# r9y9/gantts

Measured on AMD Instinct MI355X. Metric: acoustic frames/sec per G+D GAN step (B=32,T=512), higher is better.
Workload: dtype f32; 1 GPU; cfg2: TTS acoustic MLP G 425-512x3-187 + conditioned MLP D 483-256x3-1, Adagrad, MGE+ADV loss, global B=32 T=512 (32 sequences per GPU, strong scaling), fp32, dropout 0.5 (Philox); global_batch=32, per_gpu_batch=32, parallelism=dp1

## Files before the change

### gantts_amd/_lib.py

```python
import ctypes as C
import os

import torch

_HERE = os.path.dirname(os.path.abspath(__file__))
LIB_PATH = os.environ.get("GT_HIP_LIB") or os.path.join(_HERE, "libgantts_hip.so")

GT_OK, GT_ERR_INVALID, GT_ERR_HIP, GT_ERR_STATE, GT_ERR_DIM = 0, 1, 2, 3, 4
ROLE_G, ROLE_D = 0, 1
OPT_LSTM_PERSISTENT, OPT_LSTM_FWD_UNITS, OPT_LSTM_XCD_LOCAL, OPT_MATMUL_BF16, OPT_SPLIT_FIRST_LAYER = 2, 3, 4, 5, 6
OPT_COMM_D_ONE_MSG, OPT_COMM_EARLY_G, OPT_COMM_FORCE = 10, 11, 13
OPT_LAUNCH_RIDERS, OPT_COMM_CLOSE_INLINE, OPT_POLL_RESULTS = 14, 15, 16
OPT_COMM_TV_IN_SUMS, OPT_COMM_IPC, OPT_FUSED_DSTACK = 17, 18, 19
OPT_SRU_D_BF16 = 20
IPC_HANDLE_BYTES, IPC_MAX_WORLD = 64, 8
PROFILE_SLOTS = 16
LSTM_PATH_SLOTS, LSTM_PATH_STEPS, LSTM_PATH_DECLINED = 34, 32, 33
GEMM_PATH_SLOTS = 588
GEMM_B16_PATH_SLOTS = 66
SRU_PATH_SLOTS = 13
CAST_PLAIN_F32, CAST_PLAIN_BF16, CAST_SEQDROP, CAST_CAT, CAST_CATDROP, CAST_MULTI = 0, 1, 2, 3, 4, 5
CAST_MAX_JOBS = 8
GEMM_ROUTE_FORWARD, GEMM_ROUTE_FORWARD_SEG, GEMM_ROUTE_BACKWARD_DATA, GEMM_ROUTE_WEIGHT_GRAD, GEMM_ROUTE_WEIGHT_GRAD_SPLIT = 0, 1, 2, 3, 4
ARCH_MLP, ARCH_IN2OUT, ARCH_LSTM, ARCH_SRU, ARCH_IN2OUT_RNN = 0, 1, 2, 3, 4
OPT_ADAGRAD, OPT_ADAM = 0, 1
OPT_SGD, OPT_RMSPROP, OPT_ADADELTA, OPT_ADAMW, OPT_ADAMAX = 2, 3, 4, 5, 6
OPT_NADAM, OPT_RADAM, OPT_RPROP, OPT_ASGD = 7, 8, 9, 10
OPTF_NESTEROV, OPTF_CENTERED, OPTF_AMSGRAD, OPTF_BUFFER_LIVE = 1, 2, 4, 8
OPTF_DECOUPLED_WD = 32
MAX_STREAMS = 8
COMM_ID_BYTES = 128


class StreamConfig(C.Structure):
    _fields_ = [("n_streams", C.c_int32),
                ("stream_sizes", C.c_int32 * MAX_STREAMS),
                ("has_dynamic_features", C.c_int32 * MAX_STREAMS),
                ("num_windows", C.c_int32),
                ("adversarial_streams", C.c_int32 * MAX_STREAMS),
                ("mask_nth_mgc_for_adv_loss", C.c_int32),
                ("discriminator_linguistic_condition", C.c_int32),
                ("cond_dim", C.c_int32)]


class ModelDesc(C.Structure):
    _fields_ = [("arch", C.c_int32), ("in_dim", C.c_int32), ("out_dim", C.c_int32),
                ("num_hidden", C.c_int32), ("hidden_dim", C.c_int32), ("static_dim", C.c_int32),
                ("dropout", C.c_float), ("last_sigmoid", C.c_int32),
                ("bidirectional", C.c_int32), ("use_relu", C.c_int32),
                ("rnn_dropout", C.c_float), ("reserved_", C.c_int32),
                ("params", C.c_void_p), ("grads", C.c_void_p), ("n_params", C.c_int64)]


class OptimDesc(C.Structure):
    _fields_ = [("kind", C.c_int32), ("lr", C.c_float), ("weight_decay", C.c_float), ("eps", C.c_float),
                ("lr_decay", C.c_float), ("beta1", C.c_float), ("beta2", C.c_float),
                ("max_grad_norm", C.c_float), ("step", C.c_int64),
                ("state0", C.c_void_p), ("state1", C.c_void_p)]


class OptimDescEx(C.Structure):
    _fields_ = ([("kind", C.c_int32), ("flags", C.c_uint32)]
                + [(n, C.c_double) for n in ("lr", "weight_decay", "eps", "lr_decay", "beta1", "beta2", "momentum", "dampening", "alpha")]
                + [("max_grad_norm", C.c_float), ("reserved_", C.c_int32), ("step", C.c_int64),
                   ("state0", C.c_void_p), ("state1", C.c_void_p), ("state2", C.c_void_p)])


class OptimDescEx2(OptimDescEx):
    _fields_ = [(n, C.c_double) for n in ("momentum_decay", "etaminus", "etaplus", "step_size_min", "step_size_max", "lambd", "t0",
                                          "host_state0", "host_state1")]


class DResult(C.Structure):
    _fields_ = [("loss_d", C.c_float), ("loss_fake_d", C.c_float), ("loss_real_d", C.c_float),
                ("real_correct_count", C.c_float), ("fake_correct_count", C.c_float), ("grad_norm", C.c_float)]


class GResult(C.Structure):
    _fields_ = [("loss_mse", C.c_float), ("loss_mge", C.c_float), ("loss_adv", C.c_float),
                ("loss_g", C.c_float), ("grad_norm", C.c_float)]


class GemmCase(C.Structure):
    _fields_ = ([(n, C.c_int32) for n in ("route", "prec", "rows", "in_dim", "out_dim", "act", "drop")] + [("p", C.c_float)]
                + [("key0", C.c_uint32), ("key1", C.c_uint32)]
                + [(n, C.c_int32) for n in ("accumulate", "col0", "ncols", "wrap", "cd", "rider", "defer", "ldx", "ldw", "ldy", "ld_dy",
                                            "ldh", "ld_mask", "ld_addm", "ld_adv", "ld_dx")]
                + [(n, C.c_void_p) for n in ("x", "w", "bias", "y", "dy", "h", "mask", "addm", "adv", "dx", "dw", "db")])


class GemmB16Case(C.Structure):
    _fields_ = ([(n, C.c_int32) for n in ("route", "rows", "in_dim", "out_dim", "act", "drop")] + [("p", C.c_float)]
                + [("key0", C.c_uint32), ("key1", C.c_uint32)]
                + [(n, C.c_int32) for n in ("accumulate", "ldx", "ldw", "ld_dy", "ldh", "ld_mask", "ldc", "ldcb", "ldcbt")]
                + [(n, C.c_void_p) for n in ("x", "w", "bias", "dy", "h", "mask", "c", "cb", "cbt", "dw", "db")])


# ... 13 lines not shown

class CastCase(C.Structure):
    _fields_ = ([(n, C.c_int32) for n in ("kind", "cols", "ldi", "ldo", "colsum_accumulate", "T", "cd", "ldf", "n_jobs", "pad_")]
                + [(n, C.c_int64) for n in ("rows", "ldt", "N", "row_off")]
                + [(n, C.c_void_p) for n in ("in_", "out", "outT", "colsum", "mul", "x", "fa", "fb", "idx")]
                + [("jobs", CastJob * CAST_MAX_JOBS)])


_P, _I, _F, _L = C.c_void_p, C.c_int, C.c_float, C.c_int64

class DistortionSums(C.Structure):
    _fields_ = [(n, C.c_double) for n in
                ("s_mcd", "s_bap", "s_f0", "n_voiced", "n_vuv_err", "s_mse", "n_frames")]


SIGNATURES = {
    "gt_last_error": (C.c_char_p, []),
    "gt_version": (C.c_char_p, []),
    "gt_engine_create": (_I, [C.POINTER(StreamConfig), C.POINTER(_P)]),
    "gt_engine_destroy": (None, [_P]),
    "gt_bind_model": (_I, [_P, _I, C.POINTER(ModelDesc)]),
    "gt_bind_optimizer": (_I, [_P, _I, C.POINTER(OptimDesc)]),
    "gt_bind_optimizer_ex": (_I, [_P, _I, C.POINTER(OptimDescEx)]),
    "gt_op_optim_step": (_I, [C.POINTER(OptimDescEx), _P, _P, _L, _P, C.POINTER(_F), _P]),
    "gt_set_training": (_I, [_P, _I, _I]),
    "gt_set_lr": (_I, [_P, _I, _F]),
    "gt_get_optimizer_step": (_I, [_P, _I, C.POINTER(_L)]),
    "gt_get_optimizer_scalars": (_I, [_P, _I, C.POINTER(C.c_double)]),
    "gt_op_optim_scalars": (_I, [C.POINTER(OptimDescEx), _L, C.POINTER(C.c_double)]),
    "gt_set_seed": (_I, [_P, C.c_uint64]),
    "gt_set_dropout_mask": (_I, [_P, _I, _I, _I, _P]),
    "gt_op_philox_mask": (_I, [_P, _I, _I, _I, _L, _F, _L, _I, _P, _P]),
    "gt_set_lengths": (_I, [_P, C.POINTER(_L), _I, _P]),
    "gt_invalidate_mlpg_cache": (_I, [_P]),
    "gt_zero_grad": (_I, [_P, _I]),
    "gt_apply_generator": (_I, [_P, _P, _P, _I, _I, _P, _P, _P]),
    "gt_update_discriminator": (_I, [_P, _P, _P, _P, _P, _I, _I, _I, _F, C.POINTER(DResult), _P]),
    "gt_update_generator": (_I, [_P, _P, _P, _P, _P, _P, _F, _P, _I, _I, _I, _F, _F, _F, C.POINTER(GResult), _P]),
    "gt_set_loss_normalizer": (_I, [_P, _F]),
    "gt_set_loss_normalizer_device": (_I, [_P, _P]),
    "gt_set_option": (_I, [_P, _I, _I]),
    "gt_set_x_pitch": (_I, [_P, _I, _I]),
    "gt_set_tuning": (_I, [C.c_char_p, _I]),
    "gt_check_faults": (_I, [_P, _P]),
    "gt_lstm_path_counts": (_I, [_P, C.POINTER(_L), _I]),
    "gt_gemm_path_counts": (_I, [C.POINTER(_L), _I]),
    "gt_op_gemm_f32": (_I, [C.POINTER(GemmCase), _P]),
    "gt_gemm_b16_path_counts": (_I, [C.POINTER(_L), _I]),
    "gt_op_gemm_b16": (_I, [C.POINTER(GemmB16Case), _P]),
    "gt_op_cast_image": (_I, [C.POINTER(CastCase), _P]),
    "gt_sru_path_counts": (_I, [C.POINTER(_L), _I]),
    "gt_op_sru_scan": (_I, [C.POINTER(SruScanCase), _P]),
    "gt_op_sru_dx_adv_finish": (_I, [_P, _L, _I, _I, _P, _I, _P, _I, _P]),
    "gt_op_sru_input_mask": (_I, [_P, _I, _I, _F, C.c_uint32, C.c_uint32, _P, _I, _I, _P]),
    "gt_op_sru_input_dropout": (_I, [_P, _I, _P, _I, _I, _I, _I, _P, _P]),
    "gt_clear_faults": (_I, [_P, _P]),
    "gt_comm_unique_id": (_I, [_P]),
    "gt_comm_init": (_I, [_P, _I, _I, _P]),
    "gt_comm_destroy": (_I, [_P]),
    "gt_comm_info": (_I, [_P, C.POINTER(_I), C.POINTER(_I)]),
    "gt_comm_trace": (_I, [_P, _I]),
    "gt_comm_trace_read": (_I, [_P, C.POINTER(C.c_double), _I, C.POINTER(_I)]),
    "gt_set_shard": (_I, [_P, _I, _I]),
    "gt_comm_ipc_export": (_I, [_P, _P]),
    "gt_comm_ipc_attach": (_I, [_P, _I, _I, _P]),
    "gt_comm_ipc_messages": (_I, [_P, C.POINTER(C.c_longlong)]),
    "gt_update_discriminator_begin": (_I, [_P, _P, _P, _P, _P, _I, _I, _I, _F, _P]),
    "gt_update_discriminator_end": (_I, [_P, _I, C.POINTER(DResult), _P]),
    "gt_update_generator_begin": (_I, [_P, _P, _P, _P, _P, _P, _F, _P, _I, _I, _I, _F, _F, _F, _P]),
    "gt_update_generator_end": (_I, [_P, _I, _F, _F, _F, C.POINTER(GResult), _P]),
    "gt_update_discriminator_result": (_I, [_P, C.POINTER(DResult)]),
    "gt_update_generator_result": (_I, [_P, C.POINTER(GResult)]),
    "gt_scalar_buffer": (_I, [_P, C.POINTER(_P), C.POINTER(_I)]),
    "gt_model_forward": (_I, [_P, _I, _P, _P, _I, _I, _P, _P, _P]),
    "gt_flush_generator_grads": (_I, [_P, _P]),
    "gt_op_sequence_mask": (_I, [_P, _I, _I, _P, _P]),
    "gt_op_masked_mse": (_I, [_P, _P, _P, _I, _I, _I, C.POINTER(_F), _P, _P]),
    "gt_compute_distortions": (_I, [_P, _P, _I, _P, _P, _I, C.POINTER(_I), C.POINTER(_I), _I, C.POINTER(_L), _I, _I,
                                    C.POINTER(DistortionSums), _P]),
    "gt_op_gather_cols": (_I, [_P, _I, _P, _I, _P, _I, _I, _L, _P]),
    "gt_op_pad_sequences": (_I, [_P, _I, _P, _P, _I, _I, _P, _I, _P]),
    "gt_op_mlpg_forward": (_I, [_P, _P, _P, _I, _I, _P, _P]),
    "gt_op_mlpg_backward": (_I, [_P, _P, _P, _I, _I, _P, _P]),
    "gt_op_linear_forward": (_I, [_P, _I, _P, _P, _P, _I, _L, _I, _I, _I, _P, _F, _P]),
    "gt_op_linear_bf16": (_I, [_P, _P, _P, _L, _I, _I, _I, _P, _F, _P, _P, _P, _I, _P, _F, _P, _P, _P, _P, _P, _P]),
    "gt_profile_enable": (_I, [_I]),
    "gt_profile_read": (_I, [C.POINTER(C.c_double), C.POINTER(C.c_double), C.POINTER(_L)]),
    "gt_profile_bytes": (_I, [C.POINTER(C.c_double)]),
    "gt_op_linear_backward": (_I, [_P, _I, _P, _I, _P, _L, _I, _I, _P, _I, _P, _I, _P, _F, _P, _P, _P]),
}


def _build_if_missing():
    import fcntl
    import shutil
    import subprocess
    if os.path.isfile(LIB_PATH):
        return
    if shutil.which("hipcc") is None and not os.path.isfile("/opt/rocm/bin/hipcc"):
        return
    with open(os.path.join(_HERE, ".build.lock"), "w") as lock:
        fcntl.flock(lock, fcntl.LOCK_EX)
        try:
            if not os.path.isfile(LIB_PATH):
                subprocess.call(["make", "-j8", "-C", os.path.join(_HERE, "csrc")], stdout=subprocess.DEVNULL)
        finally:
            fcntl.flock(lock, fcntl.LOCK_UN)


def _load():
    _build_if_missing()
    if not os.path.isfile(LIB_PATH):
        raise ImportError(
            "gantts_amd: %s not found -- the HIP engine is the product and has no fallback. "
            "Build it: make -C %s" % (LIB_PATH, os.path.join(_HERE, "csrc")))
    lib = C.CDLL(LIB_PATH)
    for name, (res, args) in SIGNATURES.items():
        fn = getattr(lib, name)
        fn.restype, fn.argtypes = res, args
    return lib


lib = _load()


class GanttsHipError(RuntimeError):
    pass


def check(rc):
    if rc == GT_OK:
        return
    msg = lib.gt_last_error().decode("utf-8", "replace")
    if rc == GT_ERR_DIM:
        raise RuntimeError(msg)
    if rc == GT_ERR_INVALID:
        raise ValueError(msg)
    if rc == GT_ERR_STATE:
        raise RuntimeError(msg)
    raise GanttsHipError("HIP error: " + msg)


def ptr(t):
    return None if t is None else C.c_void_p(t.data_ptr())


def current_stream():
    import torch
    return C.c_void_p(torch.cuda.current_stream().cuda_stream)
```

### gantts_amd/csrc/eng_core.hip

```cpp
#include "engine_internal.hip.h"

using namespace gt;
static thread_local char g_err[512] = "";
int fail(int code, const char* fmt, ...) {
  va_list ap;
  va_start(ap, fmt);
  vsnprintf(g_err, sizeof(g_err), fmt, ap);
  va_end(ap);
  return code;
}
extern "C" const char* gt_last_error(void) { return g_err; }
extern "C" const char* gt_version(void) { return "gantts_hip 0.1 (gfx950, f32 MFMA)"; }

int ensure_dyn_lds(const void* kernel, size_t bytes) {
  static std::mutex mu;
  static std::map<std::pair<const void*, int>, size_t> done;
  int dev = 0;
  HIPCHK(hipGetDevice(&dev));
  std::lock_guard<std::mutex> lk(mu);
  size_t& cur = done[std::make_pair(kernel, dev)];
  if (bytes > cur) {
    HIPCHK(hipFuncSetAttribute(kernel, hipFuncAttributeMaxDynamicSharedMemorySize, (int)bytes));
    cur = bytes;
  }
// ... 281 lines not shown
  Net& n = e->net[role];
  if (!n.bound) return fail(GT_ERR_STATE, "bind the model before its optimizer");
  if (!n.d.grads) return fail(GT_ERR_INVALID, "model was bound without a grads buffer");
  if (od->kind != GT_OPT_ADAGRAD && od->kind != GT_OPT_ADAM) return fail(GT_ERR_INVALID, "unknown optimizer kind");
  if (!od->state0 || (od->kind == GT_OPT_ADAM && !od->state1)) return fail(GT_ERR_INVALID, "optimizer state buffer is null");
  gt_optim_desc_ex x;
  memset(&x, 0, sizeof(x));
  x.kind = od->kind; x.lr = od->lr; x.weight_decay = od->weight_decay; x.eps = od->eps; x.lr_decay = od->lr_decay;
  x.beta1 = od->beta1; x.beta2 = od->beta2; x.max_grad_norm = od->max_grad_norm; x.step = od->step;
  x.state0 = od->state0; x.state1 = od->state1;
  n.od = x;
  n.step = n.bound_step = od->step;
  n.buf_live = false;
  n.hs_cache = OptimScalarCache();
  n.has_opt = true;
  return GT_OK;
}
extern "C" int gt_bind_optimizer_ex(gt_engine* e, int role, const gt_optim_desc_ex* od) {
  if (!e || !od || role < 0 || role > 1) return fail(GT_ERR_INVALID, "bad argument");
  Net& n = e->net[role];
  if (!n.bound) return fail(GT_ERR_STATE, "bind the model before its optimizer");
  if (!n.d.grads) return fail(GT_ERR_INVALID, "model was bound without a grads buffer");
  CHK(optim_check_desc(od));
  optim_desc_copy(od, &n.od);
  if (od->kind != GT_OPT_ASGD) n.od.lr = (double)(float)od->lr;
  n.step = n.bound_step = od->step;
  n.hs_cache = OptimScalarCache();
  n.buf_live = (od->flags & GT_OPTF_BUFFER_LIVE) != 0;
  n.has_opt = true;
  return GT_OK;
}
extern "C" int gt_set_training(gt_engine* e, int role, int training) {
  if (!e || role < 0 || role > 1) return fail(GT_ERR_INVALID, "bad argument");
  e->net[role].training = training != 0;
  return GT_OK;
}
extern "C" int gt_set_lr(gt_engine* e, int role, float lr) {
  if (!e || role < 0 || role > 1 || !e->net[role].has_opt) return fail(GT_ERR_INVALID, "no optimizer bound");
  e->net[role].od.lr = lr;
  return GT_OK;
}
extern "C" int gt_get_optimizer_step(gt_engine* e, int role, int64_t* step) {
  if (!e || role < 0 || role > 1 || !step) return fail(GT_ERR_INVALID, "bad argument");
  *step = e->net[role].step;
  return GT_OK;
}
extern "C" int gt_get_optimizer_scalars(gt_engine* e, int role, double out[2]) {
  if (!e || role < 0 || role > 1 || !out) return fail(GT_ERR_INVALID, "bad argument");
  Net& n = e->net[role];
  if (!n.has_opt) return fail(GT_ERR_INVALID, "no optimizer bound");
  optim_host_scalars(n.od, n.step, &n.hs_cache, out);
  return GT_OK;
}
extern "C" int gt_set_seed(gt_engine* e, uint64_t seed) {
  if (!e) return fail(GT_ERR_INVALID, "null engine");
  e->seed = seed;
  e->step_counter = 0;
  return GT_OK;
}
extern "C" int gt_set_dropout_mask(gt_engine* e, int role, int pass, int layer, const float* mask) {
  if (!e || role < 0 || role > 1 || pass < 0 || pass > 2 || layer < 0 || layer > 15) return fail(GT_ERR_INVALID, "bad argument");
  e->net[role].inj[pass][layer] = mask;
  return GT_OK;
}
extern "C" int gt_set_option(gt_engine* e, int option, int value) {
  if (!e) return fail(GT_ERR_INVALID, "null engine");
  switch (option) {
    case GT_OPT_LSTM_PERSISTENT: e->lstm_persistent = value != 0; return GT_OK;
    case GT_OPT_LSTM_FWD_UNITS: e->lstm_fwd_upc = value; return GT_OK;
    case GT_OPT_LSTM_XCD_LOCAL: e->lstm_xcd_local = value != 0; return GT_OK;
    case GT_OPT_SPLIT_FIRST_LAYER:
      if (e->opt_split_first != (value != 0)) invalidate_d_images(e);
      e->opt_split_first = value != 0;
      return GT_OK;
    case GT_OPT_COMM_D_ONE_MSG: e->opt_comm_d_one_msg = value != 0; return GT_OK;
    case GT_OPT_COMM_EARLY_G: e->opt_comm_early_g = value != 0; return GT_OK;
    case GT_OPT_COMM_FORCE: e->opt_comm_force = value != 0; return GT_OK;
    case GT_OPT_COMM_CLOSE_INLINE: e->opt_comm_close_inline = value != 0; return GT_OK;
    case GT_OPT_COMM_IPC: e->opt_comm_ipc = value != 0; return GT_OK;
    case GT_OPT_FUSED_DSTACK: e->opt_fused_dstack = value < 0 ? 0 : value > 2 ? 2 : value; return GT_OK;
    case GT_OPT_COMM_TV_IN_SUMS: e->opt_comm_tv_in_sums = value != 0; return GT_OK;
    case GT_OPT_POLL_RESULTS: e->opt_poll_results = value != 0; return GT_OK;
    case GT_OPT_LAUNCH_RIDERS: e->opt_launch_riders = value != 0; return GT_OK;
    case GT_OPT_MATMUL_BF16:
      if (e->matmul_bf16 != (value != 0)) {
        invalidate_d_images(e);
        e->g_pass_valid = false; e->leak_pending = false; e->cxd_src = nullptr;
        e->d_begin_done = false; e->g_begin_done = false;
      }
      e->matmul_bf16 = value != 0;
      return GT_OK;
    case GT_OPT_SRU_D_BF16:
      if (value != 0 && value != 1) return fail(GT_ERR_INVALID, "GT_OPT_SRU_D_BF16 takes 0 or 1, not %d", value);
      if (e->sru_d_bf16 != (value != 0)) { invalidate_d_images(e); e->leak_pending = false; e->d_begin_done = false; e->g_begin_done = false; }
      e->sru_d_bf16 = value != 0;
      return GT_OK;
  }
  return fail(GT_ERR_INVALID, "unknown option %d", option);
}
GtTuning& gt_tuning() {
  static GtTuning t = [] {
    GtTuning v;
    auto geti = [](const char* n, int d) { const char* s = getenv(n); return s && s[0] ? atoi(s) : d; };
    v.gemm_pair = geti("GT_GEMM_PAIR", v.gemm_pair); v.pair_order = geti("GT_PAIR_ORDER", v.pair_order);
    { const char* s = getenv("GT_GEMM_TILES"); v.gemm_tiles_big = s && !strcmp(s, "big") ? 1 : 0; }
    v.gemm_unaligned = geti("GT_GEMM_UNALIGNED", v.gemm_unaligned); v.tn_wgs = geti("GT_TN_WGS", v.tn_wgs); v.tn_split_wgs = geti("GT_TN_SPLIT_WGS", v.tn_split_wgs); v.split_fused = geti("GT_SPLIT_FUSED", v.split_fused);
    v.b16_tiles = geti("GT_B16_TILES", v.b16_tiles); v.b16_wg_tile = geti("GT_B16_WG_TILE", v.b16_wg_tile); v.b16_dma = geti("GT_B16_DMA", v.b16_dma);
    v.mlpg_fpl = geti("GT_MLPG_FPL", v.mlpg_fpl); v.mlpg_tt = geti("GT_MLPG_TT", v.mlpg_tt); v.sru_coop = geti("GT_SRU_COOP", v.sru_coop); v.sru_cs_waves = geti("GT_SRU_CS_WAVES", v.sru_cs_waves); v.leak_rider = geti("GT_LEAK_RIDER", v.leak_rider);
    v.head_vec = geti("GT_HEAD_VEC", v.head_vec);
    v.lstm_bt = geti("GT_LSTM_BT", v.lstm_bt);
    if (v.lstm_bt != 8 && v.lstm_bt != 16) v.lstm_bt = 0;
    return v;
  }();
  return t;
}
extern "C" int gt_set_tuning(const char* name, int value) {
  if (!name) return fail(GT_ERR_INVALID, "null name");
  GtTuning& t = gt_tuning();
  struct { const char* n; int* p; } tab[] = {
      {"gemm_pair", &t.gemm_pair}, {"pair_order", &t.pair_order}, {"gemm_tiles_big", &t.gemm_tiles_big}, {"gemm_unaligned", &t.gemm_unaligned},
      {"tn_wgs", &t.tn_wgs}, {"tn_split_wgs", &t.tn_split_wgs}, {"split_fused", &t.split_fused}, {"b16_tiles", &t.b16_tiles},
      {"b16_wg_tile", &t.b16_wg_tile}, {"b16_dma", &t.b16_dma}, {"mlpg_fpl", &t.mlpg_fpl}, {"mlpg_tt", &t.mlpg_tt}, {"sru_coop", &t.sru_coop}, {"sru_cs_waves", &t.sru_cs_waves}, {"leak_rider", &t.leak_rider}, {"head_vec", &t.head_vec}};
  if (!strcmp(name, "lstm_bt")) {
    if (value != 0 && value != 8 && value != 16) return fail(GT_ERR_INVALID, "lstm_bt must be 0 (by shape), 8 or 16, not %d", value);
    t.lstm_bt = value;
    return GT_OK;
  }
  if (!strcmp(name, "sru_lw")) { t.sru_coop = value >= 2; return GT_OK; }
  for (auto& e : tab) if (!strcmp(e.n, name)) { *e.p = value; return GT_OK; }
  return fail(GT_ERR_INVALID, "unknown tuning knob '%s'", name);
}
extern "C" int gt_set_x_pitch(gt_engine* e, int ld_generator_input, int ld_condition) {
  if (!e || ld_generator_input < 0 || ld_condition < 0) return fail(GT_ERR_INVALID, "bad argument");
  e->ld_gx = ld_generator_input; e->ld_cx = ld_condition;
  return GT_OK;
}
extern "C" int gt_set_loss_normalizer(gt_engine* e, float tv) {
  if (!e) return fail(GT_ERR_INVALID, "null engine");
  e->tv_override = tv;
  e->tv_dev = nullptr;
  return GT_OK;
}
extern "C" int gt_set_loss_normalizer_device(gt_engine* e, const double* tv_dev) {
  if (!e) return fail(GT_ERR_INVALID, "null engine");
  e->tv_dev = tv_dev;
  e->tv_mask = nullptr; e->tv_inflight = false;
  return GT_OK;
}
extern "C" int gt_set_lengths(gt_engine* e, const int64_t* lengths_host, int B, void* stream) {
  if (!e || !lengths_host || B < 1) return fail(GT_ERR_INVALID, "bad argument");
  hipStream_t s = (hipStream_t)stream;
  e->h_lengths.resize(B);
  for (int b = 0; b < B; ++b) {
    if (lengths_host[b] < 0 || lengths_host[b] > 0x3fffffff) return fail(GT_ERR_INVALID, "length out of range");
    e->h_lengths[b] = (int)lengths_host[b];
  }
  if (2 * B > e->len_cap) {
    HIPCHK(hipStreamSynchronize(s));
    const int cap = std::max(64, 2 * B + B);
    for (int i = 0; i < gt_engine::LEN_RING; ++i) {
      if (e->len_ev[i]) HIPCHK(hipEventSynchronize(e->len_ev[i]));
      if (e->len_host[i]) { HIPCHK(hipHostFree(e->len_host[i])); e->len_host[i] = nullptr; }
      HIPCHK(hipHostMalloc((void**)&e->len_host[i], (size_t)cap * sizeof(int)));
      if (!e->len_ev[i]) HIPCHK(hipEventCreateWithFlags(&e->len_ev[i], hipEventDisableTiming));
    }
    e->len_cap = cap;
// ... 127 lines not shown
```

### gantts_amd/csrc/eng_ops.hip

```cpp
#include "engine_internal.hip.h"

using namespace gt;
extern "C" int gt_op_sequence_mask(const int64_t* lengths, int B, int T, float* mask, void* stream) {
  if (!lengths || !mask || B < 1 || T < 1) return fail(GT_ERR_INVALID, "bad argument");
  hipLaunchKernelGGL(sequence_mask_kernel, dim3(cdiv((long)B * T, 256)), dim3(256), 0, (hipStream_t)stream, (const long*)lengths, B, T, mask);
  LAUNCH_CHECK();
  return GT_OK;
}

extern "C" int gt_op_masked_mse(const float* input, const float* target, const float* mask, int B, int T, int D, float* loss_out,
                                float* grad_input, void* stream) {
  if (!input || !target) return fail(GT_ERR_INVALID, "null tensor");
  if (!mask) return fail(GT_ERR_INVALID, "Should provide either lengths or mask");
  hipStream_t s = (hipStream_t)stream;
  const long N = (long)B * T;
  static thread_local Scratch tls_ws;
  CHK(tls_ws.ensure(1024 + 1024 * sizeof(double)));
  void* ws = tls_ws.p;
  StepScalars* sc = (StepScalars*)ws;
  double* part = (double*)((char*)ws + 1024);
  hipLaunchKernelGGL(mask_sum_kernel, dim3(1), dim3(1024), 0, s, mask, (int)N, -1.f, (const double*)nullptr, sc);
  const int nblk = (int)std::min<long>(1000, cdiv(N * D, RED_THREADS * 4));
  hipLaunchKernelGGL(masked_sqerr_kernel, dim3(nblk), dim3(RED_THREADS), 0, s, input, D, target, D, mask, N, D, part, grad_input, D,
                     1.f, sc);
  hipLaunchKernelGGL(sum_partials_kernel, dim3(1), dim3(256), 0, s, part, nblk, &sc->s_mse);
  StepScalars h;
  hipError_t err = hipMemcpyAsync(&h, sc, sizeof(h), hipMemcpyDeviceToHost, s);
  if (err == hipSuccess) err = hipStreamSynchronize(s);
  if (err != hipSuccess) return fail(GT_ERR_HIP, "masked_mse: %s", hipGetErrorString(err));
  if (loss_out) *loss_out = (float)h.s_mse / h.tv;
  return GT_OK;
}

extern "C" int gt_compute_distortions(const float* y_static, const float* y_hat_static, int Ds, const void* stat_mean,
                                      const void* stat_std, int stats_f64, const int32_t* col_stat_host,
                                      const int32_t* col_role_host, int vuv_col, const int64_t* lengths_host, int B, int T,
                                      gt_distortion_sums* out, void* stream) {
  if (!y_static || !y_hat_static || !stat_mean || !stat_std || !col_stat_host || !col_role_host || !out)
    return fail(GT_ERR_INVALID, "null argument");
  if (Ds < 1 || B < 1 || T < 1 || vuv_col >= Ds) return fail(GT_ERR_DIM, "bad sizes: Ds=%d B=%d T=%d vuv_col=%d", Ds, B, T, vuv_col);
  hipStream_t s = (hipStream_t)stream;
  const long N = (long)B * T;
  const int nblk = (int)std::min<long>(1024, cdiv(N, 4));
  std::vector<int> host(2 * Ds + B);
  for (int c = 0; c < Ds; ++c) {
    if (col_stat_host[c] < 0) return fail(GT_ERR_INVALID, "negative statistics index");
    host[c] = col_stat_host[c];
    host[Ds + c] = col_role_host[c];
  }
  for (int b = 0; b < B; ++b) {
    const int64_t n = lengths_host ? lengths_host[b] : T;
    if (n < 0 || n > T) return fail(GT_ERR_INVALID, "length %lld outside [0, T=%d]", (long long)n, T);
    host[2 * Ds + b] = (int)n;
  }
  static thread_local Scratch tls_ws;
  const size_t off_part = ((host.size() * sizeof(int) + 255) / 256) * 256;
  const size_t off_out = off_part + (size_t)nblk * DIST_NSUM * sizeof(double);
  CHK(tls_ws.ensure(off_out + DIST_NSUM * sizeof(double)));
  void* ws = tls_ws.p;
  int* d_int = (int*)ws;
  double* part = (double*)((char*)ws + off_part);
  double* d_out = (double*)((char*)ws + off_out);
  hipError_t err = hipMemcpyAsync(d_int, host.data(), host.size() * sizeof(int), hipMemcpyHostToDevice, s);
  if (err == hipSuccess) {
    if (stats_f64)
      hipLaunchKernelGGL(distortion_kernel<double>, dim3(nblk), dim3(256), 0, s, y_static, y_hat_static, Ds, (const double*)stat_mean,
                         (const double*)stat_std, d_int, d_int + Ds, vuv_col, d_int + 2 * Ds, B, T, part);
    else
      hipLaunchKernelGGL(distortion_kernel<float>, dim3(nblk), dim3(256), 0, s, y_static, y_hat_static, Ds, (const float*)stat_mean,
                         (const float*)stat_std, d_int, d_int + Ds, vuv_col, d_int + 2 * Ds, B, T, part);
    hipLaunchKernelGGL(distortion_finalize_kernel, dim3(1), dim3(64 * DIST_NSUM), 0, s, part, nblk, d_out);
    err = hipGetLastError();
  }
  double h[DIST_NSUM];
  if (err == hipSuccess) err = hipMemcpyAsync(h, d_out, sizeof(h), hipMemcpyDeviceToHost, s);
  if (err == hipSuccess) err = hipStreamSynchronize(s);
  if (err != hipSuccess) return fail(GT_ERR_HIP, "compute_distortions: %s", hipGetErrorString(err));
  out->s_mcd = h[0]; out->s_bap = h[1]; out->s_f0 = h[2]; out->n_voiced = h[3];
  out->n_vuv_err = h[4]; out->s_mse = h[5]; out->n_frames = h[6];
  return GT_OK;
}

extern "C" int gt_op_pad_sequences(const float* ragged, int D, const int64_t* start, const int64_t* len, int B, int T, float* out, int ld_out,
                                   void* stream) {
  if (!ragged || !start || !len || !out || D < 1 || B < 1 || T < 1 || ld_out < D) return fail(GT_ERR_INVALID, "bad argument");
  hipLaunchKernelGGL(pad_sequences_kernel, dim3(cdiv((long)B * T * ld_out, 256)), dim3(256), 0, (hipStream_t)stream, ragged, D,
                     (const long*)start, (const long*)len, B, T, out, ld_out);
  LAUNCH_CHECK();
  return GT_OK;
}
extern "C" int gt_op_gather_cols(const float* in, int ld_in, const int32_t* idx, int n_idx, float* out, int ld_out,
                                 int out_col_offset, int64_t rows, void* stream) {
  if (!in || !out || n_idx < 0 || rows < 0) return fail(GT_ERR_INVALID, "bad argument");
  if (rows == 0 || n_idx == 0) return GT_OK;
  hipLaunchKernelGGL(gather_cols_kernel, dim3(cdiv(rows * n_idx, 256)), dim3(256), 0, (hipStream_t)stream, in, ld_in, 0, idx, out,
                     ld_out, out_col_offset, (int)rows, n_idx);
  LAUNCH_CHECK();
  return GT_OK;
}

extern "C" int gt_op_mlpg_forward(gt_engine* e, const float* y, const float* R, int B, int T, float* y_static, void* stream) {
  CHK(check_common(e, B, T));
  if (!y || !R || !y_static) return fail(GT_ERR_INVALID, "null tensor");
  hipStream_t s = (hipStream_t)stream;
  CHK(ensure_band(e, R, T, s));
  return mlpg_forward(e, y, e->Dout_cfg, e->d_scol, e->d_sstride, e->Ds, y_static, e->Ds, B, T, s);
}
extern "C" int gt_op_mlpg_backward(gt_engine* e, const float* g_static, const float* R, int B, int T, float* g_y, void* stream) {
  CHK(check_common(e, B, T));
  if (!g_static || !R || !g_y) return fail(GT_ERR_INVALID, "null tensor");
  hipStream_t s = (hipStream_t)stream;
  CHK(ensure_band(e, R, T, s));
  return mlpg_backward(e, g_static, e->Ds, e->d_scol, e->d_sstride, e->Ds, g_y, e->Dout_cfg, B, T, 0.f, nullptr, nullptr, 0, nullptr, s);
}

static DropoutSpec buffer_spec(const float* keep_mask, float p, int ld) {
  DropoutSpec d = no_drop();
  if (keep_mask && p > 0.f) { d.mode = DROP_BUFFER; d.mask = keep_mask; d.ld_mask = ld; d.p = p; d.scale = 1.f / (1.f - p); }
  return d;
}

extern "C" int gt_op_linear_forward(const float* X, int ldx, const float* W, const float* bias, float* Y, int ldy, int64_t rows,
                                    int in_dim, int out_dim, int act, const float* keep_mask, float p, void* stream) {
  if (!X || !W || !Y || rows < 1 || in_dim < 1 || out_dim < 1) return fail(GT_ERR_INVALID, "bad argument");
  if (act < 0 || act > 2) return fail(GT_ERR_INVALID, "unknown activation");
  tl_gemm_prec = PREC_F32;
  return linear_forward(X, ldx, W, in_dim, bias, Y, ldy, rows, in_dim, out_dim, act, buffer_spec(keep_mask, p, out_dim), (hipStream_t)stream);
}

extern "C" int gt_op_linear_backward(const float* dY, int lddy, const float* X, int ldx, const float* W, int64_t rows, int in_dim,
                                     int out_dim, float* dX, int lddx, const float* H_prev, int act_prev,
                                     const float* keep_mask_prev, float p_prev, float* dW, float* db, void* stream) {
  if (!dY || rows < 1 || in_dim < 1 || out_dim < 1) return fail(GT_ERR_INVALID, "bad argument");
  hipStream_t s = (hipStream_t)stream;
  tl_gemm_prec = PREC_F32;
  if (dX) {
    if (!W) return fail(GT_ERR_INVALID, "dX requested without W");
    if (act_prev != ACT_NONE && !H_prev) return fail(GT_ERR_INVALID, "activation derivative requested without H_prev");
    CHK(linear_backward_data(dY, lddy, W, in_dim, 0, dX, lddx, rows, out_dim, in_dim, act_prev, H_prev, in_dim,
                             buffer_spec(keep_mask_prev, p_prev, in_dim), s));
  }
  if (dW || db) {
    if (dW && !X) return fail(GT_ERR_INVALID, "dW requested without X");
    Scratch slabs, colp;
    int r = linear_backward_weight(dY, lddy, X, ldx, rows, out_dim, in_dim, dW, db, false, slabs, colp, s);
    hipError_t err = hipStreamSynchronize(s);
    slabs.release(); colp.release();
    if (r) return r;
    if (err != hipSuccess) return fail(GT_ERR_HIP, "linear_backward: %s", hipGetErrorString(err));
  }
  return GT_OK;
}

extern "C" int gt_op_linear_bf16(const float* X, const float* W, const float* bias, int64_t rows, int in_dim, int out_dim, int act,
                                 const float* keep_mask, float p, float* Y, const float* dY, const float* H_prev, int act_prev,
                                 const float* keep_mask_prev, float p_prev, float* dX, float* dW, float* db,
                                 float* Y_image, float* YT_image, void* stream) {
  if (!X || !W || rows < 1 || in_dim < 1 || out_dim < 1) return fail(GT_ERR_INVALID, "bad argument");
  if (act < 0 || act > 2 || act_prev < 0 || act_prev > 2) return fail(GT_ERR_INVALID, "unknown activation");
  hipStream_t s = (hipStream_t)stream;
  const int in8 = pad8(in_dim), out8 = pad8(out_dim);
  const long rows8 = pad8(rows);
  Scratch xb, xbt, wb, wbt, yb, ybt, dyb, dybt, hb, slabs, colp;
  int r = GT_OK;
  auto body = [&]() -> int {
    CHK(xb.ensure((size_t)rows * in8 * 2)); CHK(xbt.ensure((size_t)in_dim * rows8 * 2));
    CHK(wb.ensure((size_t)out_dim * in8 * 2)); CHK(wbt.ensure((size_t)in_dim * out8 * 2));
    CHK(cast_transpose(X, in_dim, rows, in_dim, xb.as<__bf16>(), in8, xbt.as<__bf16>(), rows8, nullptr, false, &colp, s));
    CHK(cast_transpose(W, in_dim, out_dim, in_dim, wb.as<__bf16>(), in8, wbt.as<__bf16>(), out8, nullptr, false, &colp, s));
    if (Y) {
      CHK(yb.ensure((size_t)rows * out8 * 2)); CHK(ybt.ensure((size_t)out_dim * rows8 * 2));
      GemmB16Args g = b16_args();
      g.A = xb.as<__bf16>(); g.lda = in8; g.B = wb.as<__bf16>(); g.ldb = in8; g.M = (int)rows; g.N = out_dim; g.K = in_dim;
      g.C = Y; g.ldc = out_dim; g.Cb = yb.as<__bf16>(); g.ldcb = out8; g.CbT = ybt.as<__bf16>(); g.ldcbt = (int)rows8;
      g.bias = bias; g.epi = B16_FWD; g.act = act; g.drop = buffer_spec(keep_mask, p, out_dim);
      CHK(launch_gemm_b16(g, 1, s));
      if (Y_image) {
        hipLaunchKernelGGL(bf16_to_f32_kernel, dim3(cdiv(rows * out_dim, 256)), dim3(256), 0, s, (const __bf16*)yb.as<__bf16>(), (long)out8, rows, out_dim, Y_image);
        LAUNCH_CHECK();
      }
      if (YT_image) {
        hipLaunchKernelGGL(bf16_to_f32_kernel, dim3(cdiv(rows * out_dim, 256)), dim3(256), 0, s, (const __bf16*)ybt.as<__bf16>(), rows8, (long)out_dim, (int)rows, YT_image);
        LAUNCH_CHECK();
      }
    }
    if (dY) {
      CHK(dyb.ensure((size_t)rows * out8 * 2)); CHK(dybt.ensure((size_t)out_dim * rows8 * 2));
      CHK(cast_transpose(dY, out_dim, rows, out_dim, dyb.as<__bf16>(), out8, dybt.as<__bf16>(), rows8, nullptr, false, &colp, s));
      if (dX) {
// ... 597 lines not shown
```

### gantts_amd/csrc/eng_step.hip

```cpp
#include "engine_internal.hip.h"
#include "dstack_f32.hip.h"

using namespace gt;
int ensure_band(gt_engine* e, const float* R, int T, hipStream_t s) {
  MlpgCache& m = e->mlpg;
  ++m.tick;
  for (auto* b : m.entries)
    if (b->R == R && b->T == T) { b->last_use = m.tick; m.cur = b; return GT_OK; }
  const int nW = e->cfg.num_windows;
  CHK(m.tmp.ensure((size_t)(2 * T - 1) * sizeof(float)));
  hipLaunchKernelGGL(mlpg_offset_max_kernel, dim3(2 * T - 1), dim3(256), 0, s, R, T, nW, m.tmp.as<float>());
  LAUNCH_CHECK();
  std::vector<float> off(2 * T - 1);
  HIPCHK(hipMemcpyAsync(off.data(), m.tmp.p, off.size() * sizeof(float), hipMemcpyDeviceToHost, s));
  HIPCHK(hipStreamSynchronize(s));
  float peak = 0.f;
  for (float v : off) peak = fmaxf(peak, v);
  if (!(peak > 0.f) || !isfinite(peak)) return fail(GT_ERR_INVALID, "MLPG matrix R is empty or not finite");
  int kb = 0;
  for (int o = -(T - 1); o <= T - 1; ++o)
    if (off[o + T - 1] > 1e-9f * peak) kb = std::max(kb, abs(o));
  if (kb > 63 || (kb > 48 && kb > T / 4))
    return fail(GT_ERR_INVALID, "MLPG matrix R is not banded (half-width %d of T=%d): only window sets whose "
                "R = (W^T W)^-1 W^T decays (hparams.py:22-26) are supported", kb, T);
  MlpgBand* b = nullptr;
  if (m.entries.size() >= MlpgCache::MAX_ENTRIES) {
    size_t lru = 0;
    for (size_t i = 1; i < m.entries.size(); ++i) if (m.entries[i]->last_use < m.entries[lru]->last_use) lru = i;
    b = m.entries[lru];
    HIPCHK(hipStreamSynchronize(s));
  } else {
    b = new MlpgBand();
    m.entries.push_back(b);
  }
  const int nb = 2 * kb + 1;
  b->R = nullptr;
  CHK(b->band.ensure((size_t)T * nW * nb * sizeof(float)));
  hipLaunchKernelGGL(mlpg_extract_band_kernel, dim3(cdiv((long)T * nW * nb, 256)), dim3(256), 0, s, R, T, nW, kb, b->band.as<float>());
  LAUNCH_CHECK();
  b->R = R; b->T = T; b->kb = kb; b->last_use = m.tick;
  m.cur = b;
  return GT_OK;
}
extern "C" int gt_invalidate_mlpg_cache(gt_engine* e) {
  if (!e) return fail(GT_ERR_INVALID, "null engine");
  HIPCHK(hipDeviceSynchronize());
  e->mlpg.clear();
  return GT_OK;
}

static int mlpg_tile_frames() { return gt_tuning().mlpg_tt == 16 ? 16 : 32; }
int mlpg_forward(gt_engine* e, const float* y, int ldy, const int* scol, const int* sstride, int Ds,
                 float* ys, int ldys, int B, int T, hipStream_t s) {
  const int nW = e->cfg.num_windows, kb = e->mlpg.cur->kb;
  auto lds_of = [&](int tt) { return ((size_t)(tt + 2 * kb) * nW * MLPG_CC + (size_t)tt * nW * (2 * kb + 1 + 2 * MLPG_PAD)) * sizeof(float); };
  const int tt = mlpg_tile_frames();
  const size_t lds = lds_of(tt);
  dim3 grid(B * cdiv(T, tt), cdiv(Ds, MLPG_CC));
  const int fpl = gt_tuning().mlpg_fpl;
#define GT_MLPG_FWD(F, TTV) { CHK(ensure_dyn_lds((const void*)mlpg_forward_kernel<F, TTV>, lds)); \
    hipLaunchKernelGGL((mlpg_forward_kernel<F, TTV>), grid, dim3(MLPG_THREADS), lds, s, y, ldy, e->mlpg.cur->band.as<float>(), kb, nW, scol, sstride, Ds, ys, ldys, B, T); }
  if (tt == 16) GT_MLPG_FWD(2, 16)
  else { if (fpl == 1) GT_MLPG_FWD(1, 32) else if (fpl == 2) GT_MLPG_FWD(2, 32) else GT_MLPG_FWD(4, 32) }
#undef GT_MLPG_FWD
  LAUNCH_CHECK();
  return GT_OK;
}
int mlpg_backward(gt_engine* e, const float* gs, int ldgs, const int* scol, const int* sstride, int Ds,
                  float* gy, int ldgy, int B, int T, float mse_w, const float* yhat, const float* ytgt, int ldt,
                  const float* mask, hipStream_t s) {
  const int nW = e->cfg.num_windows, kb = e->mlpg.cur->kb;
  auto lds_of = [&](int tt) { return ((size_t)(tt + 2 * kb) * MLPG_CC + (size_t)(tt + 2 * kb) * nW * (2 * kb + 1 + 2 * MLPG_PAD)) * sizeof(float); };
  const int tt = mlpg_tile_frames();
  const size_t lds = lds_of(tt);
  dim3 grid(B * cdiv(T, tt), cdiv(Ds, MLPG_CC));
  const int fpl = gt_tuning().mlpg_fpl;
#define GT_MLPG_BWD(F, TTV) { CHK(ensure_dyn_lds((const void*)mlpg_backward_kernel<F, TTV>, lds)); \
    hipLaunchKernelGGL((mlpg_backward_kernel<F, TTV>), grid, dim3(MLPG_THREADS), lds, s, gs, ldgs, e->mlpg.cur->band.as<float>(), kb, nW, scol, sstride, Ds, \
                       gy, ldgy, B, T, mse_w, yhat, ytgt, ldt, mask, e->sc()); }
  if (tt == 16) GT_MLPG_BWD(2, 16)
  else { if (fpl == 1) GT_MLPG_BWD(1, 32) else if (fpl == 2) GT_MLPG_BWD(2, 32) else GT_MLPG_BWD(4, 32) }
#undef GT_MLPG_BWD
  LAUNCH_CHECK();
  return GT_OK;
}

static int stage_injected(gt_engine* e, int role, int layer, const int* passes, int npass, long rows_each, int width,
                          const float** out, hipStream_t s) {
  Net& n = e->net[role];
  *out = nullptr;
  if (!n.training || n.d.dropout <= 0.f) return GT_OK;
  bool any = false, all = true;
  for (int i = 0; i < npass; ++i) { any |= n.inj[passes[i]][layer] != nullptr; all &= n.inj[passes[i]][layer] != nullptr; }
  if (!any) return GT_OK;
  if (!all) return fail(GT_ERR_INVALID, "injected dropout masks must be given for every pass of a step or for none");
  if (npass == 1) { *out = n.inj[passes[0]][layer]; return GT_OK; }
  const size_t per_layer = (size_t)npass * rows_each * width * sizeof(float);
  CHK(e->dmask.ensure(per_layer * n.d.num_hidden));
  float* base = (float*)((char*)e->dmask.p + per_layer * layer);
  for (int i = 0; i < npass; ++i)
    HIPCHK(hipMemcpyAsync(base + (size_t)i * rows_each * width, n.inj[passes[i]][layer], (size_t)rows_each * width * sizeof(float),
                          hipMemcpyDeviceToDevice, s));
  *out = base;
  return GT_OK;
}

struct FirstSplit {
  const float* x; int ldx; int cd;
  const float* xp; int ldxp;
  const float* adv; int ld_adv;
  long wrap;
};
static int pitched_rows(gt_engine* e, int slot, const float* p, int ld, int cols, long rows, const float** out, int* ldo, hipStream_t s) {
  if (gemm_vec_ok(p, ld)) { *out = p; *ldo = ld; return GT_OK; }
  gt_engine::Pitched& P = e->pitched[slot];
  const int ldp = (cols + 3) & ~3;
  if (!(P.src == p && P.ld == ld && P.cols == cols && P.rows == rows && P.step == e->step_counter)) {
    CHK(P.buf.ensure((size_t)rows * ldp * sizeof(float)));
    hipLaunchKernelGGL(repitch_kernel, dim3(cdiv(rows * (ldp / 4), 256)), dim3(256), 0, s, p, ld, cols, rows, P.buf.as<float>(), ldp);
    LAUNCH_CHECK();
    P.src = p; P.ld = ld; P.cols = cols; P.rows = rows; P.step = e->step_counter;
  }
  *out = P.buf.as<float>(); *ldo = ldp;
  return GT_OK;
}

static int stack_forward(gt_engine* e, int role, const float* in, int ld_in, long rows, std::vector<Scratch>& acts,
                         const int* passes, int npass, long rows_each, std::vector<DropoutSpec>& specs, hipStream_t s,
                         const FirstSplit* fs = nullptr, int max_layers = 1 << 30 ) {
  Net& n = e->net[role];
  specs.resize(n.hidden.size());
  const float* cur = in;
  int ld = ld_in;
  for (size_t l = 0; l < n.hidden.size(); ++l) {
    const Lin& L = n.hidden[l];
    CHK(acts[l].ensure((size_t)rows * L.out * sizeof(float)));
    const float* inj = nullptr;
    CHK(stage_injected(e, role, (int)l, passes, npass, rows_each, L.out, &inj, s));
    specs[l] = drop_spec(e, role, passes[0], (int)l, inj, L.out, npass == 2 ? rows_each : 0);
    if ((int)l >= max_layers) continue;
    if (l == 0 && fs && specs[l].mode == DROP_PHILOX && gt_tuning().split_fused && gemm_vec_ok(fs->x, fs->ldx, true) &&
        gemm_vec_ok(L.W, L.in, true) && gemm_vec_ok(fs->adv, fs->ld_adv, true) && fs->wrap > 64 && gemm_small_tiles_ok() &&
        tl_gemm_prec == PREC_F32 && (rows == fs->wrap || rows == 2 * fs->wrap)) {
      GemmArgs g;
      memset(&g, 0, sizeof(g));
      g.A = fs->x; g.lda = fs->ldx; g.B = L.W; g.ldb = L.in; g.C = acts[l].as<float>(); g.ldc = L.out;
      g.M = (int)fs->wrap; g.N = L.out; g.K = fs->cd; g.bias = L.b; g.act = ACT_LEAKY_DROPOUT; g.drop = specs[l];
      g.A_seg = fs->adv; g.lda_seg = fs->ld_adv; g.B_seg = L.W + fs->cd; g.K_seg = L.in - fs->cd;
      g.dual_rows = rows == 2 * fs->wrap ? (int)fs->wrap : 0;
      CHK(launch_gemm(GEMM_NT, g, 1, s));
      cur = acts[l].as<float>();
      ld = L.out;
      continue;
    }
    if (l == 0 && fs) {
      const int Da = L.in - fs->cd;
      CHK(e->d_pre.ensure((size_t)fs->wrap * L.out * sizeof(float)));
      CHK(linear_forward(fs->x, fs->ldx, L.W, L.in, L.b, e->d_pre.as<float>(), L.out, fs->wrap, fs->cd, L.out, ACT_NONE, no_drop(), s));
      GemmArgs g;
      memset(&g, 0, sizeof(g));
      g.A = fs->adv; g.lda = fs->ld_adv; g.B = L.W + fs->cd; g.ldb = L.in; g.C = acts[l].as<float>(); g.ldc = L.out;
      g.M = (int)rows; g.N = L.out; g.K = Da; g.act = ACT_LEAKY_DROPOUT; g.drop = specs[l];
      g.addm = e->d_pre.as<float>(); g.ld_addm = L.out; g.addm_wrap = (int)fs->wrap;
      CHK(launch_gemm(GEMM_NT, g, 1, s));
// ... 729 lines not shown
  CHK(d_pass_head(e, p, hc, nullptr, s));
  e->early_done = false;
  if (plain_early) CHK(post_early_results(e, s, hc.ticket));
  if (comm_early) CHK(comm_early_results(e, GT_ROLE_D, unnorm ? &e->sc()->tv_sum : &e->sc()->s_real, unnorm ? 5 : 4, 0.f, 0.f, 0.f, s));
  if (tr) {
    CHK(comm_grads_ready(e, GT_ROLE_D, D.last.dW, (long)D.last.in * D.last.out + D.last.out, s));
    Net& G = e->net[GT_ROLE_G];
    const bool want_leak = G.bound && G.d.grads && e->g_pass_valid && y_hat_static == e->last_yhs && e->N == N;
    if (want_leak && e->leak_pending)
      return fail(GT_ERR_STATE, "update_discriminator called twice without optimizer_g.zero_grad() (train.py:538)");
    float* leak = nullptr;
    if (want_leak) { CHK(e->leak.ensure((size_t)N * e->Da * sizeof(float))); leak = e->leak.as<float>(); }
    CHK(d_pass_backward(e, p, leak, s));
    D.grads_dirty = true;
    if (want_leak) { e->leak_pending = true; e->leak_unnorm = unnorm; }
  }
  CHK(comm_finish_step(e, GT_ROLE_D, tr, &e->sc()->s_real, comm_early ? 0 : 4, s));
  e->d_begin_done = true;
  return GT_OK;
}

static void fill_d_result(const StepResults* h, gt_d_result* out) {
  out->loss_d = h->loss_d; out->loss_fake_d = h->loss_fake_d; out->loss_real_d = h->loss_real_d;
  out->real_correct_count = h->real_correct; out->fake_correct_count = h->fake_correct;
  out->grad_norm = h->gnorm_d;
}
static void fill_g_result(const StepResults* h, gt_g_result* out) {
  out->loss_mse = h->loss_mse; out->loss_mge = h->loss_mge; out->loss_adv = h->loss_adv;
  out->loss_g = h->loss_g; out->grad_norm = h->gnorm_g;
}

extern "C" int gt_update_discriminator_end(gt_engine* e, int train, gt_d_result* out, void* stream) {
  if (!e) return fail(GT_ERR_INVALID, "null argument");
  if (!e->d_begin_done) return fail(GT_ERR_STATE, "gt_update_discriminator_end without _begin");
  hipStream_t s = (hipStream_t)stream;
  e->d_begin_done = false;
  if (!out && e->early_done) return fail(GT_ERR_STATE, "deferred results are a split-phase feature");
  if (train) CHK(optimizer_step(e, GT_ROLE_D, &e->sc()->gnorm2_d, s));
  if (e->early_done) {
    CHK(wait_early_results(e));
    e->early_done = false;
  } else {
    hipLaunchKernelGGL(finalize_d_kernel, dim3(1), dim3(1), 0, s, e->sc(), e->res(), train ? 0 : 1);
    LAUNCH_CHECK();
    if (!out) return post_deferred_results(e, GT_ROLE_D, s);
    CHK(fetch_results(e, s));
  }
  fill_d_result(e->h_res, out);
  return GT_OK;
}
extern "C" int gt_update_discriminator_result(gt_engine* e, gt_d_result* out) {
  if (!e || !out) return fail(GT_ERR_INVALID, "null argument");
  if (!e->def_pending[GT_ROLE_D]) return fail(GT_ERR_STATE, "no deferred discriminator result pending");
  HIPCHK(hipEventSynchronize(e->ev_def[GT_ROLE_D]));
  e->def_pending[GT_ROLE_D] = false;
  fill_d_result(e->h_def[GT_ROLE_D], out);
  return GT_OK;
}

extern "C" int gt_update_discriminator(gt_engine* e, const float* x, const float* y_static, const float* y_hat_static,
                                       const float* mask, int B, int T, int train, float eps, gt_d_result* out, void* stream) {
  if (!e) return fail(GT_ERR_INVALID, "null engine");
  e->early = true;
  int r = gt_update_discriminator_begin(e, x, y_static, y_hat_static, mask, B, T, train, eps, stream);
  e->early = false;
  if (r != GT_OK) { e->early_done = false; e->d_unnorm = false; e->ticket_wait = 0; return r; }
  return gt_update_discriminator_end(e, train, out, stream);
}

static int sum_sqerr(gt_engine* e, const float* a, int lda, const float* b, int ldb, const float* mask, long rows, int D,
                     double* out, float* g, int ldg, float gscale, hipStream_t s, int* deferred_blocks = nullptr) {
  const int nblk = (int)std::min<long>(1024, cdiv(rows * D, RED_THREADS * 4));
  CHK(e->partial.ensure(4096 * sizeof(double)));
  double* part = e->partial.as<double>() + 1024;
  hipLaunchKernelGGL(masked_sqerr_kernel, dim3(nblk), dim3(RED_THREADS), 0, s, a, lda, b, ldb, mask, rows, D, part, g, ldg, gscale, e->sc());
  LAUNCH_CHECK();
  if (deferred_blocks) { *deferred_blocks = nblk; return GT_OK; }
  hipLaunchKernelGGL(sum_partials_kernel, dim3(1), dim3(256), 0, s, part, nblk, out);
  LAUNCH_CHECK();
  return GT_OK;
}

static int generator_backward(gt_engine* e, const float* x, const float* y, const float* y_hat, const float* mask,
                              float mse_w, hipStream_t s) {
  Net& G = e->net[GT_ROLE_G];
  const long N = e->N;
  const int B = e->B, T = e->T, Do = G.d.out_dim;
  const bool mlp_body = !(has_lstm_body(G.d.arch) || G.d.arch == GT_ARCH_SRU);
  const int ldgy = mlp_body && (is_i2o(G.d.arch) || e->g_used_mlpg) ? (Do + 3) & ~3 : Do;
  CHK(e->gy.ensure((size_t)N * ldgy * sizeof(float)));
  float* gy = e->gy.as<float>();
  const float* gs = e->gs.as<float>();
  if (is_i2o(G.d.arch)) {
    const int sd = G.d.static_dim;
    if (G.d.arch == GT_ARCH_IN2OUT_RNN) mse_w = 0.f;
    CHK(e->dgx.ensure((size_t)N * sd * sizeof(float)));
    CHK(e->dtz.ensure((size_t)N * sd * sizeof(float)));
    hipLaunchKernelGGL(highway_backward_kernel, dim3(cdiv(N * sd, 256)), dim3(256), 0, s, gs, sd, e->tx.as<float>(), sd,
                       e->gx.as<float>(), sd, e->dgx.as<float>(), sd, e->dtz.as<float>(), sd, N, sd);
    LAUNCH_CHECK();
    CHK(linear_backward_weight(e->dtz.as<float>(), sd, x, G.d.in_dim, N, sd, sd, G.gate.dW, G.gate.db, G.grads_dirty, e->slabs,
                               e->colp, s, &e->sdefer[GT_ROLE_G]));
    CHK(comm_grads_ready(e, GT_ROLE_G, G.gate.dW, (long)sd * sd + sd, s));
    CHK(mlpg_backward(e, e->dgx.as<float>(), sd, e->d_scol_i2o, e->d_sstride_i2o, sd, gy, ldgy, B, T, mse_w, y_hat, y, Do, mask, s));
  } else if (e->g_used_mlpg) {
    CHK(mlpg_backward(e, gs, e->Ds, e->d_scol, e->d_sstride, e->Ds, gy, ldgy, B, T, mse_w, y_hat, y, Do, mask, s));
  } else {
    if (mse_w != 0.f) CHK(sum_sqerr(e, y_hat, Do, y, Do, mask, N, Do, &e->sc()->s_mse, gy, Do, mse_w, s));
    hipLaunchKernelGGL(slab_reduce_kernel, dim3(cdiv(N * Do, 256)), dim3(256), 0, s, gs, 0L, 1, N * Do, gy, mse_w != 0.f ? 1 : 0);
    LAUNCH_CHECK();
  }
  if (G.d.last_sigmoid && !is_i2o(G.d.arch)) {
    hipLaunchKernelGGL(sigmoid_grad_kernel, dim3(cdiv(N * Do, 256)), dim3(256), 0, s, gy, ldgy, y_hat, Do, N, Do);
    LAUNCH_CHECK();
  }
  if (has_lstm_body(G.d.arch) || G.d.arch == GT_ARCH_SRU) {
    CHK(has_lstm_body(G.d.arch) ? lstm_backward(e, x, gy, B, T, s) : sru_backward(e, x, gy, B, T, s));
    G.grads_dirty = true;
    return GT_OK;
  }
  if (use_b16(e, GT_ROLE_G)) {
    const int H = G.d.hidden_dim;
    CHK(e->gy_b.ensure(N, Do, true));
    CHK(cast_transpose(gy, ldgy, N, Do, e->gy_b.r(), e->gy_b.ld, e->gy_b.t(), e->gy_b.ldt, nullptr, false, &e->colp, s));
    B16Img& top = e->g_actb.back();
    CHK(weight_grad_b16(e->gy_b.t(), e->gy_b.ldt, top.t(), top.ldt, N, Do, G.last.in, G.last.dW, G.last.db, G.grads_dirty, e->slabs, s,
                        &e->sdefer[GT_ROLE_G]));
    CHK(comm_grads_ready(e, GT_ROLE_G, G.last.dW, (long)Do * G.last.in + Do, s));
    const LinShadow& ws = e->wsh[GT_ROLE_G][G.hidden.size()];
    CHK(e->dz_b[0].ensure(N, H, true));
    GemmB16Args g = b16_args();
    g.A = e->gy_b.r(); g.lda = e->gy_b.ld; g.B = ws.wt.as<__bf16>(); g.ldb = ws.ldwt; g.M = (int)N; g.N = H; g.K = Do;
    g.epi = B16_BWD_DATA; g.act = ACT_LEAKY_DROPOUT; g.H = top.r(); g.ldh = top.ld; g.drop = e->g_specs.back();
    g.Cb = e->dz_b[0].r(); g.ldcb = e->dz_b[0].ld; g.CbT = e->dz_b[0].t(); g.ldcbt = (int)e->dz_b[0].ldt;
    CHK(launch_gemm_b16(g, 1, s));
    CHK(stack_backward_b16(e, GT_ROLE_G, e->xin_b.t(), e->xin_b.ldt, N, e->g_actb, e->g_specs, 0, true, nullptr, 0, 0, 0, 0, 0, s));
    G.grads_dirty = true;
    return GT_OK;
  }
  const Lin& Lt = G.hidden.back();
  const int H = G.d.hidden_dim;
  CHK(e->dzA.ensure((size_t)2 * N * H * sizeof(float)));
  CHK(e->dzB.ensure((size_t)2 * N * H * sizeof(float)));
  const GemmArgs nn_last = backward_data_args(gy, ldgy, G.last.W, G.last.in, 0, e->dzA.as<float>(), H, N, Do, H, ACT_LEAKY_DROPOUT,
                                              e->g_act.back().as<float>(), H, e->g_specs.back());
  bool rode = false;
  CHK(linear_backward_weight(gy, ldgy, e->g_act.back().as<float>(), Lt.out, N, Do, G.last.in, G.last.dW, G.last.db, G.grads_dirty,
                             e->slabs, e->colp, s, &e->sdefer[GT_ROLE_G], &nn_last, &rode));
  CHK(comm_grads_ready(e, GT_ROLE_G, G.last.dW, (long)Do * G.last.in + Do, s));
  if (!rode) CHK(launch_gemm(GEMM_NN, nn_last, 1, s));
  const float* xin = x;
  int ldxin = gx_pitch(e);
  if (!gemm_vec_ok(x, ldxin) && tl_gemm_prec == PREC_F32) {
    if (e->img_cat.valid && e->img_cat.x == x && e->cfg.discriminator_linguistic_condition && cond_dim(e) == G.d.in_dim && e->dcat.p) {
      ldxin = (d_in_dim(e) + 3) & ~3;
      xin = e->dcat.as<float>() + N * ldxin;
    } else {
      const int slot = (e->pitched[0].src == x && e->pitched[0].ld == gx_pitch(e) && e->pitched[0].cols == G.d.in_dim && e->pitched[0].step == e->step_counter) ? 0 : 1;
      CHK(pitched_rows(e, slot, x, gx_pitch(e), G.d.in_dim, N, &xin, &ldxin, s));
    }
  }
  CHK(stack_backward(e, GT_ROLE_G, xin, ldxin, N, e->g_act, e->g_specs, e->dzA.as<float>(), e->dzB.as<float>(), true,
                     nullptr, 0, 0, 0, 0, 0, s));
  G.grads_dirty = true;
  return GT_OK;
}

extern "C" int gt_update_generator_begin(gt_engine* e, const float* x, const float* y, const float* y_hat, const float* y_static,
                                         const float* y_hat_static, float adv_w, const float* mask, int B, int T, int train,
                                         float mse_w, float mge_w, float eps, void* stream) {
  CHK(check_common(e, B, T));
  Net& G = e->net[GT_ROLE_G];
  Net& D = e->net[GT_ROLE_D];
  if (!G.bound) return fail(GT_ERR_STATE, "generator not bound");
  if (!y || !y_hat || !y_static || !y_hat_static || !mask) return fail(GT_ERR_INVALID, "null tensor");
  hipStream_t s = (hipStream_t)stream;
  const long N = (long)B * T;
  const bool tr = train != 0;
  if (tr) {
    if (!e->g_pass_valid || y_hat != e->last_yhat || y_hat_static != e->last_yhs || N != e->N)
      return fail(GT_ERR_STATE, "update_generator(phase=\"train\") needs the y_hat / y_hat_static returned by the last apply_generator");
    if (!G.d.grads) return fail(GT_ERR_STATE, "phase == \"train\" but the generator was bound without grads");
  }
  const int Do = G.d.out_dim;
  const int Ds = is_i2o(G.d.arch) ? G.d.static_dim : e->Ds;
  if (comm_on(e) && tr && G.grads_dirty)
    return fail(GT_ERR_STATE, "data-parallel step: optimizer_g.zero_grad() must precede update_generator");
  e->sdefer[GT_ROLE_G].reset(e->early && tr && G.has_opt);
  CHK(ensure_tv(e, mask, N, s));
  const bool direct = !is_i2o(G.d.arch) && !e->g_used_mlpg;
  const bool early_fold = e->early && !comm_on(e) && !(tr && direct && mse_w != 0.f);
  int mse_blocks = 0, mge_pre_blocks = 0;
  const bool riders = early_fold && e->opt_launch_riders;
  const bool riders_dp = e->early && comm_on(e) && e->opt_launch_riders && !(tr && direct && mse_w != 0.f);
  if (riders || riders_dp) {
    mse_blocks = (int)std::min<long>(1024, cdiv(N * Do, RED_THREADS * 4));
    mge_pre_blocks = (int)std::min<long>(1024, cdiv(N * Ds, RED_THREADS * 4));
    CHK(e->partial.ensure(4096 * sizeof(double)));
    hipLaunchKernelGGL(g_losses_kernel, dim3(mse_blocks + mge_pre_blocks), dim3(RED_THREADS), 0, s, y_hat, Do, y, Do, Do, mse_blocks,
                       e->partial.as<double>() + 1024, y_hat_static, Ds, y_static, Ds, Ds, e->partial.as<double>(), mask, N);
    LAUNCH_CHECK();
  } else if (!(tr && direct && mse_w != 0.f)) {
    CHK(sum_sqerr(e, y_hat, Do, y, Do, mask, N, Do, &e->sc()->s_mse, nullptr, 0, 0.f, s, early_fold ? &mse_blocks : nullptr));
  }
  e->g_has_adv = adv_w > 0.f;
  float* gadv = nullptr;
  int head_blocks = 0;
  if (adv_w > 0.f) {
    if (!D.bound) return fail(GT_ERR_STATE, "adv_w > 0 but no discriminator bound");
    DPass p;
    CHK(d_pass_plan(e, x, nullptr, y_hat_static, Ds, 1, B, T, false, &p));
    AdvRiders none;
    memset(&none, 0, sizeof(none));
    CHK(d_pass_input(e, p, none, s));
    CHK(d_pass_forward(e, p, s));
    if (tr) { CHK(e->gadv.ensure((size_t)N * e->Da * sizeof(float))); gadv = e->gadv.as<float>(); }
    HeadCall hc;
    memset(&hc, 0, sizeof(hc));
    hc.mode = HEAD_G_ADV; hc.rows = p.rows; hc.n_real = N; hc.mask = mask; hc.n_mask = N; hc.eps = eps; hc.want_grad = tr; hc.want_w = false;
    hc.defer_scalars = riders || riders_dp ? &head_blocks : nullptr;
    CHK(d_pass_head(e, p, hc, gadv, s));
    if (tr) CHK(d_pass_backward(e, p, gadv, s));
  }
  const bool early_ok = e->early && !(tr && direct && mse_w != 0.f);
  const bool early_now = early_ok && !comm_on(e), comm_early = early_ok && comm_on(e) && e->opt_comm_early_g;
  int mge_blocks = 0;
  e->early_done = false;
  {
    const int nblk = (int)std::min<long>(1024, cdiv(N * Ds, RED_THREADS * 4));
    CHK(e->partial.ensure(4096 * sizeof(double)));
    float* gs = nullptr;
    if (tr) { CHK(e->gs.ensure((size_t)N * Ds * sizeof(float))); gs = e->gs.as<float>(); }
    const float* leak = (tr && e->leak_pending) ? e->leak.as<float>() : nullptr;
    GFinalize fin;
    memset(&fin, 0, sizeof(fin));
    const bool rid = riders || riders_dp;
    if (rid) {
      fin.on = 1; fin.sc = e->sc(); fin.out = riders ? early_res_target(e) : (StepResults*)nullptr; fin.adv_w = adv_w; fin.mse_w = mse_w; fin.mge_w = mge_w;
      fin.has_adv = e->g_has_adv ? 1 : 0;
      fin.part_mge = e->partial.as<double>(); fin.n_mge = mge_pre_blocks;
      fin.part_mse = e->partial.as<double>() + 1024; fin.n_mse = mse_blocks;
      fin.hp = head_blocks ? e->headp.as<HeadPartials>() : (const HeadPartials*)nullptr; fin.n_hp = head_blocks;
      if (riders) { fin.ticket_value = take_ticket(e); fin.ticket = fin.ticket_value ? e->ticket_dev() : (unsigned*)nullptr; }
    }
    if (tr || !rid)
      hipLaunchKernelGGL(static_grad_kernel, dim3(nblk + (rid ? 1 : 0)), dim3(RED_THREADS), 0, s, y_hat_static, Ds,
                         y_static, Ds, mask, N, Ds, mge_w, e->d_adv_inv, leak, e->Da, gadv, e->Da, adv_w, gs, Ds,
                         rid ? (double*)nullptr : e->partial.as<double>(), e->sc(), fin, leak && e->leak_unnorm ? 1 : 0);
    else
      hipLaunchKernelGGL(finalize_g_rider_kernel, dim3(1), dim3(RED_THREADS), 0, s, fin);
    LAUNCH_CHECK();
    mge_blocks = nblk;
    if (riders) CHK(post_early_results(e, s, fin.ticket_value));
    else if (!early_now && !riders_dp) {
      hipLaunchKernelGGL(sum_partials_kernel, dim3(1), dim3(256), 0, s, e->partial.as<double>(), nblk, &e->sc()->s_mge);
      LAUNCH_CHECK();
    }
  }
  if (early_now && !riders) {
    hipLaunchKernelGGL(finalize_g_kernel, dim3(1), dim3(256), 0, s, e->sc(), early_res_target(e), adv_w, mse_w, mge_w, e->g_has_adv ? 1 : 0, 1,
                       (const double*)e->partial.as<double>(), mge_blocks,
                       mse_blocks ? (const double*)(e->partial.as<double>() + 1024) : (const double*)nullptr, mse_blocks);
    LAUNCH_CHECK();
    CHK(post_early_results(e, s));
  }
  if (comm_early) CHK(comm_early_results(e, GT_ROLE_G, &e->sc()->s_adv, 3, adv_w, mse_w, mge_w, s));
  if (tr) {
    CHK(generator_backward(e, e->last_x, y, y_hat, mask, mse_w, s));
    e->leak_pending = false; e->leak_unnorm = false;
  }
  CHK(comm_finish_step(e, GT_ROLE_G, tr, &e->sc()->s_adv, comm_early ? 0 : 3, s));
  e->g_begin_done = true;
  return GT_OK;
}

extern "C" int gt_update_generator_end(gt_engine* e, int train, float adv_w, float mse_w, float mge_w, gt_g_result* out,
                                       void* stream) {
  if (!e) return fail(GT_ERR_INVALID, "null argument");
  if (!e->g_begin_done) return fail(GT_ERR_STATE, "gt_update_generator_end without _begin");
  hipStream_t s = (hipStream_t)stream;
  e->g_begin_done = false;
  if (!out && e->early_done) return fail(GT_ERR_STATE, "deferred results are a split-phase feature");
  if (train) CHK(optimizer_step(e, GT_ROLE_G, &e->sc()->gnorm2_g, s));
  if (e->early_done) {
    CHK(wait_early_results(e));
    e->early_done = false;
  } else {
    hipLaunchKernelGGL(finalize_g_kernel, dim3(1), dim3(1), 0, s, e->sc(), e->res(), adv_w, mse_w, mge_w, e->g_has_adv ? 1 : 0,
                       train ? 0 : 1, (const double*)nullptr, 0, (const double*)nullptr, 0);
    LAUNCH_CHECK();
    if (!out) return post_deferred_results(e, GT_ROLE_G, s);
    CHK(fetch_results(e, s));
  }
  fill_g_result(e->h_res, out);
  return fault_seen(e);
}
extern "C" int gt_update_generator_result(gt_engine* e, gt_g_result* out) {
  if (!e || !out) return fail(GT_ERR_INVALID, "null argument");
  if (!e->def_pending[GT_ROLE_G]) return fail(GT_ERR_STATE, "no deferred generator result pending");
  HIPCHK(hipEventSynchronize(e->ev_def[GT_ROLE_G]));
  e->def_pending[GT_ROLE_G] = false;
  fill_g_result(e->h_def[GT_ROLE_G], out);
  return GT_OK;
}

extern "C" int gt_update_generator(gt_engine* e, const float* x, const float* y, const float* y_hat, const float* y_static,
                                   const float* y_hat_static, float adv_w, const float* mask, int B, int T, int train,
                                   float mse_w, float mge_w, float eps, gt_g_result* out, void* stream) {
  if (!e) return fail(GT_ERR_INVALID, "null engine");
  e->early = true;
  int r = gt_update_generator_begin(e, x, y, y_hat, y_static, y_hat_static, adv_w, mask, B, T, train, mse_w, mge_w, eps, stream);
  e->early = false;
  if (r != GT_OK) { e->early_done = false; return r; }
  return gt_update_generator_end(e, train, adv_w, mse_w, mge_w, out, stream);
}

extern "C" int gt_flush_generator_grads(gt_engine* e, void* stream) {
  if (!e) return fail(GT_ERR_INVALID, "null engine");
  Net& G = e->net[GT_ROLE_G];
  if (!G.bound || !G.d.grads || !e->g_pass_valid) return fail(GT_ERR_STATE, "no generator pass to back-propagate");
  hipStream_t s = (hipStream_t)stream;
  tl_gemm_prec = e->matmul_bf16 ? PREC_BF16 : PREC_F32;
  CHK(fault_seen(e));
  e->sdefer[GT_ROLE_G].reset(false);
  const long N = e->N;
  const int Ds = is_i2o(G.d.arch) ? G.d.static_dim : e->Ds;
  CHK(e->gs.ensure((size_t)N * Ds * sizeof(float)));
  HIPCHK(hipMemsetAsync(e->gs.p, 0, (size_t)N * Ds * sizeof(float), s));
  if (e->leak_pending) {
    std::vector<int>& cols = e->h_adv_cols;
    for (int j = 0; j < e->Da; ++j) {
      hipLaunchKernelGGL(gather_cols_kernel, dim3(cdiv(N, 256)), dim3(256), 0, s, e->leak.as<float>(), e->Da, j, (const int*)nullptr,
                         e->gs.as<float>(), Ds, cols[j], (int)N, 1);
    }
    if (e->leak_unnorm) hipLaunchKernelGGL(scale_by_inv_tv_kernel, dim3(cdiv(N * Ds, 256)), dim3(256), 0, s, e->gs.as<float>(), N * Ds, e->sc());
    LAUNCH_CHECK();
  }
  CHK(generator_backward(e, e->last_x, e->last_yhat, e->last_yhat, (const float*)nullptr, 0.f, s));
  e->leak_pending = false; e->leak_unnorm = false;
  HIPCHK(hipStreamSynchronize(s));
  return GT_OK;
}

extern "C" int gt_model_forward(gt_engine* e, int role, const float* x, const float* R, int B, int T, float* out, float* out2,
                                void* stream) {
  CHK(check_common(e, B, T));
  if (role < 0 || role > 1 || !e->net[role].bound) return fail(GT_ERR_STATE, "model not bound");
  if (!x || !out) return fail(GT_ERR_INVALID, "null tensor");
  hipStream_t s = (hipStream_t)stream;
  Net& n = e->net[role];
  const long N = (long)B * T;
// ... 40 lines not shown
```

### gantts_amd/csrc/engine_internal.hip.h

```cpp
#pragma once
#include <hip/hip_runtime.h>
#include <math.h>
#include <stdarg.h>
#include <stdio.h>
#include <stdlib.h>
#include <string.h>
#include <algorithm>
#include <map>
#include <mutex>
#include <string>
#include <vector>

#pragma GCC visibility push(default)
#include "../../include/gantts_hip.h"
#pragma GCC visibility pop
#include "frame_kernels.hip.h"
#include "gemm_f32.hip.h"
#include "gemm_bf16s.hip.h"
#include "sru_args.hip.h"

using namespace gt;

int fail(int code, const char* fmt, ...);
#define HIPCHK(expr)                                                                         \
  do {                                                                                       \
    hipError_t _e = (expr);                                                                  \
    if (_e != hipSuccess)                                                                    \
      return fail(GT_ERR_HIP, "%s failed: %s (%s:%d)", #expr, hipGetErrorString(_e), __FILE__, __LINE__); \
  } while (0)
#define CHK(expr)            \
  do {                       \
    int _r = (expr);         \
    if (_r != GT_OK) return _r; \
  } while (0)
#define LAUNCH_CHECK() HIPCHK(hipGetLastError())

static inline bool env_flag(const char* name, bool dflt) { const char* v = getenv(name); return v && v[0] ? v[0] != '0' : dflt; }
static inline int cdiv(long a, long b) { return (int)((a + b - 1) / b); }
static inline int pad8(long n) { return (int)((n + 7) & ~7L); }

int ensure_dyn_lds(const void* kernel, size_t bytes);
int gemm_cu_count();

struct GtTuning {
  int gemm_pair = 1;
  int pair_order = 1;
  int gemm_tiles_big = 0;
  int gemm_unaligned = 1;
  int tn_wgs = 512;
  int split_fused = 1;
  int tn_split_wgs = 1024;
  int b16_tiles = 0;
  int b16_wg_tile = 0;
  int b16_dma = 1;
  int mlpg_fpl = 2;
  int head_vec = 0;
  int mlpg_tt = 0;
  int leak_rider = 1;
  int sru_cs_waves = 0;
  int sru_coop = 1;
  int lstm_bt = 0;
};
GtTuning& gt_tuning();

struct GemmProfiler {
  bool on = false;
  int only_kind = -1;
  bool wants(int kind) const { return on && (only_kind < 0 || only_kind == kind); }
  struct Rec { int kind, bn, am; double flops, bytes; hipEvent_t e0, e1; };
  double last_bytes[GT_PROFILE_SLOTS] = {};
  std::vector<Rec> recs;
  std::vector<hipEvent_t> pool;
  hipEvent_t get() {
    if (!pool.empty()) { hipEvent_t e = pool.back(); pool.pop_back(); return e; }
    hipEvent_t e; (void)hipEventCreate(&e); return e;
  }
};
extern GemmProfiler g_prof;

struct Scratch {
  void* p = nullptr;
  size_t bytes = 0;
  int ensure(size_t need) {
    if (need <= bytes) return GT_OK;
    if (p) { HIPCHK(hipDeviceSynchronize()); HIPCHK(hipFree(p)); p = nullptr; bytes = 0; }
    const size_t cap = need + need / 8;
    HIPCHK(hipMalloc(&p, cap));
    bytes = cap;
    return GT_OK;
  }
  void release() { if (p) { (void)hipFree(p); p = nullptr; bytes = 0; } }
  template <typename T> T* as() const { return (T*)p; }
};

struct SlabDefer {
  Scratch pool;
  size_t used = 0;
  SlabJobs jobs;
  int blocks = 0;
  bool active = false;
  SlabDefer() { jobs.n = 0; jobs.pad_ = 0; }
  void reset(bool on) { jobs.n = 0; blocks = 0; used = 0; active = on; }
};

struct Lin { float *W, *b, *dW, *db; int in, out; };
struct B16Img {
  Scratch rm, tr;
  int ld = 0; long ldt = 0;
  __bf16* r() { return rm.as<__bf16>(); }
  __bf16* t() { return tr.as<__bf16>(); }
  int ensure(long rows, int cols, bool want_t) {
    ld = pad8(cols); ldt = pad8(rows);
    CHK(rm.ensure((size_t)rows * ld * 2 + 64));
    if (want_t) CHK(tr.ensure((size_t)cols * ldt * 2 + 64));
    return GT_OK;
  }
  void release() { rm.release(); tr.release(); }
};
struct LinShadow { Scratch w, wt; int ldw = 0, ldwt = 0; };
static inline bool is_i2o(int arch) { return arch == GT_ARCH_IN2OUT || arch == GT_ARCH_IN2OUT_RNN; }
static inline bool has_lstm_body(int arch) { return arch == GT_ARCH_LSTM || arch == GT_ARCH_IN2OUT_RNN; }
struct LstmDirP { float *Wih, *Whh, *bih, *bhh, *dWih, *dWhh, *dbih, *dbhh; };
struct LstmLayerP { int in; LstmDirP d[2]; };
struct SruLayerP { int in, k; float *W, *b, *dW, *db; };

struct OptimScalarCache { bool valid = false; long step = 0; float mu_product = 1.f; };

struct Net {
  bool bound = false;
  gt_model_desc d;
  std::vector<Lin> hidden;
  Lin last, gate;
  std::vector<LstmLayerP> lstm;
  std::vector<SruLayerP> sru;
  bool training = true;
  bool grads_dirty = false;
  bool has_opt = false;
  gt_optim_desc_ex od;
  long step = 0;
  long bound_step = 0;
  bool buf_live = false;
  OptimScalarCache hs_cache;
  const float* inj[3][16];
  Net() { memset(inj, 0, sizeof(inj)); }
};

struct MlpgBand {
  const float* R = nullptr;
  int T = 0, kb = 0;
  uint64_t last_use = 0;
  Scratch band;
};
struct MlpgCache {
  static constexpr size_t MAX_ENTRIES = 256;
  std::vector<MlpgBand*> entries;
  MlpgBand* cur = nullptr;
  uint64_t tick = 0;
  Scratch tmp;
  void clear() { for (auto* b : entries) { b->band.release(); delete b; } entries.clear(); cur = nullptr; }
};

struct gt_engine {
  gt_stream_config cfg;
  Net net[2];
  uint64_t seed = 0x5DEECE66DULL;
  uint64_t step_counter = 0;
  float tv_override = -1.f;
  const double* tv_dev = nullptr;
  int Dout_cfg = 0, Ds = 0, Da = 0;
  std::vector<int> h_scol, h_sstride, h_adv_cols, h_adv_inv;
  int *d_scol = nullptr, *d_sstride = nullptr, *d_adv_cols = nullptr, *d_adv_inv = nullptr;
  int *d_scol_i2o = nullptr, *d_sstride_i2o = nullptr; int i2o_ds = 0;
  MlpgCache mlpg;
  std::vector<Scratch> g_act, d_act;
  Scratch dcat, dzA, dzB, leak, gadv, gs, gy, slabs, colp, partial, headp, headw, dmask, tx, gx, dgx, dtz, dout;
  Scratch scal;
  StepResults* h_res = nullptr;
  StepResults* h_res_dev = nullptr;
  int B = 0, T = 0; long N = 0;
  const float* last_x = nullptr; const float* last_yhat = nullptr; const float* last_yhs = nullptr;
  bool g_pass_valid = false, leak_pending = false;
  struct DImage {
    bool valid = false; const float* x = nullptr; const float* yhs = nullptr;
    bool holds(const float* x_, const float* yhs_) const { return valid && x == x_ && yhs == yhs_; }
    void built(const float* x_, const float* yhs_) { valid = true; x = x_; yhs = yhs_; }
  };
  DImage img_cat, img_cat_b, img_adv2;
  bool d_begin_done = false, g_begin_done = false, g_has_adv = false, g_used_mlpg = false;
  const float* tv_mask = nullptr; long tv_n = 0; float tv_ovr = 0.f;
  bool early = false, early_done = false;
  hipEvent_t ev_res = nullptr;
  unsigned ticket_next = 0, ticket_wait = 0;
  unsigned* ticket_dev() { return h_res_dev ? (unsigned*)((char*)h_res_dev + 64) : nullptr; }
  volatile unsigned* ticket_host() { return (volatile unsigned*)((char*)h_res + 64); }
  StepResults* h_def[2] = {nullptr, nullptr}; hipEvent_t ev_def[2] = {nullptr, nullptr}; bool def_pending[2] = {false, false};
  std::vector<DropoutSpec> g_specs, d_specs;
  std::vector<Scratch> l_xproj, l_gates, l_cst, l_out, l_outd;
  Scratch i2o_gout;
  Scratch l_state, l_dout, l_hshift;
  std::vector<Scratch> dl_xproj, dl_gates, dl_cst, dl_out, dl_outd;
  Scratch dl_dout, dl_hshift, d_dx0;
  Scratch l_xch;
  struct GtComm* comm = nullptr;
  struct GtIpc* ipc = nullptr;
  bool opt_comm_ipc = env_flag("GT_COMM_IPC", true);
  int dp_rank = 0, dp_world = 1;
  int chk_B = 0, chk_T = 0;
  std::vector<std::pair<long, long>> comm_done[2];
  std::vector<std::pair<long, long>> comm_pending[2];
  Scratch comm_tv;
  bool tv_inflight = false;
  std::vector<B16Img> g_actb, d_actb;
  B16Img xin_b, dcat_b, gy_b, dz_b[2], fwd_b;
  std::vector<B16Img> l_in_b;
  std::vector<B16Img> s_in_b;
  B16Img s_du_b;
  std::vector<LinShadow> ssh;
  std::vector<B16Img> l_dg_b;
  B16Img l_hs_b;
  std::vector<LinShadow> lsh;
  std::vector<LinShadow> wsh[2];
  SlabDefer sdefer[2];
  Scratch d_pre;
  Scratch adv2; int ld_adv2 = 0;
  struct Pitched { Scratch buf; const float* src = nullptr; int ld = 0, cols = 0; long rows = 0; uint64_t step = ~0ULL; };
  Pitched pitched[2];
  int opt_fused_dstack = getenv("GT_FUSED_DSTACK") ? atoi(getenv("GT_FUSED_DSTACK")) : 1;
  bool opt_split_first = env_flag("GT_D_SPLIT", true);
  bool opt_comm_d_one_msg = env_flag("GT_COMM_D_ONE_MSG", true), opt_comm_early_g = env_flag("GT_COMM_EARLY_G", true),
       opt_comm_force = getenv("GT_COMM_FORCE_COLLECTIVES") != nullptr;
  bool opt_comm_close_inline = env_flag("GT_COMM_CLOSE_INLINE", true);
  bool opt_comm_tv_in_sums = env_flag("GT_COMM_TV_IN_SUMS", true);
  bool d_unnorm = false, leak_unnorm = false;
  bool opt_poll_results = env_flag("GT_POLL_RESULTS", true);
  bool opt_launch_riders = env_flag("GT_LAUNCH_RIDERS", true);
  int ld_gx = 0, ld_cx = 0;
  Scratch gx_dense, cx_dense;
  bool gx_dense_on = false;
  const float* cxd_src = nullptr; uint64_t cxd_step = ~0ull; long cxd_rows = 0; int cxd_ld = 0, cxd_cols = 0;
  Scratch w0pad[2];
  unsigned int* h_fault_dev = nullptr;
  unsigned int* d_fault = nullptr;
  unsigned int* h_fault = nullptr;
  bool lstm_persistent = getenv("GT_LSTM_STEPS") == nullptr;
  int lstm_fwd_upc = 0;
  bool lstm_xcd_local = getenv("GT_LSTM_NO_XCD_LOCAL") == nullptr;
  int64_t lstm_paths[GT_LSTM_PATH_SLOTS] = {};
  bool matmul_bf16 = false;
  static constexpr int LEN_RING = 4;
  int* len_host[LEN_RING] = {nullptr, nullptr, nullptr, nullptr};
  Scratch len_dev[LEN_RING];
  hipEvent_t len_ev[LEN_RING] = {nullptr, nullptr, nullptr, nullptr};
  int len_cap = 0, len_slot = -1;
  int* d_lengths() { return len_slot < 0 ? nullptr : len_dev[len_slot].as<int>(); }
  std::vector<Scratch> s_wt;
  std::vector<Scratch> s_u, s_h, s_c, s_xdrop, s_xmask;
  Scratch s_du, s_dx, s_dbias;
  std::vector<Scratch> ds_wt, ds_u, ds_h, ds_c, ds_xdrop, ds_xmask, ds_omask;
  bool sru_d_bf16 = env_flag("GT_SRU_D_BF16", false);
  std::vector<B16Img> ds_in_b;
  B16Img ds_du_b;
  std::vector<LinShadow> dssh;
  std::vector<int> h_lengths;
  StepScalars* sc() { return scal.as<StepScalars>(); }
  StepResults* res() { return (StepResults*)((char*)scal.p + 256); }
};
static inline void invalidate_d_images(gt_engine* e) { e->img_cat.valid = e->img_cat_b.valid = e->img_adv2.valid = false; }

int check_common(gt_engine* e, int B, int T);
int fault_seen(gt_engine* e);
int optim_check_desc(const gt_optim_desc_ex* od);
void optim_desc_copy(const gt_optim_desc_ex* in, gt_optim_desc_ex* out);
int launch_optim_step(const gt_optim_desc_ex& od, long step, bool buf_live, OptimScalarCache* cache, float* params, float* grads, long n,
                      const double* part, int n_partial, double* norm2_out, const unsigned int* fault_dev, unsigned int* fault_host,
                      unsigned int* skipped_host, const float* gscale, hipStream_t s);
void optim_host_scalars(const gt_optim_desc_ex& od, long t, OptimScalarCache* cache, double out[2]);
gt::DropoutSpec philox_site_spec(gt_engine* e, int role, int pass, int layer, uint64_t step, float p, long half_rows = 0);
gt::DropoutSpec drop_spec(gt_engine* e, int role, int pass, int layer, const float* stacked_mask, int ld, long half_rows = 0);

extern thread_local int tl_gemm_prec;
enum { GEMM_PATH_PAIR = 576, GEMM_PATH_TN_PAIR = 580, GEMM_PATH_REDUCE4 = 582, GEMM_PATH_REDUCE = 583, GEMM_PATH_REDUCE_SMALL = 584,
       GEMM_PATH_COLSUM_PARTIAL = 585, GEMM_PATH_COLSUM_FINALIZE = 586, GEMM_PATH_REDUCE_MULTI = 587 };
static_assert(GEMM_PATH_REDUCE_MULTI + 1 == GT_GEMM_PATH_SLOTS, "gt_gemm_path_counts slots");
constexpr int gemm_path_slot(int kind, int bm, int bn, bool va, bool vb, int prec, int amode) {
  return (((((kind * 2 + (bm == 128)) * 2 + (bn == 128)) * 2 + va) * 2 + vb) * 2 + (prec == gt::PREC_BF16)) * 6 + (amode + 1);
}
void gemm_path_count(int slot);
bool gemm_vec_ok(const float* p, int ld, bool k_contiguous = false);
bool gemm_wide_store_ok(int kind, const gt::GemmArgs& g);
bool gemm_small_tiles_ok();
namespace gt { struct DStackArgs; }
bool dstack_hidden_ok(int hidden_dim);
int dstack_panels(long rows);
int launch_dstack(const gt::DStackArgs& a, int hidden_dim, hipStream_t s);
gt::DropoutSpec no_drop();
int launch_gemm(int kind, const gt::GemmArgs& g, int nslab, hipStream_t s);
int linear_forward(const float* X, int ldx, const float* W, int ldw, const float* b, float* Y, int ldy,
                   long rows, int in, int out, int act, const gt::DropoutSpec& drop, hipStream_t s);
gt::GemmArgs backward_data_args(const float* dZ, int lddz, const float* W, int ldw, int col0, float* dX, int lddx,
                                long rows, int out, int ncols, int act_prev, const float* H, int ldh, const gt::DropoutSpec& drop);
int linear_backward_data(const float* dZ, int lddz, const float* W, int ldw, int col0, float* dX, int lddx,
                         long rows, int out, int ncols, int act_prev, const float* H, int ldh, const gt::DropoutSpec& drop, hipStream_t s);
int slab_defer_flush(SlabDefer& d, hipStream_t s);
int linear_backward_weight(const float* dZ, int lddz, const float* X, int ldx, long rows, int out, int in,
                           float* dW, float* db, bool accumulate, Scratch& slabs, Scratch& colp, hipStream_t s,
                           SlabDefer* defer = nullptr, const gt::GemmArgs* ride_along = nullptr, bool* rode = nullptr);

int linear_backward_weight_split(const float* dZ, int lddz, long rows, long wrap, const float* xp, int ldxp, int cd,
                                 const float* adv, int ld_adv, int Da, int out, float* dW, float* db, bool accumulate,
                                 Scratch& slabs, hipStream_t s, SlabDefer* defer, const GemmArgs* rider = nullptr, bool* rode = nullptr);

gt::GemmB16Args b16_args();
enum { B16_PATH_CAST_F32 = 60, B16_PATH_CAST_BF16 = 61, B16_PATH_CAST_SEQDROP = 62, B16_PATH_CAST_MULTI = 63, B16_PATH_CAST_CAT = 64,
       B16_PATH_CAST_CATDROP = 65 };
static_assert(B16_PATH_CAST_CATDROP + 1 == GT_GEMM_B16_PATH_SLOTS, "gt_gemm_b16_path_counts slots");
constexpr int b16_path_slot(int epi, int amode, int form) { return (epi * 5 + amode) * 4 + form; }
void b16_path_count(int slot);
int launch_gemm_b16(const gt::GemmB16Args& g, int nslab, hipStream_t s, int tile = 0);
int cast_transpose(const float* in, int ld_in, long rows, int cols, __bf16* out, int ldo, __bf16* outT, long ldt,
                   float* colsum, bool colsum_accumulate, Scratch* colp, hipStream_t s);
int cast_transpose(const __bf16* in, int ld_in, long rows, int cols, __bf16* out, int ldo, __bf16* outT, long ldt,
                   float* colsum, bool colsum_accumulate, Scratch* colp, hipStream_t s);
int cast_jobs_add(gt::CastJobs& jobs, int& blocks, const float* in, int ldi, long rows, int cols, __bf16* out, int ldo, __bf16* outT, long ldt);
int cast_transpose_multi(const gt::CastJobs& jobs, int blocks, hipStream_t s);
int seqdrop_cast_transpose(const gt::SeqDropSrc& src, long rows, int cols, __bf16* out, int ldo, __bf16* outT, long ldt, hipStream_t s);
int cat_cast_transpose(const gt::CatSrc& src, long rows, int cols, __bf16* out, int ldo, __bf16* outT, long ldt, hipStream_t s);
int catdrop_cast_transpose(const gt::CatDropSrc& src, long rows, int cols, __bf16* out, int ldo, __bf16* outT, long ldt, hipStream_t s);
int weight_grad_b16(const __bf16* dZT, long lddzt, const __bf16* XT, long ldxt, long rows, int out, int in, float* dW, float* db,
                    bool accumulate, Scratch& slabs, hipStream_t s, SlabDefer* defer = nullptr);

int ensure_band(gt_engine* e, const float* R, int T, hipStream_t s);
int mlpg_forward(gt_engine* e, const float* y, int ldy, const int* scol, const int* sstride, int Ds,
                 float* ys, int ldys, int B, int T, hipStream_t s);
int mlpg_backward(gt_engine* e, const float* gs, int ldgs, const int* scol, const int* sstride, int Ds,
                  float* gy, int ldgy, int B, int T, float mse_w, const float* yhat, const float* ytgt, int ldt,
                  const float* mask, hipStream_t s);
int post_early_results(gt_engine* e, hipStream_t s, unsigned ticket = 0);
int cond_dim(gt_engine* e);

struct GtComm {
  void* comm = nullptr;
  int rank = 0, world = 1;
  hipStream_t stream = nullptr;
  hipEvent_t ev[8] = {nullptr, nullptr, nullptr, nullptr, nullptr, nullptr, nullptr, nullptr};
  int next_ev = 0;
  hipEvent_t ev_done = nullptr;
  struct TraceRec { int kind, inl; double bytes; hipEvent_t e0, e1; bool closed; };
  bool trace = false;
  long trace_dropped = 0;
  std::vector<TraceRec> trec;
};
bool comm_on(const gt_engine* e);
int comm_grads_ready(gt_engine* e, int role, const float* lo, long count, hipStream_t compute);
int comm_flush(gt_engine* e, int role, hipStream_t compute, bool closing = false);
int comm_tv_sent(gt_engine* e, hipStream_t s);
void ipc_destroy(gt_engine* e);
bool ipc_usable(const gt_engine* e, size_t bytes);
int ipc_allreduce(gt_engine* e, void* buf, size_t count, bool dtype_double, hipStream_t s);
int comm_tv_join(gt_engine* e, hipStream_t s);
int comm_finish_step(gt_engine* e, int role, bool grads, double* sums, int n_sums, hipStream_t compute);
int comm_early_results(gt_engine* e, int role, double* sums, int n_sums, float adv_w, float mse_w, float mge_w, hipStream_t compute);
int ensure_tv_begin(gt_engine* e, const float* mask, long N, hipStream_t s);
int ensure_tv(gt_engine* e, const float* mask, long N, hipStream_t s);

int lstm_forward(gt_engine* e, const float* x, int B, int T, float* y_hat, hipStream_t s);
int lstm_check_lengths(gt_engine* e, int B, int T);
int lstm_stack_forward(gt_engine* e, int role, const float* x, int ld_x, int nseq, int T, const int* passes, int npass, hipStream_t s,
                       const float** top, int* ld_top);
int lstm_stack_backward(gt_engine* e, int role, const float* x, int ld_x, int nseq, int T, const int* passes, int npass, bool want_w,
                        float* dx0, hipStream_t s);
int lstm_backward(gt_engine* e, const float* x, const float* gy, int B, int T, hipStream_t s);
int sru_forward(gt_engine* e, const float* x, int B, int T, float* y_hat, hipStream_t s);
int sru_backward(gt_engine* e, const float* x, const float* gy, int B, int T, hipStream_t s);
int sru_stack_forward(gt_engine* e, int role, const float* x, int ld_x, int nseq, int T, const int* passes, int npass, hipStream_t s,
                      const float** top, int* ld_top, const gt::CatSrc* cat0 = nullptr, bool want_w = true);
bool sru_b16(const gt_engine* e, int role);
enum { SRU_PATH_FWD = 0, SRU_PATH_FWD_CS = 1, SRU_PATH_BWD = 5, SRU_PATH_BWD_CS = 6, SRU_PATH_INPUT_MASK = 10, SRU_PATH_INPUT_DROPOUT = 11,
       SRU_PATH_DX_ADV_FINISH = 12 };
static_assert(SRU_PATH_DX_ADV_FINISH + 1 == GT_SRU_PATH_SLOTS, "gt_sru_path_counts slots");
int sru_scan_waves(long B, int ncols);
uint32_t sru_drop_thresh(float p);
int sru_launch_fwd(const gt::SruArgs& a, hipStream_t s);
int sru_launch_bwd(const gt::SruArgs& a, hipStream_t s);
int sru_launch_input_mask(float* mul, int B, int n, float keep_scale, uint32_t thresh, uint32_t key0, uint32_t key1, const float* inj,
                          int seq_mul, int seq_add, hipStream_t s);
int sru_launch_input_dropout(const float* x, int ldx, float* y, int ldy, int B, int T, int n, const float* mul, hipStream_t s);
int sru_launch_dx_adv_finish(const gt::SruDxAdvArgs& f, hipStream_t s);
bool sru_d_needs_f32_input(const gt_engine* e);
int sru_stack_backward(gt_engine* e, int role, const float* x, int ld_x, int nseq, int T, const int* passes, int npass, bool want_w,
                       float* dx_adv, hipStream_t s);
```

### gantts_amd/csrc/frame_kernels.hip.h

```cpp
#pragma once
#include <hip/hip_runtime.h>
#include <stdint.h>
#include "gemm_f32.hip.h"

namespace gt {

constexpr int RED_THREADS = 256;

__device__ __forceinline__ float wave_sum(float v) {
#pragma unroll
  for (int o = 32; o > 0; o >>= 1) v += __shfl_xor(v, o, 64);
  return v;
}
__device__ __forceinline__ double wave_sum_d(double v) {
#pragma unroll
  for (int o = 32; o > 0; o >>= 1) v += __shfl_xor(v, o, 64);
  return v;
}
__device__ __forceinline__ float block_sum(float v, float* sh) {
  v = wave_sum(v);
  const int lane = threadIdx.x & 63, w = threadIdx.x >> 6;
  __syncthreads();
  if (lane == 0) sh[w] = v;
  __syncthreads();
// ... 171 lines not shown
                                        const float* __restrict__ tv_mask, int tv_n, float tv_override, StepScalars* sc,
                                        double* __restrict__ tv_total ) {
  if (tv_mask && blockIdx.x == gridDim.x - 1) {
    __shared__ double sh[16];
    if (tv_total) {
      const double tot = mask_total_body(tv_mask, tv_n, sh);
      if (threadIdx.x == 0) tv_total[0] = tot;
    } else mask_sum_body(tv_mask, tv_n, tv_override, nullptr, sc, sh);
    return;
  }
  __shared__ int sidx[256];
  const bool map_lds = na <= 256;
  if (map_lds) {
    for (int k = threadIdx.x; k < na; k += blockDim.x) sidx[k] = idx[k];
    __syncthreads();
  }
  const long e4 = (long)blockIdx.x * blockDim.x + threadIdx.x;
  const int g4 = ldo >> 2;
  if (e4 >= rows * g4) return;
  const long r = e4 / g4;
  const int c = (int)(e4 - r * g4) * 4;
  const float* src = r < split ? fa + r * ldf : fb + (r - split) * ldf;
  int ix[4];
#pragma unroll
  for (int k = 0; k < 4; ++k) ix[k] = map_lds ? sidx[min(c + k, na - 1)] : idx[min(c + k, na - 1)];
  f32x4 v;
#pragma unroll
  for (int k = 0; k < 4; ++k) v[k] = src[ix[k]];
#pragma unroll
  for (int k = 0; k < 4; ++k) v[k] = c + k < na ? v[k] : 0.f;
  *reinterpret_cast<f32x4*>(out + r * ldo + c) = v;
}
static __global__ void repitch_kernel(const float* __restrict__ in, int ld_in, int cols, long rows, float* __restrict__ out, int ldo) {
  const long i = (long)blockIdx.x * blockDim.x + threadIdx.x;
  const int g4 = ldo >> 2;
  if (i >= rows * g4) return;
  const long r = i / g4;
  const int c = (int)(i - r * g4) * 4;
  const float* src = in + r * ld_in + c;
  f32x4 v;
#pragma unroll
  for (int k = 0; k < 4; ++k) v[k] = c + k < cols ? src[k] : 0.f;
  *reinterpret_cast<f32x4*>(out + r * ldo + c) = v;
}
static __global__ void pad_rows_kernel(const float* __restrict__ in, int cols, int rows, float* __restrict__ out, int ldo) {
  const long i = (long)blockIdx.x * blockDim.x + threadIdx.x;
  if (i >= (long)rows * ldo) return;
  const int r = (int)(i / ldo), c = (int)(i - (long)r * ldo);
  out[i] = c < cols ? in[(long)r * cols + c] : 0.f;
}

static __global__ void mlpg_offset_max_kernel(const float* __restrict__ R, int T, int nW, float* __restrict__ offmax) {
  const int o = blockIdx.x - (T - 1);
  __shared__ float sh[16];
  float mx = 0.f;
  for (int i = threadIdx.x; i < T * nW; i += blockDim.x) {
    const int w = i / T, t = i - w * T;
    const int tt = t + o;
    if (tt >= 0 && tt < T) mx = fmaxf(mx, fabsf(R[(long)t * nW * T + (long)w * T + tt]));
  }
#pragma unroll
  for (int s = 32; s > 0; s >>= 1) mx = fmaxf(mx, __shfl_xor(mx, s, 64));
  const int lane = threadIdx.x & 63, wv = threadIdx.x >> 6;
  if (lane == 0) sh[wv] = mx;
  __syncthreads();
  if (threadIdx.x == 0) {
    for (int i = 1; i < (int)(blockDim.x >> 6); ++i) mx = fmaxf(mx, sh[i]);
    offmax[blockIdx.x] = mx;
  }
}

static __global__ void mlpg_extract_band_kernel(const float* __restrict__ R, int T, int nW, int kb, float* __restrict__ band) {
  const int nb = 2 * kb + 1;
  const int i = blockIdx.x * blockDim.x + threadIdx.x;
  if (i >= T * nW * nb) return;
  const int j = i % nb, w = (i / nb) % nW, t = i / (nb * nW);
  const int tt = t + j - kb;
  band[i] = (tt >= 0 && tt < T) ? R[(long)t * nW * T + (long)w * T + tt] : 0.f;
}

constexpr int MLPG_TT = 32;
constexpr int MLPG_CC = 64;

constexpr int MLPG_PAD = 3;
constexpr int MLPG_MAXW = 4;
constexpr int MLPG_THREADS = 1024;

template <int FPL, int TT = MLPG_TT>
__global__ __launch_bounds__(MLPG_THREADS) void mlpg_forward_kernel(
    const float* __restrict__ y, int ldy, const float* __restrict__ band, int kb, int nW,
    const int* __restrict__ scol, const int* __restrict__ sstride, int Ds,
    float* __restrict__ ys, int ldys, int B, int T) {
  extern __shared__ __attribute__((aligned(16))) float sm[];
  const int nb = 2 * kb + 1, nbp = nb + 2 * MLPG_PAD;
  const int tiles_t = (T + TT - 1) / TT;
  const int b = blockIdx.x / tiles_t, t0 = (blockIdx.x % tiles_t) * TT;
  const int c0 = blockIdx.y * MLPG_CC;
  const int nc = min(MLPG_CC, Ds - c0);
  const int rows = TT + 2 * kb;
  float* sb = sm + rows * nW * MLPG_CC;
  const float* yb = y + (long)b * T * ldy;
  const int lane = threadIdx.x & 63, wv = threadIdx.x >> 6, nwv = MLPG_THREADS / 64;
  float vb0[8];
  {
    const long src_rows = (long)T * nW;
    const int jc = min(max(lane - MLPG_PAD, 0), nb - 1);
#pragma unroll
    for (int q = 0; q < 8; ++q) vb0[q] = band[min((long)t0 * nW + wv + q * nwv, src_rows - 1) * nb + jc];
  }
  {
    const bool c_ok = lane < nc;
    const int my_col = c_ok ? scol[c0 + lane] : 0, my_st = c_ok ? sstride[c0 + lane] : 0;
    const int nrw = rows * nW;
    const int dr = nwv / nW, dw = nwv % nW;
    int r = wv / nW, w = wv % nW;
    for (int rw0 = wv; rw0 < nrw; rw0 += 8 * nwv) {
      float v[8];
#pragma unroll
      for (int q = 0; q < 8; ++q) {
        const int t = t0 - kb + r;
        const int tc = min(max(t, 0), T - 1);
        const float x = yb[(long)tc * ldy + my_col + (my_st > 0 ? w * my_st : 0)];
        v[q] = (c_ok && t >= 0 && t < T && (my_st > 0 || w == 0)) ? x : 0.f;
        r += dr; w += dw;
        if (w >= nW) { w -= nW; ++r; }
      }
#pragma unroll
      for (int q = 0; q < 8; ++q) {
        const int rw = rw0 + q * nwv;
        if (rw < nrw) sm[rw * MLPG_CC + lane] = v[q];
      }
    }
  }
  {
    const int nrow = TT * nW;
    const long src_rows = (long)T * nW;
    if (lane < nbp) {
      const int j = lane - MLPG_PAD;
      const bool j_ok = j >= 0 && j < nb;
#pragma unroll
      for (int q = 0; q < 8; ++q) {
        const int tw = wv + q * nwv;
        if (tw < nrow) sb[tw * nbp + lane] = (j_ok && (long)t0 * nW + tw < src_rows) ? vb0[q] : 0.f;
      }
    }
    for (int jp = lane; jp < nbp; jp += 64) {
      const int j = jp - MLPG_PAD;
      const bool j_ok = j >= 0 && j < nb;
      const int jc = min(max(j, 0), nb - 1);
      for (int tw0 = jp == lane ? wv + 8 * nwv : wv; tw0 < nrow; tw0 += 8 * nwv) {
        float v[8];
#pragma unroll
        for (int q = 0; q < 8; ++q) {
          const long row = (long)t0 * nW + tw0 + q * nwv;
          const float x = band[min(row, src_rows - 1) * nb + jc];
          v[q] = (j_ok && row < src_rows) ? x : 0.f;
        }
#pragma unroll
        for (int q = 0; q < 8; ++q) {
          const int tw = tw0 + q * nwv;
          if (tw < nrow) sb[tw * nbp + jp] = v[q];
        }
      }
    }
  }
  __syncthreads();
  static_assert(FPL >= 1 && FPL <= MLPG_PAD + 1, "the band rows are padded for at most MLPG_PAD + 1 frames per lane");
  if (threadIdx.x >= TT * 32 / FPL) return;
  const int cp = threadIdx.x & 31, fg = threadIdx.x >> 5;
  const int tl0 = fg * FPL;
  float acc[FPL][2];
#pragma unroll
  for (int i = 0; i < FPL; ++i) acc[i][0] = acc[i][1] = 0.f;
  const int ntap = (FPL - 1) + nb;
  for (int w = 0; w < nW; ++w) {
    const float* dcol = sm + (tl0 * nW + w) * MLPG_CC + 2 * cp;
    const float* cf = sb + (tl0 * nW + w) * nbp + MLPG_PAD;
#pragma unroll 8
    for (int j0 = 0; j0 < ntap; ++j0) {
      const float2 d = *reinterpret_cast<const float2*>(dcol + j0 * nW * MLPG_CC);
#pragma unroll
      for (int i = 0; i < FPL; ++i) {
        const float cfi = cf[i * nW * nbp + j0 - i];
        acc[i][0] = fmaf(cfi, d.x, acc[i][0]);
        acc[i][1] = fmaf(cfi, d.y, acc[i][1]);
      }
    }
  }
#pragma unroll
  for (int q = 0; q < 2; ++q) {
    const int c = 2 * cp + q;
    if (c >= nc) continue;
    const bool pass = sstride[c0 + c] == 0;
#pragma unroll
    for (int i = 0; i < FPL; ++i) {
      const int t = t0 + tl0 + i;
      if (t >= T) continue;
      const float out = pass ? sm[((tl0 + i + kb) * nW + 0) * MLPG_CC + c] : acc[i][q];
      ys[((long)b * T + t) * ldys + c0 + c] = out;
    }
  }
}

template <int FPL, int TT = MLPG_TT>
__global__ __launch_bounds__(MLPG_THREADS) __attribute__((amdgpu_waves_per_eu(FPL <= 2 ? 8 : 4)))
void mlpg_backward_kernel(
    const float* __restrict__ gs, int ldgs, const float* __restrict__ band, int kb, int nW,
    const int* __restrict__ scol, const int* __restrict__ sstride, int Ds,
    float* __restrict__ gy, int ldgy, int B, int T,
    float mse_w, const float* __restrict__ yhat, const float* __restrict__ ytgt, int ldt,
    const float* __restrict__ mask, const StepScalars* __restrict__ sc) {
  extern __shared__ __attribute__((aligned(16))) float sm[];
  const int nb = 2 * kb + 1, nbp = nb + 2 * MLPG_PAD;
  const int tiles_t = (T + TT - 1) / TT;
  const int b = blockIdx.x / tiles_t, t0 = (blockIdx.x % tiles_t) * TT;
  const int c0 = blockIdx.y * MLPG_CC;
  const int nc = min(MLPG_CC, Ds - c0);
  const int rows = TT + 2 * kb;
  float* sb = sm + rows * MLPG_CC;
  const float* gb = gs + (long)b * T * ldgs;
  const int lane = threadIdx.x & 63, wv = threadIdx.x >> 6, nwv = MLPG_THREADS / 64;
  float vb0[16];
  {
    const long src_rows = (long)T * nW, base = (long)(t0 - kb) * nW;
    const int jc = min(max(lane - MLPG_PAD, 0), nb - 1);
#pragma unroll
    for (int q = 0; q < 16; ++q) vb0[q] = band[min(max(base + wv + q * nwv, 0L), src_rows - 1) * nb + jc];
  }
  {
    const bool c_ok = lane < nc;
    const int ccl = c_ok ? c0 + lane : c0;
    for (int r0 = wv; r0 < rows; r0 += 8 * nwv) {
      float v[8];
#pragma unroll
      for (int q = 0; q < 8; ++q) {
        const int t = t0 - kb + r0 + q * nwv;
        const int tc = min(max(t, 0), T - 1);
        const float x = gb[(long)tc * ldgs + ccl];
        v[q] = (c_ok && t >= 0 && t < T) ? x : 0.f;
      }
#pragma unroll
      for (int q = 0; q < 8; ++q) {
        const int r = r0 + q * nwv;
        if (r < rows) sm[r * MLPG_CC + lane] = v[q];
      }
    }
  }
  {
    const int nrow = rows * nW;
    const long src_rows = (long)T * nW, base = (long)(t0 - kb) * nW;
    if (lane < nbp) {
      const int j = lane - MLPG_PAD;
      const bool j_ok = j >= 0 && j < nb;
#pragma unroll
      for (int q = 0; q < 16; ++q) {
        const int rw = wv + q * nwv;
        const long row = base + rw;
        if (rw < nrow) sb[rw * nbp + lane] = (j_ok && row >= 0 && row < src_rows) ? vb0[q] : 0.f;
      }
    }
    for (int jp = lane; jp < nbp; jp += 64) {
      const int j = jp - MLPG_PAD;
      const bool j_ok = j >= 0 && j < nb;
      const int jc = min(max(j, 0), nb - 1);
      for (int rw0 = jp == lane ? wv + 16 * nwv : wv; rw0 < nrow; rw0 += 8 * nwv) {
        float v[8];
#pragma unroll
        for (int q = 0; q < 8; ++q) {
          const long row = base + rw0 + q * nwv;
          const float x = band[min(max(row, 0L), src_rows - 1) * nb + jc];
          v[q] = (j_ok && row >= 0 && row < src_rows) ? x : 0.f;
        }
#pragma unroll
        for (int q = 0; q < 8; ++q) {
          const int rw = rw0 + q * nwv;
          if (rw < nrow) sb[rw * nbp + jp] = v[q];
        }
      }
    }
  }
  __syncthreads();
  static_assert(FPL >= 1 && FPL <= MLPG_PAD + 1, "the band rows are padded for at most MLPG_PAD + 1 frames per lane");
  if (threadIdx.x >= TT * 32 / FPL) return;
  const int cp = threadIdx.x & 31, fg = threadIdx.x >> 5;
  const int tl0 = fg * FPL;
  float acc[MLPG_MAXW][FPL][2];
#pragma unroll
  for (int w = 0; w < MLPG_MAXW; ++w)
#pragma unroll
    for (int i = 0; i < FPL; ++i) acc[w][i][0] = acc[w][i][1] = 0.f;
  const int ntap = (FPL - 1) + nb;
  const float* drow = sm + tl0 * MLPG_CC + 2 * cp;
  const float* cfrow = sb + (long)tl0 * nW * nbp + MLPG_PAD + (nb - 1);
#pragma unroll 4
  for (int j0 = 0; j0 < ntap; ++j0) {
    const float2 d = *reinterpret_cast<const float2*>(drow + j0 * MLPG_CC);
    const float* cf = cfrow + (long)j0 * nW * nbp - j0;
#pragma unroll
    for (int w = 0; w < MLPG_MAXW; ++w) {
      if (w >= nW) break;
#pragma unroll
      for (int i = 0; i < FPL; ++i) {
        const float cfi = cf[w * nbp + i];
        acc[w][i][0] = fmaf(cfi, d.x, acc[w][i][0]);
        acc[w][i][1] = fmaf(cfi, d.y, acc[w][i][1]);
      }
    }
  }
  const float msk_scale = mse_w != 0.f ? 2.f * mse_w * sc->inv_tv : 0.f;
#pragma unroll
  for (int q = 0; q < 2; ++q) {
    const int c = 2 * cp + q;
    if (c >= nc) continue;
    const int col0 = scol[c0 + c], st = sstride[c0 + c];
#pragma unroll
    for (int i = 0; i < FPL; ++i) {
      const int tp = t0 + tl0 + i;
      if (tp >= T) continue;
      const long row = (long)b * T + tp;
      const float m = msk_scale != 0.f ? mask[row] : 0.f;
#pragma unroll
      for (int w = 0; w < MLPG_MAXW; ++w) {
        if (w >= nW || (st == 0 && w > 0)) break;
        float out = st == 0 ? sm[(tl0 + i + kb) * MLPG_CC + c] : acc[w][i][q];
        const int col = col0 + w * st;
        if (msk_scale != 0.f) out += msk_scale * (yhat[row * ldt + col] * m - ytgt[row * ldt + col] * m) * m;
        gy[row * ldgy + col] = out;
      }
    }
  }
}

__device__ __forceinline__ double masked_sqerr_body(
    const float* __restrict__ a, int lda, const float* __restrict__ b, int ldb,
    const float* __restrict__ mask, long rows, int D, float* __restrict__ g, int ldg, float gs, int blk, int nblk) {
  double acc = 0.0;
  const long total = rows * D;
  const long stride = (long)nblk * blockDim.x;
  const long sr = stride / D;
  const int sd = (int)(stride - sr * D);
  long e = (long)blk * blockDim.x + threadIdx.x;
  long r = e / D;
  int d = (int)(e - r * D);
  for (; e < total; e += 4 * stride) {
    long rr[4];
    int dd[4];
    bool ok[4];
#pragma unroll
    for (int u = 0; u < 4; ++u) {
      rr[u] = r; dd[u] = d; ok[u] = e + u * stride < total;
      r += sr; d += sd;
      if (d >= D) { d -= D; ++r; }
    }
    float m[4], av[4], bv[4];
#pragma unroll
    for (int u = 0; u < 4; ++u) {
      m[u] = ok[u] ? mask[rr[u]] : 0.f; av[u] = ok[u] ? a[rr[u] * lda + dd[u]] : 0.f; bv[u] = ok[u] ? b[rr[u] * ldb + dd[u]] : 0.f;
    }
#pragma unroll
    for (int u = 0; u < 4; ++u) {
      if (!ok[u]) continue;
      const float diff = av[u] * m[u] - bv[u] * m[u];
      acc += (double)diff * (double)diff;
      if (g) g[rr[u] * ldg + dd[u]] = gs * diff * m[u];
    }
  }
  return acc;
}
static __global__ __launch_bounds__(RED_THREADS) void masked_sqerr_kernel(
    const float* __restrict__ a, int lda, const float* __restrict__ b, int ldb,
    const float* __restrict__ mask, long rows, int D, double* __restrict__ partial,
    float* __restrict__ g, int ldg, float gscale, const StepScalars* __restrict__ sc) {
  __shared__ double sh[16];
  const float gs = g ? 2.f * gscale * sc->inv_tv : 0.f;
  const double acc = masked_sqerr_body(a, lda, b, ldb, mask, rows, D, g, ldg, gs, blockIdx.x, gridDim.x);
  const double tot = block_sum_d(acc, sh);
  if (threadIdx.x == 0) partial[blockIdx.x] = tot;
}
static __global__ __launch_bounds__(RED_THREADS) void g_losses_kernel(
    const float* __restrict__ a1, int lda1, const float* __restrict__ b1, int ldb1, int D1, int n1, double* __restrict__ partial1,
    const float* __restrict__ a2, int lda2, const float* __restrict__ b2, int ldb2, int D2, double* __restrict__ partial2,
    const float* __restrict__ mask, long rows) {
  __shared__ double sh[16];
  const bool first = (int)blockIdx.x < n1;
  const int blk = first ? blockIdx.x : blockIdx.x - n1, nblk = first ? n1 : gridDim.x - n1;
  const double acc = first ? masked_sqerr_body(a1, lda1, b1, ldb1, mask, rows, D1, nullptr, 0, 0.f, blk, nblk)
                           : masked_sqerr_body(a2, lda2, b2, ldb2, mask, rows, D2, nullptr, 0, 0.f, blk, nblk);
  const double tot = block_sum_d(acc, sh);
  if (threadIdx.x == 0) (first ? partial1 : partial2)[blk] = tot;
}

enum HeadMode { HEAD_D_STEP = 0, HEAD_G_ADV = 1 };

struct HeadPartials {
  double s_real, s_fake, n_real_ok, n_fake_ok, db;
};

template <int KP, typename TH = float, bool B16OUT = false, bool VEC = false>
__global__ __launch_bounds__(256) void d_head_kernel(
    const TH* __restrict__ H, int ldh, int K, const float* __restrict__ w, const float* __restrict__ bias,
    const float* __restrict__ mask, int n_mask, int n_real, int n_rows, int mode, float eps,
    float* __restrict__ Dout, float* __restrict__ dH, int lddh, int want_grad, DropoutSpec drop,
    int has_act, const StepScalars* __restrict__ sc,
    HeadPartials* __restrict__ hp, float* __restrict__ dw_partial ,
    __bf16* __restrict__ dHb = nullptr, int lddhb = 0,
    __bf16* __restrict__ dHbT = nullptr, long lddhbt = 0,
    const double* __restrict__ tv_dev = nullptr,
    int unit_tv = 0) {
  extern __shared__ __attribute__((aligned(16))) float smf[];
  __shared__ double shd[5][4];
  const int lane = threadIdx.x & 63, wv = threadIdx.x >> 6;
  const float inv_tv = unit_tv ? 1.0f : tv_dev ? 1.0f / (float)*tv_dev : sc->inv_tv;
  if (tv_dev && blockIdx.x == 0 && threadIdx.x == 0) {
// ... 159 lines not shown
  }
  if (want_grad && dw_partial) {
    for (int k = threadIdx.x; k < K; k += blockDim.x)
      dw_partial[(long)blockIdx.x * K + k] = (smf[k] + smf[K + k]) + (smf[2 * K + k] + smf[3 * K + k]);
  }
}

static __global__ __launch_bounds__(1024) void d_head_finalize_kernel(const HeadPartials* __restrict__ hp, const float* __restrict__ dw_partial,
                                                               int nblk, int K, int mode, StepScalars* sc,
                                                               float* __restrict__ dw, float* __restrict__ db, int accumulate,
                                                               StepResults* early_res ,
                                                               unsigned* ticket = nullptr, unsigned ticket_value = 0,
                                                               int cgw = 64 ,
                                                               int scal_blk = 0 ) {
  __shared__ float shw[1024];
  __shared__ double shd[16];
  const int nparts = (int)blockDim.x / cgw;
  const int kl = threadIdx.x % cgw, part = threadIdx.x / cgw;
  const int k = blockIdx.x * cgw + kl;
  if (dw) {
    float sa[16];
#pragma unroll
    for (int u = 0; u < 16; ++u) sa[u] = 0.f;
    if (k < K) {
      int i = part;
      for (; i + 15 * nparts < nblk; i += 16 * nparts) {
#pragma unroll
        for (int u = 0; u < 16; ++u) sa[u] += dw_partial[(long)(i + nparts * u) * K + k];
      }
      for (; i < nblk; i += nparts) sa[0] += dw_partial[(long)i * K + k];
    }
#pragma unroll
    for (int u = 0; u < 8; ++u) sa[u] += sa[u + 8];
#pragma unroll
    for (int u = 0; u < 4; ++u) sa[u] += sa[u + 4];
    shw[part * cgw + kl] = (sa[0] + sa[1]) + (sa[2] + sa[3]);
    __syncthreads();
    if (part == 0 && k < K) {
      float tot = 0.f;
      for (int q = 0; q < nparts; ++q) tot += shw[q * cgw + kl];
      dw[k] = accumulate ? dw[k] + tot : tot;
    }
  }
  if ((int)blockIdx.x == scal_blk) {
    double v[5] = {0, 0, 0, 0, 0};
    for (int i = threadIdx.x; i < nblk; i += blockDim.x) {
      v[0] += hp[i].s_real; v[1] += hp[i].s_fake; v[2] += hp[i].n_real_ok; v[3] += hp[i].n_fake_ok; v[4] += hp[i].db;
    }
    double r[5];
    for (int q = 0; q < 5; ++q) r[q] = block_sum_d(v[q], shd);
    if (threadIdx.x == 0) {
      if (mode == HEAD_D_STEP) {
        sc->s_real = r[0]; sc->s_fake = r[1]; sc->n_real_ok = r[2]; sc->n_fake_ok = r[3];
        if (early_res) {
          const float T = sc->tv;
          const float lr = -((float)r[0]) / T, lf = -((float)r[1]) / T;
          early_res->loss_real_d = lr; early_res->loss_fake_d = lf; early_res->loss_d = lr + lf;
          early_res->real_correct = (float)r[2]; early_res->fake_correct = (float)r[3];
          early_res->gnorm_d = 0.f; early_res->tv = T;
          publish_ticket(ticket, ticket_value);
        }
      } else sc->s_adv = r[0];
      if (db) db[0] = accumulate ? db[0] + (float)r[4] : (float)r[4];
    }
  }
}


struct GFinalize {
  int on;
  StepScalars* sc;
  StepResults* out;
  float adv_w, mse_w, mge_w;
  int has_adv;
  const double* part_mge; int n_mge;
  const double* part_mse; int n_mse;
  const HeadPartials* hp; int n_hp;
  unsigned* ticket; unsigned ticket_value;
};
__device__ __forceinline__ void finalize_g_body(StepScalars* sc, StepResults* out, float adv_w, float mse_w, float mge_w, int has_adv,
                                                int zero_gnorm, const double* __restrict__ part_mge, int n_mge,
                                                const double* __restrict__ part_mse, int n_mse,
                                                const HeadPartials* __restrict__ hp, int n_hp, double* shp ,
                                                unsigned* ticket = nullptr, unsigned ticket_value = 0) {
  if (part_mge || part_mse || hp) {
    if (part_mge) {
      double v = 0.0;
      for (int i = threadIdx.x; i < n_mge; i += blockDim.x) v += __builtin_nontemporal_load(part_mge + i);
      const double t = block_sum_d(v, shp);
      if (threadIdx.x == 0) sc->s_mge = t;
    }
    if (part_mse) {
      double v = 0.0;
      for (int i = threadIdx.x; i < n_mse; i += blockDim.x) v += __builtin_nontemporal_load(part_mse + i);
      const double t = block_sum_d(v, shp);
      if (threadIdx.x == 0) sc->s_mse = t;
    }
    if (hp) {
      double v = 0.0;
      for (int i = threadIdx.x; i < n_hp; i += blockDim.x) v += hp[i].s_real;
      const double t = block_sum_d(v, shp);
      if (threadIdx.x == 0) sc->s_adv = t;
    }
    __syncthreads();
  }
  if (threadIdx.x || !out) return;
  const float T = sc->tv;
  const float mse = (float)sc->s_mse / T, mge = (float)sc->s_mge / T;
  const float adv = has_adv ? -((float)sc->s_adv) / T : 0.f;
  out->loss_mse = mse; out->loss_mge = mge; out->loss_adv = adv;
  out->loss_g = (mse_w * mse + mge_w * mge) + adv_w * adv;
  out->gnorm_g = zero_gnorm ? 0.f : (float)sqrt(sc->gnorm2_g); out->tv = T;
  publish_ticket(ticket, ticket_value);
}

static __global__ __launch_bounds__(RED_THREADS) void static_grad_kernel(
    const float* __restrict__ yhs, int ld1, const float* __restrict__ ys, int ld2,
    const float* __restrict__ mask, long rows, int Ds, float mge_w,
    const int* __restrict__ adv_inv , const float* __restrict__ leak, int ldl,
    const float* __restrict__ gadv, int lda, float adv_w,
    float* __restrict__ gs, int ldg, double* __restrict__ partial, StepScalars* __restrict__ sc, const GFinalize fin,
    int leak_unnorm ) {
  __shared__ double sh[16];
  int nblk = gridDim.x;
  const int blk = blockIdx.x;
  if (fin.on) {
    if (blockIdx.x == gridDim.x - 1) {
      finalize_g_body(fin.sc, fin.out, fin.adv_w, fin.mse_w, fin.mge_w, fin.has_adv, 1, fin.part_mge, fin.n_mge, fin.part_mse, fin.n_mse,
                      fin.hp, fin.n_hp, sh, fin.ticket, fin.ticket_value);
      return;
    }
    --nblk;
  }
  double acc = 0.0;
  const long total = rows * Ds;
  const float sc2 = 2.f * mge_w * sc->inv_tv;
  const float leak_s = leak_unnorm ? sc->inv_tv : 1.f;
  const long stride = (long)nblk * blockDim.x;
  const long sr = stride / Ds;
  const int sd = (int)(stride - sr * Ds);
  long e = (long)blk * blockDim.x + threadIdx.x;
  long r = e / Ds;
  int c = (int)(e - r * Ds);
  for (; e + 3 * stride < total; e += 4 * stride) {
    long rr[4];
    int cc[4];
#pragma unroll
    for (int u = 0; u < 4; ++u) {
      if (c >= Ds) { c -= Ds; ++r; }
      rr[u] = r; cc[u] = c;
      r += sr; c += sd;
    }
    float m[4], yv[4], tv[4], lk[4], ga[4];
    int jj[4];
#pragma unroll
    for (int u = 0; u < 4; ++u) {
      m[u] = mask[rr[u]]; yv[u] = yhs[rr[u] * ld1 + cc[u]]; tv[u] = ys[rr[u] * ld2 + cc[u]];
      jj[u] = (gs && adv_inv) ? adv_inv[cc[u]] : -1;
    }
#pragma unroll
    for (int u = 0; u < 4; ++u) {
      lk[u] = (jj[u] >= 0 && leak) ? leak[rr[u] * ldl + jj[u]] : 0.f;
      ga[u] = (jj[u] >= 0 && gadv) ? gadv[rr[u] * lda + jj[u]] : 0.f;
    }
#pragma unroll
    for (int u = 0; u < 4; ++u) {
      const float diff = yv[u] * m[u] - tv[u] * m[u];
      if (partial) acc += (double)diff * (double)diff;
      if (gs) {
        float v = sc2 * diff * m[u];
        if (jj[u] >= 0) {
          if (leak) v += leak_s * lk[u];
          if (gadv) v += adv_w * ga[u];
        }
        gs[rr[u] * ldg + cc[u]] = v;
      }
    }
  }
  for (; e < total; e += stride, r += sr, c += sd) {
    if (c >= Ds) { c -= Ds; ++r; }
    const float m = mask[r];
    const float diff = yhs[r * ld1 + c] * m - ys[r * ld2 + c] * m;
    if (partial) acc += (double)diff * (double)diff;
    if (gs) {
      float v = sc2 * diff * m;
      const int j = adv_inv ? adv_inv[c] : -1;
      if (j >= 0) {
        if (leak) v += leak_s * leak[r * ldl + j];
        if (gadv) v += adv_w * gadv[r * lda + j];
      }
      gs[r * ldg + c] = v;
    }
  }
  if (partial) {
    const double tot = block_sum_d(acc, sh);
    if (threadIdx.x == 0) partial[blk] = tot;
  }
}

static __global__ __launch_bounds__(RED_THREADS) void finalize_g_rider_kernel(const GFinalize fin) {
  __shared__ double sh[16];
  finalize_g_body(fin.sc, fin.out, fin.adv_w, fin.mse_w, fin.mge_w, fin.has_adv, 1, fin.part_mge, fin.n_mge, fin.part_mse, fin.n_mse,
                  fin.hp, fin.n_hp, sh, fin.ticket, fin.ticket_value);
}

static __global__ void scale_by_inv_tv_kernel(float* __restrict__ g, long n, const StepScalars* __restrict__ sc) {
  const long i = (long)blockIdx.x * blockDim.x + threadIdx.x;
  if (i < n) g[i] *= sc->inv_tv;
}

static __global__ __launch_bounds__(256) void sum_partials_kernel(const double* __restrict__ partial, int n, double* __restrict__ out) {
  __shared__ double sh[16];
  double v = 0.0;
  for (int i = threadIdx.x; i < n; i += blockDim.x) v += partial[i];
  const double tot = block_sum_d(v, sh);
  if (threadIdx.x == 0) *out = tot;
}

static __global__ __launch_bounds__(256) void colsum_partial_kernel(const float* __restrict__ X, int ldx, long rows, int cols,
                                                             int rows_per_blk, float* __restrict__ partial) {
  __shared__ float sh[4][64];
  const int cl = threadIdx.x & 63, rl = threadIdx.x >> 6;
  const int c = blockIdx.y * 64 + cl;
  const long r0 = (long)blockIdx.x * rows_per_blk;
  const long r1 = min(rows, r0 + rows_per_blk);
  float s = 0.f;
  if (c < cols) for (long r = r0 + rl; r < r1; r += 4) s += X[r * ldx + c];
  sh[rl][cl] = s;
  __syncthreads();
  if (rl == 0 && c < cols) partial[(long)blockIdx.x * cols + c] = (sh[0][cl] + sh[1][cl]) + (sh[2][cl] + sh[3][cl]);
}
static __global__ void colsum_finalize_kernel(const float* __restrict__ partial, int nblk, int cols, float* __restrict__ out, int accumulate) {
  const int c = blockIdx.x * blockDim.x + threadIdx.x;
  if (c >= cols) return;
  float s = 0.f;
  for (int i = 0; i < nblk; ++i) s += partial[(long)i * cols + c];
  out[c] = accumulate ? out[c] + s : s;
}

__device__ __forceinline__ void slab_reduce4_body(int blk, const float* __restrict__ slabs, long slab_stride, int nslab, long n4,
                                                  float* __restrict__ out, int accumulate,
                                                  const float* __restrict__ bslabs, int nb, float* __restrict__ bout, int main_blocks) {
  if (blk >= main_blocks) {
    const int c = (blk - main_blocks) * blockDim.x + threadIdx.x;
    if (c >= nb) return;
    float s0 = 0.f, s1 = 0.f, s2 = 0.f, s3 = 0.f;
    int k = 0;
    for (; k + 4 <= nslab; k += 4) {
      s0 += bslabs[(long)k * nb + c];       s1 += bslabs[(long)(k + 1) * nb + c];
      s2 += bslabs[(long)(k + 2) * nb + c]; s3 += bslabs[(long)(k + 3) * nb + c];
    }
    for (; k < nslab; ++k) s0 += bslabs[(long)k * nb + c];
    const float tot = (s0 + s1) + (s2 + s3);
    bout[c] = accumulate ? bout[c] + tot : tot;
    return;
  }
  const long i = (long)blk * blockDim.x + threadIdx.x;
  if (i >= n4) return;
  const f32x4* p = reinterpret_cast<const f32x4*>(slabs) + i;
  const long st4 = slab_stride / 4;
  f32x4 s = {0.f, 0.f, 0.f, 0.f};
  int k = 0;
  for (; k + 8 <= nslab; k += 8) {
    f32x4 v[8];
#pragma unroll
    for (int q = 0; q < 8; ++q) v[q] = p[(long)(k + q) * st4];
#pragma unroll
    for (int q = 0; q < 8; ++q) s += v[q];
  }
  for (; k < nslab; ++k) s += p[(long)k * st4];
  f32x4* o = reinterpret_cast<f32x4*>(out) + i;
  if (accumulate) s += *o;
  *o = s;
}
constexpr int SLAB_MAX_JOBS = 8;
struct SlabJob {
  const float* slabs; long slab_stride; long n4; float* out;
  const float* bslabs; float* bout;
  int nslab, accumulate, nb, main_blocks, block0, pad_;
};
struct SlabJobs { int n, pad_; SlabJob j[SLAB_MAX_JOBS]; };
static __global__ __launch_bounds__(256) void slab_reduce_multi_kernel(const SlabJobs jobs) {
  int q = 0;
  while (q + 1 < jobs.n && (int)blockIdx.x >= jobs.j[q + 1].block0) ++q;
  const SlabJob& J = jobs.j[q];
  slab_reduce4_body((int)blockIdx.x - J.block0, J.slabs, J.slab_stride, J.nslab, J.n4, J.out, J.accumulate, J.bslabs, J.nb, J.bout, J.main_blocks);
// ... 510 lines not shown
```

### gantts_amd/engine.py

```python
import ctypes as C
import weakref

import numpy as np
import torch

from . import _lib as L
from ._lib import check, lib, ptr


def stream_config_from_hp(hp):
    cfg = L.StreamConfig()
    ss = list(hp.stream_sizes)
    hd = list(hp.has_dynamic_features) if hp.has_dynamic_features is not None else [False] * len(ss)
    if len(ss) > L.MAX_STREAMS:
        raise ValueError("at most %d streams are supported" % L.MAX_STREAMS)
    cfg.n_streams = len(ss)
    for i, (s, d) in enumerate(zip(ss, hd)):
        cfg.stream_sizes[i] = int(s)
        cfg.has_dynamic_features[i] = int(bool(d))
    cfg.num_windows = len(hp.windows)
    adv = getattr(hp, "adversarial_streams", None)
    if adv is None:
        cfg.adversarial_streams[0] = -1
    else:
# ... 125 lines not shown
    def comm_destroy(self):
        check(lib.gt_comm_destroy(self._h))

    def comm_ipc_export(self):
        buf = (C.c_char * L.IPC_HANDLE_BYTES)()
        check(lib.gt_comm_ipc_export(self._h, buf))
        return bytes(buf.raw)

    def comm_ipc_attach(self, rank, world, handles):
        if len(handles) != world * L.IPC_HANDLE_BYTES:
            raise ValueError("handles must be world * %d bytes" % L.IPC_HANDLE_BYTES)
        buf = (C.c_char * len(handles)).from_buffer_copy(handles)
        check(lib.gt_comm_ipc_attach(self._h, int(rank), int(world), buf))

    def comm_ipc_messages(self):
        n = C.c_longlong()
        check(lib.gt_comm_ipc_messages(self._h, C.byref(n)))
        return n.value

    def set_shard(self, rank, world):
        check(lib.gt_set_shard(self._h, int(rank), int(world)))
        self._dp_world = int(world)

    def comm_trace(self, enable):
        check(lib.gt_comm_trace(self._h, 1 if enable else 0))

    def comm_trace_read(self):
        import numpy as np
        n = C.c_int()
        check(lib.gt_comm_trace_read(self._h, None, 0, C.byref(n)))
        out = np.zeros((max(n.value, 1), 5), dtype=np.float64)
        check(lib.gt_comm_trace_read(self._h, out.ctypes.data_as(C.POINTER(C.c_double)), n.value, C.byref(n)))
        return out[:n.value]

    def comm_info(self):
        r, w = C.c_int(), C.c_int()
        check(lib.gt_comm_info(self._h, C.byref(r), C.byref(w)))
        return r.value, w.value

    def check_faults(self):
        check(lib.gt_check_faults(self._h, L.current_stream()))

    def lstm_path_counts(self, reset=False):
        out = (C.c_int64 * L.LSTM_PATH_SLOTS)()
        check(lib.gt_lstm_path_counts(self._h, out, 1 if reset else 0))
        return list(out)

    def clear_faults(self):
        check(lib.gt_clear_faults(self._h, L.current_stream()))

    def invalidate_mlpg_cache(self):
        check(lib.gt_invalidate_mlpg_cache(self._h))

    def optimizer_step_count(self, role):
        n = C.c_int64()
        check(lib.gt_get_optimizer_step(self._h, role, C.byref(n)))
        return n.value

    def optimizer_scalars(self, role):
        out = (C.c_double * 2)()
        check(lib.gt_get_optimizer_scalars(self._h, role, out))
        return out[0], out[1]

    def zero_grad(self, role):
        check(lib.gt_zero_grad(self._h, role))

    def set_seed(self, seed):
        check(lib.gt_set_seed(self._h, C.c_uint64(int(seed))))

    def philox_mask(self, role, pass_index, layer, p, rows, cols, steps_ahead=1):
        m = torch.empty(rows, cols, device="cuda", dtype=torch.float32)
        check(lib.gt_op_philox_mask(self._h, role, pass_index, layer, int(steps_ahead), float(p), int(rows), int(cols),
                                    ptr(m), L.current_stream()))
        return m

    def set_option(self, name, value):
        opts = {"lstm_persistent": L.OPT_LSTM_PERSISTENT,
                "lstm_fwd_units": L.OPT_LSTM_FWD_UNITS, "lstm_xcd_local": L.OPT_LSTM_XCD_LOCAL,
                "matmul_bf16": L.OPT_MATMUL_BF16, "split_first_layer": L.OPT_SPLIT_FIRST_LAYER,
                "comm_d_one_msg": L.OPT_COMM_D_ONE_MSG, "comm_early_g": L.OPT_COMM_EARLY_G,
                "comm_force": L.OPT_COMM_FORCE, "launch_riders": L.OPT_LAUNCH_RIDERS,
                "comm_close_inline": L.OPT_COMM_CLOSE_INLINE, "poll_results": L.OPT_POLL_RESULTS,
                "comm_tv_in_sums": L.OPT_COMM_TV_IN_SUMS, "comm_ipc": L.OPT_COMM_IPC, "fused_dstack": L.OPT_FUSED_DSTACK,
                "sru_d_bf16": L.OPT_SRU_D_BF16}
        if name not in opts:
            raise ValueError("unknown engine option %r" % (name,))
        check(lib.gt_set_option(self._h, opts[name], int(value)))
        if name == "matmul_bf16":
            self._opt_bf16 = bool(value)

    def set_loss_normalizer(self, tv):
        if isinstance(tv, torch.Tensor) and tv.is_cuda:
            if tv.dtype != torch.float64 or tv.numel() != 1:
                raise ValueError("device loss normaliser must be a 1-element float64 tensor")
            self._keep["tv"] = tv
            check(lib.gt_set_loss_normalizer_device(self._h, ptr(tv)))
        else:
            self._keep.pop("tv", None)
            check(lib.gt_set_loss_normalizer(self._h, float(tv)))

    def set_lengths(self, lengths, B, T):
        if lengths is None:
            vals = [T] * B
        elif isinstance(lengths, torch.Tensor):
            vals = [int(v) for v in lengths.detach().cpu().view(-1).tolist()]
        else:
            vals = [int(v) for v in lengths]
        if len(vals) != B:
            raise RuntimeError("lengths has %d entries for a batch of %d sequences" % (len(vals), B))
        arr = (C.c_int64 * B)(*vals)
        check(lib.gt_set_lengths(self._h, arr, B, L.current_stream()))

    def apply_generator(self, model_g, x, R, lengths=None):
        x, ld = _check_x(x, "x", model_g.in_dim)
        self._set_pitch(gx=ld)
        B, T, _ = x.shape
        model_g._check_masks(B, T)
        self.bind_model(L.ROLE_G, model_g, with_grads=True)
        if getattr(model_g, "needs_lengths", False):
            self.set_lengths(lengths, B, T)
        static_w = model_g.static_dim if model_g.include_parameter_generation() else self.static_dim
        y_hat = torch.empty(B, T, model_g.out_dim, device=x.device, dtype=torch.float32)
        y_hat_static = torch.empty(B, T, static_w, device=x.device, dtype=torch.float32)
        if R is not None:
            R = _check_frames(R, "R")
            if R.dim() != 2 or R.size(0) != T or R.size(1) != self.num_windows * T:
                raise RuntimeError("R must be (T, num_windows*T) = (%d, %d), got %s" % (T, self.num_windows * T, tuple(R.shape)))
        check(lib.gt_apply_generator(self._h, ptr(x), ptr(R), B, T, ptr(y_hat), ptr(y_hat_static), L.current_stream()))
        self._keep["g"] = (x, R, y_hat, y_hat_static)
        y_hat._gt_engine = y_hat_static._gt_engine = self
        return y_hat, y_hat_static

    def _set_pitch(self, gx=None, cx=None):
        if gx is not None:
            self._ld_gx = gx
        if cx is not None:
            self._ld_cx = cx
        if (self._ld_gx, self._ld_cx) != self._pitch_sent:
            check(lib.gt_set_x_pitch(self._h, self._ld_gx, self._ld_cx))
            self._pitch_sent = (self._ld_gx, self._ld_cx)

    def _cond_x(self, x, model_d):
        x, ld = _check_x(x, "x", model_d.in_dim - self._adv_width())
        self._set_pitch(cx=ld)
        return x

    def _mask2d(self, mask, B, T):
        mask = _check_frames(mask, "mask")
        if mask.numel() != B * T:
            raise RuntimeError("mask must have B*T = %d elements, got %s" % (B * T, tuple(mask.shape)))
        return mask

    def _d_lengths(self, model_d, lengths, B, T):
        if getattr(model_d, "needs_lengths", False):
            self.set_lengths(lengths, B, T)

    def update_discriminator(self, model_d, optimizer_d, x, y_static, y_hat_static, mask, phase, eps=1e-20, lengths=None):
        y_static = _check_frames(y_static, "y_static")
        y_hat_static_c = _same_storage(y_hat_static, _check_frames(y_hat_static, "y_hat_static", y_static.size(-1)), "y_hat_static")
        B, T, _ = y_static.shape
        mask = self._mask2d(mask, B, T)
        train = phase == "train"
        model_d._check_masks(B, T)
        self._d_lengths(model_d, lengths, B, T)
        self.bind_model(L.ROLE_D, model_d, with_grads=True)
        if train:
            self.bind_optimizer(L.ROLE_D, optimizer_d)
# ... 65 lines not shown
        check(lib.gt_update_discriminator_end(self._h, int(train), None if defer else C.byref(res), L.current_stream()))
        if train:
            optimizer_d._note_step(self, L.ROLE_D)
        if defer:
            return None
        return res.loss_d, res.loss_fake_d, res.loss_real_d, res.real_correct_count, res.fake_correct_count

    def update_discriminator_result(self):
        res = L.DResult()
        check(lib.gt_update_discriminator_result(self._h, C.byref(res)))
        return res.loss_d, res.loss_fake_d, res.loss_real_d, res.real_correct_count, res.fake_correct_count

    def update_generator_begin(self, model_g, model_d, optimizer_g, x, y, y_hat, y_static, y_hat_static,
                               adv_w, mask, phase, mse_w, mge_w, eps=1e-20, lengths=None):
        y = _check_frames(y, "y", model_g.out_dim)
        y_hat_c = _check_frames(y_hat, "y_hat", model_g.out_dim)
        y_static = _check_frames(y_static, "y_static")
        y_hat_static_c = _same_storage(y_hat_static, _check_frames(y_hat_static, "y_hat_static", y_static.size(-1)), "y_hat_static")
        B, T, _ = y.shape
        mask = self._mask2d(mask, B, T)
        train = phase == "train"
        self.bind_model(L.ROLE_G, model_g, with_grads=True)
        if train:
            self.bind_optimizer(L.ROLE_G, optimizer_g)
        if adv_w > 0:
            model_d._check_masks(B, T)
            self._d_lengths(model_d, lengths, B, T)
            self.bind_model(L.ROLE_D, model_d, with_grads=False)
            x = self._cond_x(x, model_d) if self.signature[5] else None
        else:
            x = None
        check(lib.gt_update_generator_begin(self._h, ptr(x), ptr(y), ptr(y_hat_c), ptr(y_static), ptr(y_hat_static_c),
                                            float(adv_w), ptr(mask), B, T, int(train), float(mse_w), float(mge_w),
                                            float(eps), L.current_stream()))

    def update_generator_end(self, optimizer_g, adv_w, mse_w, mge_w, phase, defer=False):
        train = phase == "train"
        res = L.GResult()
        check(lib.gt_update_generator_end(self._h, int(train), float(adv_w), float(mse_w), float(mge_w),
                                          None if defer else C.byref(res), L.current_stream()))
        if train:
            optimizer_g._note_step(self, L.ROLE_G)
        if defer:
            return None
        return res.loss_mse, res.loss_mge, res.loss_adv, res.loss_g

    def update_generator_result(self):
        res = L.GResult()
        check(lib.gt_update_generator_result(self._h, C.byref(res)))
        return res.loss_mse, res.loss_mge, res.loss_adv, res.loss_g

    def _adv_width(self):
        ss, hd, nW, adv, nmask, _ = self.signature
        static = [s // nW if d else s for s, d in zip(ss, hd)]
        if adv is None:
            return sum(static)
        return sum(s for s, a in zip(static, adv) if a) - (nmask if nmask > 0 else 0)

    def flush_generator_grads(self):
        check(lib.gt_flush_generator_grads(self._h, L.current_stream()))

    def model_forward(self, model, x, R=None, lengths=None):
        squeeze = x.dim() == 2
        if squeeze:
            x = x.unsqueeze(0)
        x = _check_frames(x, "x", model.in_dim)
        B, T, _ = x.shape
        model._check_masks(B, T)
        self.bind_model(L.ROLE_G, model, with_grads=False)
        if getattr(model, "needs_lengths", False):
            self.set_lengths(lengths, B, T)
        out = torch.empty(B, T, model.out_dim, device=x.device, dtype=torch.float32)
        out2 = None
        if model.include_parameter_generation():
            if R is None:
                raise RuntimeError("In2OutHighwayNet.forward needs R")
            R = _check_frames(R, "R")
            out2 = torch.empty(B, T, model.static_dim, device=x.device, dtype=torch.float32)
        check(lib.gt_model_forward(self._h, L.ROLE_G, ptr(x), ptr(R), B, T, ptr(out), ptr(out2), L.current_stream()))
        if out2 is not None:
            return out, out2
        return out.squeeze(0) if squeeze else out

    def mlpg_forward(self, y, R):
        y = _check_frames(y, "inputs")
        R = _check_frames(R, "R")
        B, T, _ = y.shape
        out = torch.empty(B, T, self.static_dim, device=y.device, dtype=torch.float32)
        check(lib.gt_op_mlpg_forward(self._h, ptr(y), ptr(R), B, T, ptr(out), L.current_stream()))
        return out

    def mlpg_backward(self, g_static, R, full_dim):
        g = _check_frames(g_static, "grad")
        R = _check_frames(R, "R")
        B, T, _ = g.shape
        out = torch.empty(B, T, full_dim, device=g.device, dtype=torch.float32)
        check(lib.gt_op_mlpg_backward(self._h, ptr(g), ptr(R), B, T, ptr(out), L.current_stream()))
        return out


_engines_by_sig = {}


def engine_for(hp, model_g=None):
    sig = _hp_signature(hp)
    if model_g is not None:
        eng = getattr(model_g, "_step_engine", None)
        if eng is None or eng.signature != sig:
            eng = StepEngine(hp)
            model_g._step_engine = eng
        return eng
    eng = _engines_by_sig.get(sig)
    if eng is None:
        eng = _engines_by_sig[sig] = StepEngine(hp)
    return eng


class HipStepBackend(object):

    def __init__(self, hp, model_g, model_d, optimizer_g, optimizer_d):
        self.hp, self.mg, self.md, self.og, self.od = hp, model_g, model_d, optimizer_g, optimizer_d
        self.engine = engine_for(hp, model_g)
        self._out = None

    def mask_of(self, batch):
        return batch["mask"]

    def philox_mask(self, role, pass_index, layer, p, rows, cols, steps_ahead=1):
        return self.engine.philox_mask(role, pass_index, layer, p, rows, cols, steps_ahead)

    def set_option(self, name, value):
        self.engine.set_option(name, value)

    def set_shard(self, rank, world):
        self.engine.set_shard(rank, world)

    device_normalizer = True

    def set_loss_normalizer(self, tv):
        self.engine.set_loss_normalizer(tv)

    def zero_grad(self):
        self.og.zero_grad()
        self.od.zero_grad()

    def flat_grads(self, which):
        return (self.mg if which == "G" else self.md).flat_grads()

    def scalar_sums(self, which):
        return self.engine.scalar_sums(which)

    def apply_generator(self, batch):
        self._out = self.engine.apply_generator(self.mg, batch.get("g_in", batch["x"]), batch.get("R"), batch.get("lengths"))
        return self._out

    def update_discriminator_begin(self, batch, phase):
        self.engine.update_discriminator_begin(self.md, self.od, batch["x"], batch["y_static"], self._out[1],
                                               batch["mask"], phase)

    deferred_results = True

    def update_discriminator_end(self, batch, phase, defer=False):
        return self.engine.update_discriminator_end(self.od, phase, defer=defer)

    def update_discriminator_result(self):
        return self.engine.update_discriminator_result()
# ... 11 lines not shown
```

### include/gantts_hip.h

```cpp
#ifndef GANTTS_HIP_H_
#define GANTTS_HIP_H_

#include <stdint.h>

#ifdef __cplusplus
extern "C" {
#endif

#define GT_OK 0
#define GT_ERR_INVALID 1
#define GT_ERR_HIP 2
#define GT_ERR_STATE 3
#define GT_ERR_DIM 4

#define GT_ROLE_G 0
#define GT_ROLE_D 1

#define GT_ARCH_MLP 0
#define GT_ARCH_IN2OUT 1
#define GT_ARCH_LSTM 2
#define GT_ARCH_SRU 3
#define GT_ARCH_IN2OUT_RNN 4

#define GT_OPT_ADAGRAD 0
// ... 58 lines not shown
  int32_t kind;
  uint32_t flags;
  double lr, weight_decay, eps;
  double lr_decay;
  double beta1, beta2;
  double momentum;
  double dampening;
  double alpha;
  float max_grad_norm;
  int32_t reserved_;
  int64_t step;
  float* state0;
  float* state1;
  float* state2;
  double momentum_decay;
  double etaminus, etaplus;
  double step_size_min, step_size_max;
  double lambd, t0;
  double host_state0;
  double host_state1;
} gt_optim_desc_ex;

typedef struct {
  float loss_d, loss_fake_d, loss_real_d, real_correct_count, fake_correct_count;
  float grad_norm;
} gt_d_result;

typedef struct {
  float loss_mse, loss_mge, loss_adv, loss_g;
  float grad_norm;
} gt_g_result;

const char* gt_last_error(void);
const char* gt_version(void);
int gt_engine_create(const gt_stream_config* cfg, gt_engine** out);
void gt_engine_destroy(gt_engine* e);

int gt_bind_model(gt_engine* e, int role, const gt_model_desc* desc);
int gt_bind_optimizer(gt_engine* e, int role, const gt_optim_desc* desc);
int gt_bind_optimizer_ex(gt_engine* e, int role, const gt_optim_desc_ex* desc);
int gt_set_training(gt_engine* e, int role, int training);
int gt_set_lr(gt_engine* e, int role, float lr);
int gt_get_optimizer_step(gt_engine* e, int role, int64_t* step);
int gt_get_optimizer_scalars(gt_engine* e, int role, double out[2]);
int gt_set_seed(gt_engine* e, uint64_t seed);
int gt_set_dropout_mask(gt_engine* e, int role, int pass, int layer, const float* mask);
int gt_op_philox_mask(gt_engine* e, int role, int pass, int layer, int64_t steps_ahead, float p, int64_t rows, int cols,
                      float* mask, void* stream);

int gt_set_lengths(gt_engine* e, const int64_t* lengths_host, int B, void* stream);
int gt_invalidate_mlpg_cache(gt_engine* e);

int gt_zero_grad(gt_engine* e, int role);

int gt_apply_generator(gt_engine* e, const float* x, const float* R, int B, int T,
                       float* y_hat, float* y_hat_static, void* stream);

int gt_update_discriminator(gt_engine* e, const float* x, const float* y_static, const float* y_hat_static,
                            const float* mask, int B, int T, int train, float eps,
                            gt_d_result* out, void* stream);

int gt_update_generator(gt_engine* e, const float* x, const float* y, const float* y_hat,
                        const float* y_static, const float* y_hat_static, float adv_w,
                        const float* mask, int B, int T, int train, float mse_w, float mge_w, float eps,
                        gt_g_result* out, void* stream);

int gt_set_loss_normalizer(gt_engine* e, float tv_global);
int gt_set_loss_normalizer_device(gt_engine* e, const double* tv_global_dev);
#define GT_OPT_LSTM_PERSISTENT 2
#define GT_OPT_LSTM_FWD_UNITS 3
#define GT_OPT_LSTM_XCD_LOCAL 4
#define GT_OPT_MATMUL_BF16 5
#define GT_OPT_SPLIT_FIRST_LAYER 6
#define GT_OPT_COMM_D_ONE_MSG 10
#define GT_OPT_COMM_EARLY_G 11
#define GT_OPT_COMM_FORCE 13
#define GT_OPT_LAUNCH_RIDERS 14
#define GT_OPT_COMM_CLOSE_INLINE 15
#define GT_OPT_POLL_RESULTS 16
#define GT_OPT_COMM_TV_IN_SUMS 17
#define GT_OPT_COMM_IPC 18
#define GT_OPT_FUSED_DSTACK 19
#define GT_OPT_SRU_D_BF16 20
int gt_set_option(gt_engine* e, int option, int value);
int gt_set_tuning(const char* name, int value);
int gt_set_x_pitch(gt_engine* e, int ld_generator_input, int ld_condition);
int gt_check_faults(gt_engine* e, void* stream);
#define GT_LSTM_PATH_SLOTS 34
int gt_lstm_path_counts(gt_engine* e, int64_t* counts, int reset);
int gt_clear_faults(gt_engine* e, void* stream);
#define GT_COMM_ID_BYTES 128
int gt_comm_unique_id(void* id_out);
int gt_comm_init(gt_engine* e, int rank, int world, const void* id);
int gt_comm_destroy(gt_engine* e);
int gt_comm_info(gt_engine* e, int* rank, int* world);
int gt_comm_trace(gt_engine* e, int enable);
int gt_comm_trace_read(gt_engine* e, double* out, int max_records, int* n_records);
#define GT_IPC_HANDLE_BYTES 64
#define GT_IPC_MAX_WORLD 8
int gt_comm_ipc_export(gt_engine* e, void* handle_out);
int gt_comm_ipc_attach(gt_engine* e, int rank, int world, const void* handles);
int gt_comm_ipc_messages(gt_engine* e, long long* n);
int gt_set_shard(gt_engine* e, int rank, int world);

int gt_update_discriminator_begin(gt_engine* e, const float* x, const float* y_static, const float* y_hat_static,
                                  const float* mask, int B, int T, int train, float eps, void* stream);
int gt_update_discriminator_end(gt_engine* e, int train, gt_d_result* out, void* stream);
int gt_update_generator_begin(gt_engine* e, const float* x, const float* y, const float* y_hat,
                              const float* y_static, const float* y_hat_static, float adv_w,
                              const float* mask, int B, int T, int train, float mse_w, float mge_w, float eps,
                              void* stream);
int gt_update_generator_end(gt_engine* e, int train, float adv_w, float mse_w, float mge_w,
                            gt_g_result* out, void* stream);
int gt_update_discriminator_result(gt_engine* e, gt_d_result* out);
int gt_update_generator_result(gt_engine* e, gt_g_result* out);
int gt_scalar_buffer(gt_engine* e, double** dev_ptr, int* n_doubles);

int gt_model_forward(gt_engine* e, int role, const float* x, const float* R, int B, int T,
                     float* out, float* out2, void* stream);

int gt_flush_generator_grads(gt_engine* e, void* stream);

int gt_op_sequence_mask(const int64_t* lengths, int B, int T, float* mask, void* stream);
int gt_op_masked_mse(const float* input, const float* target, const float* mask, int B, int T, int D,
                     float* loss_out, float* grad_input, void* stream);
int gt_op_optim_step(const gt_optim_desc_ex* desc, float* params, float* grads, int64_t n, const float* gscale,
                     float* grad_norm_out, void* stream);
int gt_op_optim_scalars(const gt_optim_desc_ex* desc, int64_t t, double out[2]);
int gt_op_pad_sequences(const float* ragged, int D, const int64_t* start, const int64_t* len, int B, int T, float* out, int ld_out,
                        void* stream);
int gt_op_gather_cols(const float* in, int ld_in, const int32_t* idx, int n_idx, float* out, int ld_out,
                      int out_col_offset, int64_t rows, void* stream);
typedef struct gt_distortion_sums {
  double s_mcd;
  double s_bap;
  double s_f0;
  double n_voiced;
  double n_vuv_err;
  double s_mse;
  double n_frames;
} gt_distortion_sums;
int gt_compute_distortions(const float* y_static, const float* y_hat_static, int Ds, const void* stat_mean,
                           const void* stat_std, int stats_f64, const int32_t* col_stat_host,
                           const int32_t* col_role_host, int vuv_col, const int64_t* lengths_host, int B, int T,
                           gt_distortion_sums* out, void* stream);
int gt_op_mlpg_forward(gt_engine* e, const float* y, const float* R, int B, int T, float* y_static, void* stream);
int gt_op_mlpg_backward(gt_engine* e, const float* g_static, const float* R, int B, int T, float* g_y, void* stream);
int gt_op_linear_forward(const float* X, int ldx, const float* W, const float* bias, float* Y, int ldy,
                         int64_t rows, int in_dim, int out_dim, int act, const float* keep_mask, float p,
                         void* stream);
int gt_op_linear_backward(const float* dY, int lddy, const float* X, int ldx, const float* W,
                          int64_t rows, int in_dim, int out_dim,
                          float* dX, int lddx, const float* H_prev, int act_prev, const float* keep_mask_prev, float p_prev,
                          float* dW, float* db, void* stream);

int gt_op_linear_bf16(const float* X, const float* W, const float* bias, int64_t rows, int in_dim, int out_dim, int act,
                      const float* keep_mask, float p, float* Y, const float* dY, const float* H_prev, int act_prev,
                      const float* keep_mask_prev, float p_prev, float* dX, float* dW, float* db,
                      float* Y_image, float* YT_image, void* stream);

#define GT_GEMM_ROUTE_FORWARD 0
#define GT_GEMM_ROUTE_FORWARD_SEG 1
#define GT_GEMM_ROUTE_BACKWARD_DATA 2
#define GT_GEMM_ROUTE_WEIGHT_GRAD 3
#define GT_GEMM_ROUTE_WEIGHT_GRAD_SPLIT 4
typedef struct gt_gemm_case {
  int32_t route, prec;
  int32_t rows, in_dim, out_dim;
  int32_t act, drop;
  float p;
  uint32_t key0, key1;
  int32_t accumulate;
  int32_t col0, ncols;
  int32_t wrap, cd;
  int32_t rider, defer;
  int32_t ldx, ldw, ldy, ld_dy, ldh, ld_mask, ld_addm, ld_adv, ld_dx;
  const float* x;
  const float* w;
  const float* bias;
  float* y;
  const float* dy;
  const float* h;
  const float* mask;
  const float* addm;
  const float* adv;
  float* dx;
  float* dw;
  float* db;
} gt_gemm_case;
int gt_op_gemm_f32(const gt_gemm_case* c, void* stream);
#define GT_GEMM_PATH_SLOTS 588
int gt_gemm_path_counts(int64_t* counts, int reset);

#define GT_GEMM_B16_PATH_SLOTS 66
int gt_gemm_b16_path_counts(int64_t* counts, int reset);

typedef struct gt_gemm_b16_case {
  int32_t route;
  int32_t rows, in_dim, out_dim;
  int32_t act, drop;
  float p;
  uint32_t key0, key1;
  int32_t accumulate;
  int32_t ldx, ldw, ld_dy, ldh, ld_mask, ldc, ldcb, ldcbt;
  const float* x;
  const float* w;
  const float* bias;
  const float* dy;
  const float* h;
  const float* mask;
  float* c;
  uint16_t* cb;
  uint16_t* cbt;
  float* dw;
  float* db;
} gt_gemm_b16_case;
int gt_op_gemm_b16(const gt_gemm_b16_case* c, void* stream);

#define GT_CAST_PLAIN_F32 0
#define GT_CAST_PLAIN_BF16 1
#define GT_CAST_SEQDROP 2
#define GT_CAST_CAT 3
#define GT_CAST_CATDROP 4
#define GT_CAST_MULTI 5
#define GT_CAST_MAX_JOBS 8
typedef struct gt_cast_job {
  const float* in;
  uint16_t* out;
  uint16_t* outT;
  int64_t rows, ldt;
// ... 67 lines not shown
```

Measured before the change: 12.84 million frames/s.

## Fold static gradient into MLPG backward kernel and rework MLPG wave mapping

Adds a fused MLPG backward kernel that computes the static-feature gradient (MGE plus adversarial terms) inline instead of first writing it to a separate buffer with static_grad_kernel. The generator finalisation rider rides as an extra block of the fused kernel. The change also rewrites the MLPG forward and backward kernels to use one wave per few output frames, a workgroup size that varies with the tile, and no padded band copy in LDS; reads now go straight from the global band. This removes one kernel launch and an N×Ds round trip through global memory, at the cost of recomputing the static gradient for each window tap and a larger set of template variants.

Result: no change. 12.73 million frames/s (-0.8%).

```diff
diff --git a/gantts_amd/_lib.py b/gantts_amd/_lib.py
--- a/gantts_amd/_lib.py
+++ b/gantts_amd/_lib.py
@@ -13,6 +13,7 @@
 OPT_LAUNCH_RIDERS, OPT_COMM_CLOSE_INLINE, OPT_POLL_RESULTS = 14, 15, 16
 OPT_COMM_TV_IN_SUMS, OPT_COMM_IPC, OPT_FUSED_DSTACK = 17, 18, 19
 OPT_SRU_D_BF16 = 20
+OPT_STATIC_FOLD = 21
 IPC_HANDLE_BYTES, IPC_MAX_WORLD = 64, 8
 PROFILE_SLOTS = 16
 LSTM_PATH_SLOTS, LSTM_PATH_STEPS, LSTM_PATH_DECLINED = 34, 32, 33
@@ -192,6 +193,8 @@
     "gt_op_pad_sequences": (_I, [_P, _I, _P, _P, _I, _I, _P, _I, _P]),
     "gt_op_mlpg_forward": (_I, [_P, _P, _P, _I, _I, _P, _P]),
     "gt_op_mlpg_backward": (_I, [_P, _P, _P, _I, _I, _P, _P]),
+    "gt_static_grad_path_counts": (_I, [C.POINTER(_L)]),
+    "gt_op_peek_gy": (_I, [_P, _P, _L, _I, _P]),
     "gt_op_linear_forward": (_I, [_P, _I, _P, _P, _P, _I, _L, _I, _I, _I, _P, _F, _P]),
     "gt_op_linear_bf16": (_I, [_P, _P, _P, _L, _I, _I, _I, _P, _F, _P, _P, _P, _I, _P, _F, _P, _P, _P, _P, _P, _P]),
     "gt_profile_enable": (_I, [_I]),
diff --git a/gantts_amd/csrc/eng_core.hip b/gantts_amd/csrc/eng_core.hip
--- a/gantts_amd/csrc/eng_core.hip
+++ b/gantts_amd/csrc/eng_core.hip
@@ -387,6 +387,7 @@
     case GT_OPT_COMM_TV_IN_SUMS: e->opt_comm_tv_in_sums = value != 0; return GT_OK;
     case GT_OPT_POLL_RESULTS: e->opt_poll_results = value != 0; return GT_OK;
     case GT_OPT_LAUNCH_RIDERS: e->opt_launch_riders = value != 0; return GT_OK;
+    case GT_OPT_STATIC_FOLD: e->opt_static_fold = value != 0; return GT_OK;
     case GT_OPT_MATMUL_BF16:
       if (e->matmul_bf16 != (value != 0)) {
         invalidate_d_images(e);
diff --git a/gantts_amd/csrc/eng_ops.hip b/gantts_amd/csrc/eng_ops.hip
--- a/gantts_amd/csrc/eng_ops.hip
+++ b/gantts_amd/csrc/eng_ops.hip
@@ -105,6 +105,13 @@
   hipStream_t s = (hipStream_t)stream;
   CHK(ensure_band(e, R, T, s));
   return mlpg_forward(e, y, e->Dout_cfg, e->d_scol, e->d_sstride, e->Ds, y_static, e->Ds, B, T, s);
+}
+extern "C" int gt_op_peek_gy(gt_engine* e, float* out, int64_t rows, int cols, void* stream) {
+  if (!e || !out) return fail(GT_ERR_INVALID, "null argument");
+  if (!e->gy.p || e->gy_ld < cols || cols < 1 || rows < 1 || rows > e->N) return fail(GT_ERR_STATE, "no generator backward of that shape has run");
+  HIPCHK(hipMemcpy2DAsync(out, (size_t)cols * sizeof(float), e->gy.p, (size_t)e->gy_ld * sizeof(float), (size_t)cols * sizeof(float), (size_t)rows,
+                          hipMemcpyDeviceToDevice, (hipStream_t)stream));
+  return GT_OK;
 }
 extern "C" int gt_op_mlpg_backward(gt_engine* e, const float* g_static, const float* R, int B, int T, float* g_y, void* stream) {
   CHK(check_common(e, B, T));
diff --git a/gantts_amd/csrc/eng_step.hip b/gantts_amd/csrc/eng_step.hip
--- a/gantts_amd/csrc/eng_step.hip
+++ b/gantts_amd/csrc/eng_step.hip
@@ -49,37 +49,63 @@
   return GT_OK;
 }
 
+static std::atomic<long long> g_static_grad_paths[2];
+extern "C" int gt_static_grad_path_counts(int64_t out[2]) {
+  if (!out) return fail(GT_ERR_INVALID, "null argument");
+  out[0] = g_static_grad_paths[0].load(); out[1] = g_static_grad_paths[1].load();
+  return GT_OK;
+}
 static int mlpg_tile_frames() { return gt_tuning().mlpg_tt == 16 ? 16 : 32; }
+static int mlpg_frames_per_wave(int dflt, int tt) { const int f = gt_tuning().mlpg_fpl, g = f == 2 || f == 4 || f == 8 ? f : dflt; return std::min(g, tt / 4); }
+#define GT_MLPG_DISPATCH(LAUNCH) \
+  if (tt == 16) { if (fpl == 2) LAUNCH(2, 16) else LAUNCH(4, 16) } \
+  else { if (fpl == 2) LAUNCH(2, 32) else if (fpl == 4) LAUNCH(4, 32) else LAUNCH(8, 32) }
+#define GT_MLPG_DISPATCH_BWD(LAUNCH) \
+  if (tt == 16) LAUNCH(4, 16) else { if (fpl == 4) LAUNCH(4, 32) else LAUNCH(8, 32) }
+#define GT_MLPG_WINDOWS(LAUNCH, F, TTV) \
+  { if (nW == 1) LAUNCH(F, TTV, 1) else if (nW == 2) LAUNCH(F, TTV, 2) else if (nW == 3) LAUNCH(F, TTV, 3) else LAUNCH(F, TTV, 4) }
 int mlpg_forward(gt_engine* e, const float* y, int ldy, const int* scol, const int* sstride, int Ds,
                  float* ys, int ldys, int B, int T, hipStream_t s) {
   const int nW = e->cfg.num_windows, kb = e->mlpg.cur->kb;
-  auto lds_of = [&](int tt) { return ((size_t)(tt + 2 * kb) * nW * MLPG_CC + (size_t)tt * nW * (2 * kb + 1 + 2 * MLPG_PAD)) * sizeof(float); };
-  const int tt = mlpg_tile_frames();
-  const size_t lds = lds_of(tt);
+  const int tt = mlpg_tile_frames(), fpl = mlpg_frames_per_wave(MLPG_FPL_FWD, tt);
+  const size_t lds = (size_t)(tt + 2 * kb) * nW * MLPG_CC * sizeof(float);
   dim3 grid(B * cdiv(T, tt), cdiv(Ds, MLPG_CC));
-  const int fpl = gt_tuning().mlpg_fpl;
 #define GT_MLPG_FWD(F, TTV) { CHK(ensure_dyn_lds((const void*)mlpg_forward_kernel<F, TTV>, lds)); \
-    hipLaunchKernelGGL((mlpg_forward_kernel<F, TTV>), grid, dim3(MLPG_THREADS), lds, s, y, ldy, e->mlpg.cur->band.as<float>(), kb, nW, scol, sstride, Ds, ys, ldys, B, T); }
-  if (tt == 16) GT_MLPG_FWD(2, 16)
-  else { if (fpl == 1) GT_MLPG_FWD(1, 32) else if (fpl == 2) GT_MLPG_FWD(2, 32) else GT_MLPG_FWD(4, 32) }
+    hipLaunchKernelGGL((mlpg_forward_kernel<F, TTV>), grid, dim3(TTV / F * 64), lds, s, y, ldy, e->mlpg.cur->band.as<float>(), kb, nW, scol, sstride, Ds, ys, ldys, B, T); }
+  GT_MLPG_DISPATCH(GT_MLPG_FWD)
 #undef GT_MLPG_FWD
   LAUNCH_CHECK();
   return GT_OK;
 }
 int mlpg_backward(gt_engine* e, const float* gs, int ldgs, const int* scol, const int* sstride, int Ds,
                   float* gy, int ldgy, int B, int T, float mse_w, const float* yhat, const float* ytgt, int ldt,
-                  const float* mask, hipStream_t s) {
+                  const float* mask, hipStream_t s, const StaticFold* fold, const GFinalize* fin) {
   const int nW = e->cfg.num_windows, kb = e->mlpg.cur->kb;
-  auto lds_of = [&](int tt) { return ((size_t)(tt + 2 * kb) * MLPG_CC + (size_t)(tt + 2 * kb) * nW * (2 * kb + 1 + 2 * MLPG_PAD)) * sizeof(float); };
-  const int tt = mlpg_tile_frames();
-  const size_t lds = lds_of(tt);
-  dim3 grid(B * cdiv(T, tt), cdiv(Ds, MLPG_CC));
-  const int fpl = gt_tuning().mlpg_fpl;
-#define GT_MLPG_BWD(F, TTV) { CHK(ensure_dyn_lds((const void*)mlpg_backward_kernel<F, TTV>, lds)); \
-    hipLaunchKernelGGL((mlpg_backward_kernel<F, TTV>), grid, dim3(MLPG_THREADS), lds, s, gs, ldgs, e->mlpg.cur->band.as<float>(), kb, nW, scol, sstride, Ds, \
+  const int tt = mlpg_tile_frames(), fpl = std::max(4, mlpg_frames_per_wave(MLPG_FPL_BWD, tt));
+  const size_t lds = (size_t)(tt + 2 * kb) * MLPG_CC * sizeof(float);
+  const int nx = B * cdiv(T, tt);
+  if (fold) {
+    dim3 grid(nx + (fin && fin->on ? 1 : 0), cdiv(Ds, MLPG_CC));
+    GFinalize f0;
+    memset(&f0, 0, sizeof(f0));
+#define GT_MLPG_BWD_FOLD_W(F, TTV, NWV) { CHK(ensure_dyn_lds((const void*)mlpg_backward_fold_kernel<F, TTV, NWV>, lds)); \
+    hipLaunchKernelGGL((mlpg_backward_fold_kernel<F, TTV, NWV>), grid, dim3(TTV / F * 64), lds, s, *fold, e->mlpg.cur->band.as<float>(), kb, scol, sstride, Ds, \
+                       gy, ldgy, B, T, mse_w, yhat, ytgt, ldt, mask, e->sc(), fin ? *fin : f0, nx); }
+#define GT_MLPG_BWD_FOLD(F, TTV) GT_MLPG_WINDOWS(GT_MLPG_BWD_FOLD_W, F, TTV)
+    GT_MLPG_DISPATCH_BWD(GT_MLPG_BWD_FOLD)
+    ++g_static_grad_paths[1];
+#undef GT_MLPG_BWD_FOLD_W
+#undef GT_MLPG_BWD_FOLD
+    LAUNCH_CHECK();
+    return GT_OK;
+  }
+  dim3 grid(nx, cdiv(Ds, MLPG_CC));
+#define GT_MLPG_BWD_W(F, TTV, NWV) { CHK(ensure_dyn_lds((const void*)mlpg_backward_kernel<F, TTV, NWV>, lds)); \
+    hipLaunchKernelGGL((mlpg_backward_kernel<F, TTV, NWV>), grid, dim3(TTV / F * 64), lds, s, gs, ldgs, e->mlpg.cur->band.as<float>(), kb, scol, sstride, Ds, \
                        gy, ldgy, B, T, mse_w, yhat, ytgt, ldt, mask, e->sc()); }
-  if (tt == 16) GT_MLPG_BWD(2, 16)
-  else { if (fpl == 1) GT_MLPG_BWD(1, 32) else if (fpl == 2) GT_MLPG_BWD(2, 32) else GT_MLPG_BWD(4, 32) }
+#define GT_MLPG_BWD(F, TTV) GT_MLPG_WINDOWS(GT_MLPG_BWD_W, F, TTV)
+  GT_MLPG_DISPATCH_BWD(GT_MLPG_BWD)
+#undef GT_MLPG_BWD_W
 #undef GT_MLPG_BWD
   LAUNCH_CHECK();
   return GT_OK;
@@ -975,7 +1001,7 @@
 }
 
 static int generator_backward(gt_engine* e, const float* x, const float* y, const float* y_hat, const float* mask,
-                              float mse_w, hipStream_t s) {
+                              float mse_w, hipStream_t s, const StaticFold* fold = nullptr, const GFinalize* fin = nullptr) {
   Net& G = e->net[GT_ROLE_G];
   const long N = e->N;
   const int B = e->B, T = e->T, Do = G.d.out_dim;
@@ -983,6 +1009,7 @@
   const int ldgy = mlp_body && (is_i2o(G.d.arch) || e->g_used_mlpg) ? (Do + 3) & ~3 : Do;
   CHK(e->gy.ensure((size_t)N * ldgy * sizeof(float)));
   float* gy = e->gy.as<float>();
+  e->gy_ld = ldgy;
   const float* gs = e->gs.as<float>();
   if (is_i2o(G.d.arch)) {
     const int sd = G.d.static_dim;
@@ -997,7 +1024,8 @@
     CHK(comm_grads_ready(e, GT_ROLE_G, G.gate.dW, (long)sd * sd + sd, s));
     CHK(mlpg_backward(e, e->dgx.as<float>(), sd, e->d_scol_i2o, e->d_sstride_i2o, sd, gy, ldgy, B, T, mse_w, y_hat, y, Do, mask, s));
   } else if (e->g_used_mlpg) {
-    CHK(mlpg_backward(e, gs, e->Ds, e->d_scol, e->d_sstride, e->Ds, gy, ldgy, B, T, mse_w, y_hat, y, Do, mask, s));
+    CHK(mlpg_backward(e, gs, e->Ds, e->d_scol, e->d_sstride, e->Ds, gy, ldgy, B, T, mse_w, y_hat, y, Do, mask, s, fold, fin));
+    if (fold && fin && fin->on) CHK(post_early_results(e, s, fin->ticket_value));
   } else {
     if (mse_w != 0.f) CHK(sum_sqerr(e, y_hat, Do, y, Do, mask, N, Do, &e->sc()->s_mse, gy, Do, mse_w, s));
     hipLaunchKernelGGL(slab_reduce_kernel, dim3(cdiv(N * Do, 256)), dim3(256), 0, s, gs, 0L, 1, N * Do, gy, mse_w != 0.f ? 1 : 0);
@@ -1119,11 +1147,16 @@
   const bool early_now = early_ok && !comm_on(e), comm_early = early_ok && comm_on(e) && e->opt_comm_early_g;
   int mge_blocks = 0;
   e->early_done = false;
+  const bool fold = tr && riders && e->opt_static_fold && !direct && !is_i2o(G.d.arch) && !has_lstm_body(G.d.arch) && G.d.arch != GT_ARCH_SRU;
+  StaticFold sfold;
+  GFinalize gfin;
+  memset(&sfold, 0, sizeof(sfold));
+  memset(&gfin, 0, sizeof(gfin));
   {
     const int nblk = (int)std::min<long>(1024, cdiv(N * Ds, RED_THREADS * 4));
     CHK(e->partial.ensure(4096 * sizeof(double)));
     float* gs = nullptr;
-    if (tr) { CHK(e->gs.ensure((size_t)N * Ds * sizeof(float))); gs = e->gs.as<float>(); }
+    if (tr && !fold) { CHK(e->gs.ensure((size_t)N * Ds * sizeof(float))); gs = e->gs.as<float>(); }
     const float* leak = (tr && e->leak_pending) ? e->leak.as<float>() : nullptr;
     GFinalize fin;
     memset(&fin, 0, sizeof(fin));
@@ -1136,15 +1169,21 @@
       fin.hp = head_blocks ? e->headp.as<HeadPartials>() : (const HeadPartials*)nullptr; fin.n_hp = head_blocks;
       if (riders) { fin.ticket_value = take_ticket(e); fin.ticket = fin.ticket_value ? e->ticket_dev() : (unsigned*)nullptr; }
     }
-    if (tr || !rid)
+    if (fold) {
+      sfold.yhs = y_hat_static; sfold.ys = y_static; sfold.mask = mask; sfold.adv_inv = e->d_adv_inv; sfold.leak = leak; sfold.ldl = e->Da;
+      sfold.gadv = gadv; sfold.lda = e->Da; sfold.mge_w = mge_w; sfold.adv_w = adv_w; sfold.leak_unnorm = leak && e->leak_unnorm ? 1 : 0;
+      gfin = fin;
+    } else if (tr || !rid) {
+      ++g_static_grad_paths[0];
       hipLaunchKernelGGL(static_grad_kernel, dim3(nblk + (rid ? 1 : 0)), dim3(RED_THREADS), 0, s, y_hat_static, Ds,
                          y_static, Ds, mask, N, Ds, mge_w, e->d_adv_inv, leak, e->Da, gadv, e->Da, adv_w, gs, Ds,
                          rid ? (double*)nullptr : e->partial.as<double>(), e->sc(), fin, leak && e->leak_unnorm ? 1 : 0);
-    else
+    } else
       hipLaunchKernelGGL(finalize_g_rider_kernel, dim3(1), dim3(RED_THREADS), 0, s, fin);
     LAUNCH_CHECK();
     mge_blocks = nblk;
-    if (riders) CHK(post_early_results(e, s, fin.ticket_value));
+    if (fold) {}
+    else if (riders) CHK(post_early_results(e, s, fin.ticket_value));
     else if (!early_now && !riders_dp) {
       hipLaunchKernelGGL(sum_partials_kernel, dim3(1), dim3(256), 0, s, e->partial.as<double>(), nblk, &e->sc()->s_mge);
       LAUNCH_CHECK();
@@ -1159,7 +1198,7 @@
   }
   if (comm_early) CHK(comm_early_results(e, GT_ROLE_G, &e->sc()->s_adv, 3, adv_w, mse_w, mge_w, s));
   if (tr) {
-    CHK(generator_backward(e, e->last_x, y, y_hat, mask, mse_w, s));
+    CHK(generator_backward(e, e->last_x, y, y_hat, mask, mse_w, s, fold ? &sfold : nullptr, fold ? &gfin : nullptr));
     e->leak_pending = false; e->leak_unnorm = false;
   }
   CHK(comm_finish_step(e, GT_ROLE_G, tr, &e->sc()->s_adv, comm_early ? 0 : 3, s));
diff --git a/gantts_amd/csrc/engine_internal.hip.h b/gantts_amd/csrc/engine_internal.hip.h
--- a/gantts_amd/csrc/engine_internal.hip.h
+++ b/gantts_amd/csrc/engine_internal.hip.h
@@ -6,6 +6,7 @@
 #include <stdlib.h>
 #include <string.h>
 #include <algorithm>
+#include <atomic>
 #include <map>
 #include <mutex>
 #include <string>
@@ -53,7 +54,7 @@
   int b16_tiles = 0;
   int b16_wg_tile = 0;
   int b16_dma = 1;
-  int mlpg_fpl = 2;
+  int mlpg_fpl = 0;
   int head_vec = 0;
   int mlpg_tt = 0;
   int leak_rider = 1;
@@ -187,6 +188,7 @@
   };
   DImage img_cat, img_cat_b, img_adv2;
   bool d_begin_done = false, g_begin_done = false, g_has_adv = false, g_used_mlpg = false;
+  int gy_ld = 0;
   const float* tv_mask = nullptr; long tv_n = 0; float tv_ovr = 0.f;
   bool early = false, early_done = false;
   hipEvent_t ev_res = nullptr;
@@ -234,6 +236,7 @@
   bool d_unnorm = false, leak_unnorm = false;
   bool opt_poll_results = env_flag("GT_POLL_RESULTS", true);
   bool opt_launch_riders = env_flag("GT_LAUNCH_RIDERS", true);
+  bool opt_static_fold = env_flag("GT_STATIC_FOLD", true);
   int ld_gx = 0, ld_cx = 0;
   Scratch gx_dense, cx_dense;
   bool gx_dense_on = false;
@@ -334,7 +337,7 @@
                  float* ys, int ldys, int B, int T, hipStream_t s);
 int mlpg_backward(gt_engine* e, const float* gs, int ldgs, const int* scol, const int* sstride, int Ds,
                   float* gy, int ldgy, int B, int T, float mse_w, const float* yhat, const float* ytgt, int ldt,
-                  const float* mask, hipStream_t s);
+                  const float* mask, hipStream_t s, const StaticFold* fold = nullptr, const GFinalize* fin = nullptr);
 int post_early_results(gt_engine* e, hipStream_t s, unsigned ticket = 0);
 int cond_dim(gt_engine* e);
 
diff --git a/gantts_amd/csrc/frame_kernels.hip.h b/gantts_amd/csrc/frame_kernels.hip.h
--- a/gantts_amd/csrc/frame_kernels.hip.h
+++ b/gantts_amd/csrc/frame_kernels.hip.h
@@ -277,35 +277,30 @@
 constexpr int MLPG_TT = 32;
 constexpr int MLPG_CC = 64;
 
-constexpr int MLPG_PAD = 3;
 constexpr int MLPG_MAXW = 4;
 constexpr int MLPG_THREADS = 1024;
+constexpr int MLPG_CHUNK = 8;
+constexpr int MLPG_FPL_FWD = 4, MLPG_FPL_BWD = 4;
 
 template <int FPL, int TT = MLPG_TT>
-__global__ __launch_bounds__(MLPG_THREADS) void mlpg_forward_kernel(
+__global__ __launch_bounds__(TT / FPL * 64) void mlpg_forward_kernel(
     const float* __restrict__ y, int ldy, const float* __restrict__ band, int kb, int nW,
     const int* __restrict__ scol, const int* __restrict__ sstride, int Ds,
     float* __restrict__ ys, int ldys, int B, int T) {
   extern __shared__ __attribute__((aligned(16))) float sm[];
-  const int nb = 2 * kb + 1, nbp = nb + 2 * MLPG_PAD;
+  static_assert(TT % FPL == 0 && TT / FPL * 64 <= MLPG_THREADS, "one wave per FPL output frames");
+  const int nb = 2 * kb + 1;
   const int tiles_t = (T + TT - 1) / TT;
   const int b = blockIdx.x / tiles_t, t0 = (blockIdx.x % tiles_t) * TT;
   const int c0 = blockIdx.y * MLPG_CC;
   const int nc = min(MLPG_CC, Ds - c0);
   const int rows = TT + 2 * kb;
-  float* sb = sm + rows * nW * MLPG_CC;
   const float* yb = y + (long)b * T * ldy;
-  const int lane = threadIdx.x & 63, wv = threadIdx.x >> 6, nwv = MLPG_THREADS / 64;
-  float vb0[8];
+  const int lane = threadIdx.x & 63, wv = __builtin_amdgcn_readfirstlane(threadIdx.x >> 6);
+  constexpr int nwv = TT / FPL;
+  const bool c_ok = lane < nc;
+  const int my_col = c_ok ? scol[c0 + lane] : 0, my_st = c_ok ? sstride[c0 + lane] : 0;
   {
-    const long src_rows = (long)T * nW;
-    const int jc = min(max(lane - MLPG_PAD, 0), nb - 1);
-#pragma unroll
-    for (int q = 0; q < 8; ++q) vb0[q] = band[min((long)t0 * nW + wv + q * nwv, src_rows - 1) * nb + jc];
-  }
-  {
-    const bool c_ok = lane < nc;
-    const int my_col = c_ok ? scol[c0 + lane] : 0, my_st = c_ok ? sstride[c0 + lane] : 0;
     const int nrw = rows * nW;
     const int dr = nwv / nW, dw = nwv % nW;
     int r = wv / nW, w = wv % nW;
@@ -327,203 +322,182 @@
       }
     }
   }
+  __syncthreads();
+  const int tl0 = wv * FPL;
+  if (t0 + tl0 >= T) return;
+  float acc[FPL];
+#pragma unroll
+  for (int i = 0; i < FPL; ++i) acc[i] = 0.f;
+  const int rstride = nW * MLPG_CC;
+  for (int w = 0; w < nW; ++w) {
+    const float* dcol = sm + (tl0 * nW + w) * MLPG_CC + lane;
+    const float* cf[FPL];
+#pragma unroll
+    for (int i = 0; i < FPL; ++i) cf[i] = band + ((long)min(t0 + tl0 + i, T - 1) * nW + w) * nb;
+    int j = 0;
+    for (; j + MLPG_CHUNK <= nb; j += MLPG_CHUNK) {
+      float d[MLPG_CHUNK + FPL - 1];
+#pragma unroll
+      for (int u = 0; u < MLPG_CHUNK + FPL - 1; ++u) d[u] = dcol[(j + u) * rstride];
+#pragma unroll
+      for (int i = 0; i < FPL; ++i)
+#pragma unroll
+        for (int u = 0; u < MLPG_CHUNK; ++u) acc[i] = fmaf(cf[i][j + u], d[i + u], acc[i]);
+    }
+    for (; j < nb; ++j) {
+#pragma unroll
+      for (int i = 0; i < FPL; ++i) acc[i] = fmaf(cf[i][j], dcol[(j + i) * rstride], acc[i]);
+    }
+  }
+  if (!c_ok) return;
+  const bool pass = my_st == 0;
+#pragma unroll
+  for (int i = 0; i < FPL; ++i) {
+    const int t = t0 + tl0 + i;
+    if (t >= T) break;
+    const float out = pass ? sm[((tl0 + i + kb) * nW + 0) * MLPG_CC + lane] : acc[i];
+    ys[((long)b * T + t) * ldys + c0 + lane] = out;
+  }
+}
+
+struct StaticFold {
+  const float* yhs; const float* ys; const float* mask; const int* adv_inv;
+  const float* leak; int ldl; const float* gadv; int lda;
+  float mge_w, adv_w; int leak_unnorm;
+};
+
+template <int FPL, int TT, int NW, bool FOLD>
+__device__ __forceinline__ void mlpg_backward_body(
+    const float* __restrict__ gs, int ldgs, const StaticFold& fold, const float* __restrict__ band, int kb,
+    const int* __restrict__ scol, const int* __restrict__ sstride, int Ds,
+    float* __restrict__ gy, int ldgy, int B, int T,
+    float mse_w, const float* __restrict__ yhat, const float* __restrict__ ytgt, int ldt,
+    const float* __restrict__ mask, const StepScalars* __restrict__ sc, float* sm, int blk_x) {
+  static_assert(TT % FPL == 0 && TT / FPL * 64 <= MLPG_THREADS, "one wave per FPL output frames");
+  static_assert(NW >= 1 && NW <= MLPG_MAXW, "windows");
+  constexpr int nW = NW;
+  const int nb = 2 * kb + 1;
+  const int tiles_t = (T + TT - 1) / TT;
+  const int b = blk_x / tiles_t, t0 = (blk_x % tiles_t) * TT;
+  const int c0 = blockIdx.y * MLPG_CC;
+  const int nc = min(MLPG_CC, Ds - c0);
+  const int rows = TT + 2 * kb;
+  const int lane = threadIdx.x & 63, wv = __builtin_amdgcn_readfirstlane(threadIdx.x >> 6);
+  constexpr int nwv = TT / FPL;
+  const bool c_ok = lane < nc;
   {
-    const int nrow = TT * nW;
-    const long src_rows = (long)T * nW;
-    if (lane < nbp) {
-      const int j = lane - MLPG_PAD;
-      const bool j_ok = j >= 0 && j < nb;
-#pragma unroll
-      for (int q = 0; q < 8; ++q) {
-        const int tw = wv + q * nwv;
-        if (tw < nrow) sb[tw * nbp + lane] = (j_ok && (long)t0 * nW + tw < src_rows) ? vb0[q] : 0.f;
-      }
-    }
-    for (int jp = lane; jp < nbp; jp += 64) {
-      const int j = jp - MLPG_PAD;
-      const bool j_ok = j >= 0 && j < nb;
-      const int jc = min(max(j, 0), nb - 1);
-      for (int tw0 = jp == lane ? wv + 8 * nwv : wv; tw0 < nrow; tw0 += 8 * nwv) {
-        float v[8];
+    const int ccl = c_ok ? c0 + lane : c0;
+    float sc2 = 0.f, leak_s = 1.f;
+    int jadv = -1;
+    if constexpr (FOLD) {
+      sc2 = 2.f * fold.mge_w * sc->inv_tv;
+      leak_s = fold.leak_unnorm ? sc->inv_tv : 1.f;
+      jadv = fold.adv_inv ? fold.adv_inv[ccl] : -1;
+    }
+    for (int r0 = wv; r0 < rows; r0 += 8 * nwv) {
+      float v[8];
+      if constexpr (FOLD) {
+        float m[8], yv[8], tv[8], lk[8], ga[8];
 #pragma unroll
         for (int q = 0; q < 8; ++q) {
-          const long row = (long)t0 * nW + tw0 + q * nwv;
-          const float x = band[min(row, src_rows - 1) * nb + jc];
-          v[q] = (j_ok && row < src_rows) ? x : 0.f;
+          const int t = t0 - kb + r0 + q * nwv;
+          const long n = (long)b * T + min(max(t, 0), T - 1);
+          m[q] = fold.mask[n]; yv[q] = fold.yhs[n * Ds + ccl]; tv[q] = fold.ys[n * Ds + ccl];
+          lk[q] = (jadv >= 0 && fold.leak) ? fold.leak[n * fold.ldl + jadv] : 0.f;
+          ga[q] = (jadv >= 0 && fold.gadv) ? fold.gadv[n * fold.lda + jadv] : 0.f;
         }
 #pragma unroll
         for (int q = 0; q < 8; ++q) {
-          const int tw = tw0 + q * nwv;
-          if (tw < nrow) sb[tw * nbp + jp] = v[q];
+          const int t = t0 - kb + r0 + q * nwv;
+          const float diff = yv[q] * m[q] - tv[q] * m[q];
+          float x = sc2 * diff * m[q];
+          if (jadv >= 0) {
+            if (fold.leak) x += leak_s * lk[q];
+            if (fold.gadv) x += fold.adv_w * ga[q];
+          }
+          v[q] = (c_ok && t >= 0 && t < T) ? x : 0.f;
+        }
+      } else {
+        const float* gb = gs + (long)b * T * ldgs;
+#pragma unroll
+        for (int q = 0; q < 8; ++q) {
+          const int t = t0 - kb + r0 + q * nwv;
+          const int tc = min(max(t, 0), T - 1);
+          const float x = gb[(long)tc * ldgs + ccl];
+          v[q] = (c_ok && t >= 0 && t < T) ? x : 0.f;
         }
       }
+#pragma unroll
+      for (int q = 0; q < 8; ++q) {
+        const int r = r0 + q * nwv;
+        if (r < rows) sm[r * MLPG_CC + lane] = v[q];
+      }
     }
   }
   __syncthreads();
-  static_assert(FPL >= 1 && FPL <= MLPG_PAD + 1, "the band rows are padded for at most MLPG_PAD + 1 frames per lane");
-  if (threadIdx.x >= TT * 32 / FPL) return;
-  const int cp = threadIdx.x & 31, fg = threadIdx.x >> 5;
-  const int tl0 = fg * FPL;
-  float acc[FPL][2];
-#pragma unroll
-  for (int i = 0; i < FPL; ++i) acc[i][0] = acc[i][1] = 0.f;
+  const int tl0 = wv * FPL;
+  if (t0 + tl0 >= T) return;
+  float acc[NW][FPL];
+#pragma unroll
+  for (int w = 0; w < NW; ++w)
+#pragma unroll
+    for (int i = 0; i < FPL; ++i) acc[w][i] = 0.f;
   const int ntap = (FPL - 1) + nb;
-  for (int w = 0; w < nW; ++w) {
-    const float* dcol = sm + (tl0 * nW + w) * MLPG_CC + 2 * cp;
-    const float* cf = sb + (tl0 * nW + w) * nbp + MLPG_PAD;
-#pragma unroll 8
-    for (int j0 = 0; j0 < ntap; ++j0) {
-      const float2 d = *reinterpret_cast<const float2*>(dcol + j0 * nW * MLPG_CC);
-#pragma unroll
-      for (int i = 0; i < FPL; ++i) {
-        const float cfi = cf[i * nW * nbp + j0 - i];
-        acc[i][0] = fmaf(cfi, d.x, acc[i][0]);
-        acc[i][1] = fmaf(cfi, d.y, acc[i][1]);
-      }
-    }
-  }
-#pragma unroll
-  for (int q = 0; q < 2; ++q) {
-    const int c = 2 * cp + q;
-    if (c >= nc) continue;
-    const bool pass = sstride[c0 + c] == 0;
-#pragma unroll
-    for (int i = 0; i < FPL; ++i) {
-      const int t = t0 + tl0 + i;
-      if (t >= T) continue;
-      const float out = pass ? sm[((tl0 + i + kb) * nW + 0) * MLPG_CC + c] : acc[i][q];
-      ys[((long)b * T + t) * ldys + c0 + c] = out;
-    }
-  }
-}
-
-template <int FPL, int TT = MLPG_TT>
-__global__ __launch_bounds__(MLPG_THREADS) __attribute__((amdgpu_waves_per_eu(FPL <= 2 ? 8 : 4)))
-void mlpg_backward_kernel(
-    const float* __restrict__ gs, int ldgs, const float* __restrict__ band, int kb, int nW,
+  const float* drow = sm + tl0 * MLPG_CC + lane;
+  const int tb = t0 - kb + tl0;
+  auto edge_row = [&](int j0) {
+    const float d = drow[j0 * MLPG_CC];
+    const float* cf = band + (long)min(max(tb + j0, 0), T - 1) * nW * nb + (nb - 1 - j0);
+#pragma unroll
+    for (int w = 0; w < NW; ++w) {
+#pragma unroll
+      for (int i = 0; i < FPL; ++i)
+        if (j0 - i >= 0 && j0 - i < nb) acc[w][i] = fmaf(cf[w * nb + i], d, acc[w][i]);
+    }
+  };
+#pragma unroll
+  for (int j0 = 0; j0 < FPL - 1; ++j0) edge_row(j0);
+#pragma unroll 4
+  for (int j0 = FPL - 1; j0 < nb; ++j0) {
+    const float d = drow[j0 * MLPG_CC];
+    const float* cf = band + (long)min(max(tb + j0, 0), T - 1) * nW * nb + (nb - 1 - j0);
+#pragma unroll
+    for (int w = 0; w < NW; ++w) {
+#pragma unroll
+      for (int i = 0; i < FPL; ++i) acc[w][i] = fmaf(cf[w * nb + i], d, acc[w][i]);
+    }
+  }
+  for (int j0 = max(nb, FPL - 1); j0 < ntap; ++j0) edge_row(j0);
+  if (!c_ok) return;
+  const float msk_scale = mse_w != 0.f ? 2.f * mse_w * sc->inv_tv : 0.f;
+  const int col0 = scol[c0 + lane], st = sstride[c0 + lane];
+#pragma unroll
+  for (int i = 0; i < FPL; ++i) {
+    const int tp = t0 + tl0 + i;
+    if (tp >= T) break;
+    const long row = (long)b * T + tp;
+    const float m = msk_scale != 0.f ? mask[row] : 0.f;
+#pragma unroll
+    for (int w = 0; w < NW; ++w) {
+      if (st == 0 && w > 0) break;
+      float out = st == 0 ? sm[(tl0 + i + kb) * MLPG_CC + lane] : acc[w][i];
+      const int col = col0 + w * st;
+      if (msk_scale != 0.f) out += msk_scale * (yhat[row * ldt + col] * m - ytgt[row * ldt + col] * m) * m;
+      gy[row * ldgy + col] = out;
+    }
+  }
+}
+
+template <int FPL, int TT, int NW>
+__global__ __launch_bounds__(TT / FPL * 64) void mlpg_backward_kernel(
+    const float* __restrict__ gs, int ldgs, const float* __restrict__ band, int kb,
     const int* __restrict__ scol, const int* __restrict__ sstride, int Ds,
     float* __restrict__ gy, int ldgy, int B, int T,
     float mse_w, const float* __restrict__ yhat, const float* __restrict__ ytgt, int ldt,
     const float* __restrict__ mask, const StepScalars* __restrict__ sc) {
   extern __shared__ __attribute__((aligned(16))) float sm[];
-  const int nb = 2 * kb + 1, nbp = nb + 2 * MLPG_PAD;
-  const int tiles_t = (T + TT - 1) / TT;
-  const int b = blockIdx.x / tiles_t, t0 = (blockIdx.x % tiles_t) * TT;
-  const int c0 = blockIdx.y * MLPG_CC;
-  const int nc = min(MLPG_CC, Ds - c0);
-  const int rows = TT + 2 * kb;
-  float* sb = sm + rows * MLPG_CC;
-  const float* gb = gs + (long)b * T * ldgs;
-  const int lane = threadIdx.x & 63, wv = threadIdx.x >> 6, nwv = MLPG_THREADS / 64;
-  float vb0[16];
-  {
-    const long src_rows = (long)T * nW, base = (long)(t0 - kb) * nW;
-    const int jc = min(max(lane - MLPG_PAD, 0), nb - 1);
-#pragma unroll
-    for (int q = 0; q < 16; ++q) vb0[q] = band[min(max(base + wv + q * nwv, 0L), src_rows - 1) * nb + jc];
-  }
-  {
-    const bool c_ok = lane < nc;
-    const int ccl = c_ok ? c0 + lane : c0;
-    for (int r0 = wv; r0 < rows; r0 += 8 * nwv) {
-      float v[8];
-#pragma unroll
-      for (int q = 0; q < 8; ++q) {
-        const int t = t0 - kb + r0 + q * nwv;
-        const int tc = min(max(t, 0), T - 1);
-        const float x = gb[(long)tc * ldgs + ccl];
-        v[q] = (c_ok && t >= 0 && t < T) ? x : 0.f;
-      }
-#pragma unroll
-      for (int q = 0; q < 8; ++q) {
-        const int r = r0 + q * nwv;
-        if (r < rows) sm[r * MLPG_CC + lane] = v[q];
-      }
-    }
-  }
-  {
-    const int nrow = rows * nW;
-    const long src_rows = (long)T * nW, base = (long)(t0 - kb) * nW;
-    if (lane < nbp) {
-      const int j = lane - MLPG_PAD;
-      const bool j_ok = j >= 0 && j < nb;
-#pragma unroll
-      for (int q = 0; q < 16; ++q) {
-        const int rw = wv + q * nwv;
-        const long row = base + rw;
-        if (rw < nrow) sb[rw * nbp + lane] = (j_ok && row >= 0 && row < src_rows) ? vb0[q] : 0.f;
-      }
-    }
-    for (int jp = lane; jp < nbp; jp += 64) {
-      const int j = jp - MLPG_PAD;
-      const bool j_ok = j >= 0 && j < nb;
-      const int jc = min(max(j, 0), nb - 1);
-      for (int rw0 = jp == lane ? wv + 16 * nwv : wv; rw0 < nrow; rw0 += 8 * nwv) {
-        float v[8];
-#pragma unroll
-        for (int q = 0; q < 8; ++q) {
-          const long row = base + rw0 + q * nwv;
-          const float x = band[min(max(row, 0L), src_rows - 1) * nb + jc];
-          v[q] = (j_ok && row >= 0 && row < src_rows) ? x : 0.f;
-        }
-#pragma unroll
-        for (int q = 0; q < 8; ++q) {
-          const int rw = rw0 + q * nwv;
-          if (rw < nrow) sb[rw * nbp + jp] = v[q];
-        }
-      }
-    }
-  }
-  __syncthreads();
-  static_assert(FPL >= 1 && FPL <= MLPG_PAD + 1, "the band rows are padded for at most MLPG_PAD + 1 frames per lane");
-  if (threadIdx.x >= TT * 32 / FPL) return;
-  const int cp = threadIdx.x & 31, fg = threadIdx.x >> 5;
-  const int tl0 = fg * FPL;
-  float acc[MLPG_MAXW][FPL][2];
-#pragma unroll
-  for (int w = 0; w < MLPG_MAXW; ++w)
-#pragma unroll
-    for (int i = 0; i < FPL; ++i) acc[w][i][0] = acc[w][i][1] = 0.f;
-  const int ntap = (FPL - 1) + nb;
-  const float* drow = sm + tl0 * MLPG_CC + 2 * cp;
-  const float* cfrow = sb + (long)tl0 * nW * nbp + MLPG_PAD + (nb - 1);
-#pragma unroll 4
-  for (int j0 = 0; j0 < ntap; ++j0) {
-    const float2 d = *reinterpret_cast<const float2*>(drow + j0 * MLPG_CC);
-    const float* cf = cfrow + (long)j0 * nW * nbp - j0;
-#pragma unroll
-    for (int w = 0; w < MLPG_MAXW; ++w) {
-      if (w >= nW) break;
-#pragma unroll
-      for (int i = 0; i < FPL; ++i) {
-        const float cfi = cf[w * nbp + i];
-        acc[w][i][0] = fmaf(cfi, d.x, acc[w][i][0]);
-        acc[w][i][1] = fmaf(cfi, d.y, acc[w][i][1]);
-      }
-    }
-  }
-  const float msk_scale = mse_w != 0.f ? 2.f * mse_w * sc->inv_tv : 0.f;
-#pragma unroll
-  for (int q = 0; q < 2; ++q) {
-    const int c = 2 * cp + q;
-    if (c >= nc) continue;
-    const int col0 = scol[c0 + c], st = sstride[c0 + c];
-#pragma unroll
-    for (int i = 0; i < FPL; ++i) {
-      const int tp = t0 + tl0 + i;
-      if (tp >= T) continue;
-      const long row = (long)b * T + tp;
-      const float m = msk_scale != 0.f ? mask[row] : 0.f;
-#pragma unroll
-      for (int w = 0; w < MLPG_MAXW; ++w) {
-        if (w >= nW || (st == 0 && w > 0)) break;
-        float out = st == 0 ? sm[(tl0 + i + kb) * MLPG_CC + c] : acc[w][i][q];
-        const int col = col0 + w * st;
-        if (msk_scale != 0.f) out += msk_scale * (yhat[row * ldt + col] * m - ytgt[row * ldt + col] * m) * m;
-        gy[row * ldgy + col] = out;
-      }
-    }
-  }
+  StaticFold none = {};
+  mlpg_backward_body<FPL, TT, NW, false>(gs, ldgs, none, band, kb, scol, sstride, Ds, gy, ldgy, B, T, mse_w, yhat, ytgt, ldt, mask, sc, sm, blockIdx.x);
 }
 
 __device__ __forceinline__ double masked_sqerr_body(
@@ -849,23 +823,26 @@
                                                 int zero_gnorm, const double* __restrict__ part_mge, int n_mge,
                                                 const double* __restrict__ part_mse, int n_mse,
                                                 const HeadPartials* __restrict__ hp, int n_hp, double* shp ,
-                                                unsigned* ticket = nullptr, unsigned ticket_value = 0) {
+                                                unsigned* ticket = nullptr, unsigned ticket_value = 0,
+                                                int nthr = 0 ) {
+  const int nt = nthr ? nthr : (int)blockDim.x;
+  const int i0 = (int)threadIdx.x < nt ? (int)threadIdx.x : 0x7fffffff - nt;
   if (part_mge || part_mse || hp) {
     if (part_mge) {
       double v = 0.0;
-      for (int i = threadIdx.x; i < n_mge; i += blockDim.x) v += __builtin_nontemporal_load(part_mge + i);
+      for (int i = i0; i < n_mge; i += nt) v += __builtin_nontemporal_load(part_mge + i);
       const double t = block_sum_d(v, shp);
       if (threadIdx.x == 0) sc->s_mge = t;
     }
     if (part_mse) {
       double v = 0.0;
-      for (int i = threadIdx.x; i < n_mse; i += blockDim.x) v += __builtin_nontemporal_load(part_mse + i);
+      for (int i = i0; i < n_mse; i += nt) v += __builtin_nontemporal_load(part_mse + i);
       const double t = block_sum_d(v, shp);
       if (threadIdx.x == 0) sc->s_mse = t;
     }
     if (hp) {
       double v = 0.0;
-      for (int i = threadIdx.x; i < n_hp; i += blockDim.x) v += hp[i].s_real;
+      for (int i = i0; i < n_hp; i += nt) v += hp[i].s_real;
       const double t = block_sum_d(v, shp);
       if (threadIdx.x == 0) sc->s_adv = t;
     }
@@ -969,6 +946,25 @@
   __shared__ double sh[16];
   finalize_g_body(fin.sc, fin.out, fin.adv_w, fin.mse_w, fin.mge_w, fin.has_adv, 1, fin.part_mge, fin.n_mge, fin.part_mse, fin.n_mse,
                   fin.hp, fin.n_hp, sh, fin.ticket, fin.ticket_value);
+}
+
+template <int FPL, int TT, int NW>
+__global__ __launch_bounds__(TT / FPL * 64) void mlpg_backward_fold_kernel(
+    const StaticFold fold, const float* __restrict__ band, int kb,
+    const int* __restrict__ scol, const int* __restrict__ sstride, int Ds,
+    float* __restrict__ gy, int ldgy, int B, int T,
+    float mse_w, const float* __restrict__ yhat, const float* __restrict__ ytgt, int ldt,
+    const float* __restrict__ mask, const StepScalars* __restrict__ sc, const GFinalize fin, int nx) {
+  extern __shared__ __attribute__((aligned(16))) float sm[];
+  static_assert(TT / FPL * 64 >= RED_THREADS, "the finalisation rider sums as static_grad_kernel's workgroup does");
+  if ((int)blockIdx.x >= nx) {
+    __shared__ double sh[16];
+    if (blockIdx.y == 0)
+      finalize_g_body(fin.sc, fin.out, fin.adv_w, fin.mse_w, fin.mge_w, fin.has_adv, 1, fin.part_mge, fin.n_mge, fin.part_mse, fin.n_mse,
+                      fin.hp, fin.n_hp, sh, fin.ticket, fin.ticket_value, RED_THREADS);
+    return;
+  }
+  mlpg_backward_body<FPL, TT, NW, true>(nullptr, 0, fold, band, kb, scol, sstride, Ds, gy, ldgy, B, T, mse_w, yhat, ytgt, ldt, mask, sc, sm, blockIdx.x);
 }
 
 static __global__ void scale_by_inv_tv_kernel(float* __restrict__ g, long n, const StepScalars* __restrict__ sc) {
diff --git a/gantts_amd/engine.py b/gantts_amd/engine.py
--- a/gantts_amd/engine.py
+++ b/gantts_amd/engine.py
@@ -231,7 +231,7 @@
                 "comm_force": L.OPT_COMM_FORCE, "launch_riders": L.OPT_LAUNCH_RIDERS,
                 "comm_close_inline": L.OPT_COMM_CLOSE_INLINE, "poll_results": L.OPT_POLL_RESULTS,
                 "comm_tv_in_sums": L.OPT_COMM_TV_IN_SUMS, "comm_ipc": L.OPT_COMM_IPC, "fused_dstack": L.OPT_FUSED_DSTACK,
-                "sru_d_bf16": L.OPT_SRU_D_BF16}
+                "sru_d_bf16": L.OPT_SRU_D_BF16, "static_fold": L.OPT_STATIC_FOLD}
         if name not in opts:
             raise ValueError("unknown engine option %r" % (name,))
         check(lib.gt_set_option(self._h, opts[name], int(value)))
@@ -463,6 +463,11 @@
             return out, out2
         return out.squeeze(0) if squeeze else out
 
+    def peek_gy(self, rows, cols):
+        out = torch.empty(rows, cols, device="cuda", dtype=torch.float32)
+        check(lib.gt_op_peek_gy(self._h, ptr(out), int(rows), int(cols), L.current_stream()))
+        return out
+
     def mlpg_forward(self, y, R):
         y = _check_frames(y, "inputs")
         R = _check_frames(R, "R")
diff --git a/include/gantts_hip.h b/include/gantts_hip.h
--- a/include/gantts_hip.h
+++ b/include/gantts_hip.h
@@ -164,6 +164,7 @@
 #define GT_OPT_COMM_IPC 18
 #define GT_OPT_FUSED_DSTACK 19
 #define GT_OPT_SRU_D_BF16 20
+#define GT_OPT_STATIC_FOLD 21
 int gt_set_option(gt_engine* e, int option, int value);
 int gt_set_tuning(const char* name, int value);
 int gt_set_x_pitch(gt_engine* e, int ld_generator_input, int ld_condition);
@@ -228,6 +229,8 @@
                            gt_distortion_sums* out, void* stream);
 int gt_op_mlpg_forward(gt_engine* e, const float* y, const float* R, int B, int T, float* y_static, void* stream);
 int gt_op_mlpg_backward(gt_engine* e, const float* g_static, const float* R, int B, int T, float* g_y, void* stream);
+int gt_static_grad_path_counts(int64_t out[2]);
+int gt_op_peek_gy(gt_engine* e, float* out, int64_t rows, int cols, void* stream);
 int gt_op_linear_forward(const float* X, int ldx, const float* W, const float* bias, float* Y, int ldy,
                          int64_t rows, int in_dim, int out_dim, int act, const float* keep_mask, float p,
                          void* stream);
```
